# eBay/KPRN

Hardware: AMD Instinct MI355X
Metric: paths/sec (train+score) at path_len=6 d=64 (higher is better)
Workload: dtype f32

## Files before the change

### kprn_amd/csrc/batch_index.hip

```cpp
#include <string.h>
#include <rocprim/device/device_radix_sort.hpp>
#include <rocprim/device/device_run_length_encode.hpp>
#include <rocprim/device/device_select.hpp>
#include <rocprim/iterator/counting_iterator.hpp>

#include <algorithm>

#include "kprn_internal.h"

namespace bidx {

namespace {
__global__ void k_keys(const int32_t* __restrict__ idx, int64_t N, int T, int F, const int32_t* __restrict__ tile_k,
                       const int32_t* __restrict__ meta, int kcap, int sentinel, int32_t* __restrict__ keys, int32_t* __restrict__ vals) {
  const int64_t i = (int64_t)blockIdx.x * blockDim.x + threadIdx.x;
  const int64_t nsteps = N * T;
  if (i < nsteps) {
    const int64_t n = i / T;
    const int t = (int)(i - n * T);
    const bool skipped = tile_k && t < tile_k[n >> 6];
    keys[i] = skipped ? sentinel : idx[i * F + F - 2] - 1;
    vals[i] = (int32_t)i;
  } else if (i < nsteps + kcap) {
    const int t = (int)(i - nsteps);
    const int64_t npad = (N + 63) / 64 * 64;
    keys[i] = (t < meta[0]) ? meta[8 + F - 2] - 1 : sentinel;
    vals[i] = (int32_t)(npad * T + t);
  }
}
__global__ void k_drop_sentinel(const int32_t* __restrict__ uniq, const int32_t* __restrict__ runs, int sentinel, int32_t* __restrict__ count_out) {
  const int n = *runs;
  *count_out = (n > 0 && uniq[n - 1] == sentinel) ? n - 1 : n;
}
int bits_for(int64_t v) { int b = 1; while (((int64_t)1 << b) < v) ++b; return b; }

__global__ void k_find_ref(const int32_t* __restrict__ idx, int64_t N, int T, int F, int c0, int32_t* __restrict__ meta) {
  const int64_t n = (int64_t)blockIdx.x * blockDim.x + threadIdx.x;
  if (n >= N) return;
  const int32_t* r = idx + n * T * F;
  bool same = true;
  for (int c = c0; c < F; ++c) same &= (r[c] == r[F + c]);
  if (same) atomicMin(meta + 1, (int32_t)n);
}
__global__ void k_prefix_len(const int32_t* __restrict__ idx, int64_t N, int T, int F, int c0, int kcap, int32_t* __restrict__ meta,
                             int32_t* __restrict__ keys, int32_t* __restrict__ vals) {
  const int64_t n = (int64_t)blockIdx.x * blockDim.x + threadIdx.x;
  if (n >= N) return;
  const int ref = meta[1];
  int k = 0;
  if (ref != 0x7fffffff) {
    const int32_t* q = idx + (int64_t)ref * T * F;
    const int32_t* r = idx + n * T * F;
    const int kmax = (T - 2 < kcap) ? T - 2 : kcap;
    while (k < kmax) {
      bool same = true;
      for (int c = c0; c < F; ++c) same &= (r[k * F + c] == q[c]);
      if (!same) break;
      ++k;
    }
    if (n == 0) for (int c = 0; c < F; ++c) meta[8 + c] = q[c];
  }
  keys[n] = k;
  vals[n] = (int32_t)n;
}
__global__ void k_prefix_apply(const int32_t* __restrict__ idx, int64_t N, int T, int F, const int32_t* __restrict__ ksorted,
                               const int32_t* __restrict__ perm, int32_t* __restrict__ idx_s, int32_t* __restrict__ slot_of, int32_t* __restrict__ tile_k,
                               int32_t* __restrict__ meta) {
  const int64_t i = (int64_t)blockIdx.x * blockDim.x + threadIdx.x;
  const int64_t row = (int64_t)T * F;
  if (i < N * row) {
    const int64_t n = i / row;
    idx_s[i] = idx[(int64_t)perm[n] * row + (i - n * row)];
  }
  if (i < N) slot_of[perm[i]] = (int32_t)i;
  if (i < (N + 63) / 64) tile_k[i] = ksorted[i * 64];
  if (i == 0) meta[0] = ksorted[N - 1];
}
}

size_t prefix_scratch_bytes(int64_t N, int kcap) {
  size_t t1 = 0;
  int32_t* p = nullptr;
  (void)rocprim::radix_sort_pairs(nullptr, t1, p, p, p, p, (size_t)N, 0, bits_for(kcap + 1), (hipStream_t)0);
  return (size_t)N * 3 * sizeof(int32_t) + ((t1 + 255) & ~(size_t)255) + 1024;
}

void prefix_plan(hipStream_t s, const int32_t* idx, int64_t N, int T, int F, int nT, int kcap, int32_t* idx_s, int32_t* perm, int32_t* slot_of, int32_t* tile_k,
                 int32_t* meta, void* scratch, size_t scratch_sz) {
  int32_t* keys = (int32_t*)scratch;
  int32_t* vals = keys + N;
  int32_t* ksorted = vals + N;
  char* tmp = (char*)(ksorted + N);
  tmp = (char*)(((uintptr_t)tmp + 255) & ~(uintptr_t)255);
  const size_t tmp_bytes = scratch_sz - (size_t)(tmp - (char*)scratch);
  const int c0 = F - nT - 2;
  HIP_TRY(hipMemsetAsync(meta, 0, (size_t)(8 + F) * sizeof(int32_t), s));
  HIP_TRY(hipMemsetD32Async((hipDeviceptr_t)(meta + 1), 0x7fffffff, 1, s));
  const dim3 gn((unsigned)((N + 255) / 256));
  hipLaunchKernelGGL(k_find_ref, gn, dim3(256), 0, s, idx, N, T, F, c0, meta);
  hipLaunchKernelGGL(k_prefix_len, gn, dim3(256), 0, s, idx, N, T, F, c0, kcap, meta, keys, vals);
  HIP_TRY(hipGetLastError());
  size_t need = 0;
  HIP_TRY(rocprim::radix_sort_pairs(nullptr, need, keys, ksorted, vals, perm, (size_t)N, 0, bits_for(kcap + 1), s));
  KPRN_REQUIRE(need <= tmp_bytes, KPRN_E_DEVICE, "prefix plan scratch too small");
  HIP_TRY(rocprim::radix_sort_pairs(tmp, need, keys, ksorted, vals, perm, (size_t)N, 0, bits_for(kcap + 1), s));
  const int64_t work = N * T * F;
  hipLaunchKernelGGL(k_prefix_apply, dim3((unsigned)((work + 255) / 256)), dim3(256), 0, s, idx, N, T, F, ksorted, perm, idx_s, slot_of, tile_k, meta);
  HIP_TRY(hipGetLastError());
}

size_t scratch_bytes(int64_t n_index, int Ve) {
  size_t t1 = 0, t2 = 0;
  int32_t* p = nullptr;
  (void)rocprim::radix_sort_pairs(nullptr, t1, p, p, p, p, (size_t)n_index, 0, bits_for((int64_t)Ve + 1), (hipStream_t)0);
  (void)rocprim::run_length_encode(nullptr, t2, p, (size_t)n_index, p, p, p, (hipStream_t)0);
  const size_t tmp = (t1 > t2 ? t1 : t2);
  return (size_t)n_index * 3 * sizeof(int32_t) + ((tmp + 255) & ~(size_t)255) + 1024 + 256;
}

void build(hipStream_t s, const int32_t* idx, int64_t N, int T, int F, int Ve, const int32_t* tile_k, const int32_t* meta, int kcap,
           int32_t* key_sorted, int32_t* pos_sorted, int32_t* uniq, int32_t* n_uniq_dev, void* scratch, size_t scratch_sz) {
  const int64_t n_index = N * T + (tile_k ? kcap : 0);
  if (n_index <= 0) return;
  int32_t* keys = (int32_t*)scratch;
  int32_t* vals = keys + n_index;
  int32_t* counts = vals + n_index;
  char* tmp = (char*)(counts + n_index);
  tmp = (char*)(((uintptr_t)tmp + 255) & ~(uintptr_t)255);
  int32_t* runs = (int32_t*)tmp;
  tmp += 256;
  size_t tmp_bytes = scratch_sz - (size_t)(tmp - (char*)scratch);
  const int sentinel = Ve;
  const int bits = bits_for((int64_t)Ve + 1);
  hipLaunchKernelGGL(k_keys, dim3((unsigned)((n_index + 255) / 256)), dim3(256), 0, s, idx, N, T, F, tile_k, meta, tile_k ? kcap : 0, sentinel, keys, vals);
  HIP_TRY(hipGetLastError());
  size_t need = 0;
  HIP_TRY(rocprim::radix_sort_pairs(nullptr, need, keys, key_sorted, vals, pos_sorted, (size_t)n_index, 0, bits, s));
  KPRN_REQUIRE(need <= tmp_bytes, KPRN_E_DEVICE, "batch index scratch too small (sort)");
  HIP_TRY(rocprim::radix_sort_pairs(tmp, need, keys, key_sorted, vals, pos_sorted, (size_t)n_index, 0, bits, s));
  HIP_TRY(rocprim::run_length_encode(nullptr, need, key_sorted, (size_t)n_index, uniq, counts, runs, s));
  KPRN_REQUIRE(need <= tmp_bytes, KPRN_E_DEVICE, "batch index scratch too small (rle)");
  HIP_TRY(rocprim::run_length_encode(tmp, need, key_sorted, (size_t)n_index, uniq, counts, runs, s));
  hipLaunchKernelGGL(k_drop_sentinel, dim3(1), dim3(1), 0, s, uniq, runs, sentinel, n_uniq_dev);
  HIP_TRY(hipGetLastError());
}

}

namespace bidx {
namespace {
template <int FRAG, bool DET>
__device__ __forceinline__ void entity_grad_body(const float* __restrict__ DX, const int32_t* __restrict__ key_sorted,
                                                 const int32_t* __restrict__ pos_sorted, int64_t nsteps, int64_t N, int T, int D, int dt, int de,
                                                 int sentinel, float* __restrict__ gWe, int n_ent_blocks, int n_red_blocks, const SlabReduce red,
                                                 const SmallGrad sg, const int dbg, float* const det_seg, float* const det_sg) {
  const int order = (dbg >> 4) & 3;
  const int n_pass = gridDim.x - n_ent_blocks;
  int bid = blockIdx.x, rb = -1;
  if (order == 1) { if (bid < n_pass) { rb = bid; } else bid -= n_pass; }
  else if (order == 2) {
    const int both = 2 * (n_pass < n_ent_blocks ? n_pass : n_ent_blocks);
    if (bid < both) { if (bid & 1) rb = bid >> 1; else bid >>= 1; }
    else if (n_pass > n_ent_blocks) rb = bid - n_ent_blocks;
    else bid -= n_pass;
  } else if (bid >= n_ent_blocks) rb = bid - n_ent_blocks;
  if (rb >= 0) {
    if (dbg & 2) return;
    if (rb >= n_red_blocks) {
      if constexpr (DET) small_grad_block<true>(sg, rb - n_red_blocks, det_sg);
      else if (!(dbg & 8)) small_grad_block(sg, rb - n_red_blocks);
      return;
    }
    if (dbg & 4) return;
    const int nbx = (red.n_elem + 255) / 256;
    slab_reduce_block(red, rb % nbx, (rb / nbx) % red.ny, rb / (nbx * red.ny));
    return;
  }
  const int lane = threadIdx.x & 63;
  const int64_t seg = (int64_t)bid * 4 + (threadIdx.x >> 6);
  const int64_t base = seg * 64;
  if (base >= nsteps) return;
  const int cnt = (int)((nsteps - base < 64) ? (nsteps - base) : 64);
  const int64_t mine = base + (lane < cnt ? lane : cnt - 1);
  const int key_ld = key_sorted[mine], pos_ld = pos_sorted[mine];
  const int kb_ld = key_sorted[base > 0 ? base - 1 : 0], ka_ld = key_sorted[base + cnt < nsteps ? base + cnt : nsteps - 1];
  const int my_key = (lane < cnt) ? key_ld : -1;
  if (__builtin_amdgcn_readlane(my_key, 0) == sentinel) return;
  const int my_pos = (lane < cnt) ? pos_ld : 0;
  const int key_before = (base > 0) ? kb_ld : -1;
  const int key_after = (base + cnt < nsteps) ? ka_ld : -1;
  const int waves_per_group = D >> 4;
  const int key_next = __shfl_down(my_key, 1, 64);
  const bool is_end = (lane < cnt) && (lane == cnt - 1 || key_next != my_key);
  const unsigned long long endmask = __ballot(is_end);
  const bool continues = __builtin_amdgcn_readlane(my_key, (cnt - 1) & 63) == key_after;
  for (int c0 = 0; c0 < de; c0 += 64) {
    const bool act = c0 + lane < de;
    const int ecol = act ? c0 + lane : de - 1;
    const int col = dt + ecol;
    const int coff = (col >> 4) * 256 + (col & 15) * 4;
    float acc = 0.f;
    bool opened_here = __builtin_amdgcn_readlane(my_key, 0) != key_before;
#pragma unroll
    for (int hf = 0; hf < 2; ++hf) {
      if (hf * 32 >= cnt) break;
      float v[32];
#pragma unroll
      for (int i2 = 0; i2 < 32; ++i2) {
        const int i = 32 * hf + i2;
        const int p = __builtin_amdgcn_readlane(my_pos, i);
        const int n = p / T, t = p - n * T;
        int64_t off;
        if (FRAG == 1) {
          const int rr = n & 15;
          off = ((int64_t)(n >> 4) * T + t) * ((int64_t)waves_per_group * 256) + (rr >> 2) * 64 + (rr & 3) + coff;
        } else if (FRAG == 2) {
          off = (int64_t)p * de + ecol;
        } else {
          off = ((int64_t)t * N + n) * D + col;
        }
        v[i2] = DX[off];
      }
#pragma unroll
      for (int i2 = 0; i2 < 32; ++i2) {
        const int i = 32 * hf + i2;
        acc += v[i2];
        if (endmask & (1ull << i)) {
          const int k = __builtin_amdgcn_readlane(my_key, i);
          const bool whole = opened_here && !(i == cnt - 1 && continues);
          if (act && k != sentinel) {
            float* dst = gWe + (int64_t)k * de + ecol;
            if (whole) *dst = acc;
            else if constexpr (DET) det_seg[(seg * 2 + (opened_here ? 1 : 0)) * de + ecol] = acc;
            else if (!(dbg & 1)) unsafeAtomicAdd(dst, acc);
          }
          acc = 0.f;
          opened_here = true;
        }
      }
    }
  }
}
template <int FRAG>
__global__ __launch_bounds__(256) void k_entity_grad(const float* __restrict__ DX, const int32_t* __restrict__ key_sorted,
                                                     const int32_t* __restrict__ pos_sorted, int64_t nsteps, int64_t N, int T, int D, int dt, int de,
                                                     int sentinel, float* __restrict__ gWe, int n_ent_blocks, int n_red_blocks, SlabReduce red,
                                                     SmallGrad sg, int dbg) {
  entity_grad_body<FRAG, false>(DX, key_sorted, pos_sorted, nsteps, N, T, D, dt, de, sentinel, gWe, n_ent_blocks, n_red_blocks, red, sg, dbg, nullptr, nullptr);
}
__global__ __launch_bounds__(256) void k_egrad_det(const float* __restrict__ DX, const int32_t* __restrict__ key_sorted, const int32_t* __restrict__ pos_sorted,
                                                   int64_t nsteps, int64_t N, int T, int D, int dt, int de, int sentinel, float* __restrict__ gWe,
                                                   int n_ent_blocks, int n_red_blocks, SlabReduce red, SmallGrad sg, DetEntity det) {
  entity_grad_body<2, true>(DX, key_sorted, pos_sorted, nsteps, N, T, D, dt, de, sentinel, gWe, n_ent_blocks, n_red_blocks, red, sg, 0, det.seg_part, det.sg_part);
}
__global__ __launch_bounds__(256) void k_egrad_det_rowmajor(const float* __restrict__ DX, const int32_t* __restrict__ key_sorted, const int32_t* __restrict__ pos_sorted,
                                                            int64_t nsteps, int64_t N, int T, int D, int dt, int de, int sentinel, float* __restrict__ gWe,
                                                            int n_ent_blocks, int n_red_blocks, SlabReduce red, SmallGrad sg, DetEntity det) {
  entity_grad_body<0, true>(DX, key_sorted, pos_sorted, nsteps, N, T, D, dt, de, sentinel, gWe, n_ent_blocks, n_red_blocks, red, sg, 0, det.seg_part, det.sg_part);
}

__global__ __launch_bounds__(256) void k_det_tail(const int32_t* __restrict__ key_sorted, int64_t nsteps, int de, int sentinel, float* __restrict__ gWe,
                                                  int n_ent_blocks, DetEntity det, SmallGrad sg, int n_sg_groups) {
  constexpr int DEPTH = 16;
  if ((int)blockIdx.x >= n_ent_blocks) {
    const int ncb_t = sg.dt >> 4, ncb = ncb_t + (sg.dr >> 4);
    const int cb = (int)blockIdx.x - n_ent_blocks;
    const bool is_type = cb < ncb_t;
    const int v = threadIdx.x >> 4, c = threadIdx.x & 15;
    float acc = 0.f;
    for (int g0 = 0; g0 < n_sg_groups; g0 += DEPTH) {
      float x[DEPTH];
#pragma unroll
      for (int u = 0; u < DEPTH; ++u) {
        const int g = g0 + u < n_sg_groups ? g0 + u : n_sg_groups - 1;
        x[u] = det.sg_part[((int64_t)g * ncb + cb) * 256 + threadIdx.x];
      }
#pragma unroll
      for (int u = 0; u < DEPTH; ++u) if (g0 + u < n_sg_groups) acc += x[u];
    }
    if (v < (is_type ? sg.Vt : sg.Vr)) {
      if (is_type) sg.gWt[(int64_t)v * sg.dt + cb * 16 + c] += acc;
      else sg.gWr[(int64_t)v * sg.dr + (cb - ncb_t) * 16 + c] += acc;
    }
    return;
  }
  const int lane = threadIdx.x & 63;
  const int64_t seg = (int64_t)blockIdx.x * 4 + (threadIdx.x >> 6);
  const int64_t base = seg * 64;
  if (base + 64 >= nsteps) return;
  const int k = key_sorted[base + 63];
  if (k == sentinel || key_sorted[base + 64] != k) return;
  if (key_sorted[base] == k && base > 0 && key_sorted[base - 1] == k) return;
  const int64_t n_seg = (nsteps + 63) / 64;
  for (int c0 = 0; c0 < de; c0 += 64) {
    const int ecol = c0 + lane < de ? c0 + lane : de - 1;
    float acc = det.seg_part[(seg * 2 + 1) * de + ecol];
    bool more = true;
    for (int64_t s0 = seg + 1; more; s0 += DEPTH) {
      float x[DEPTH];
      int ks[DEPTH];
#pragma unroll
      for (int u = 0; u < DEPTH; ++u) {
        const int64_t sc = s0 + u < n_seg ? s0 + u : n_seg - 1;
        ks[u] = key_sorted[sc * 64];
        x[u] = det.seg_part[(sc * 2) * de + ecol];
      }
#pragma unroll
      for (int u = 0; u < DEPTH; ++u) {
        more = more && s0 + u < n_seg && ks[u] == k;
        if (more) acc += x[u];
      }
    }
    if (c0 + lane < de) gWe[(int64_t)k * de + ecol] += acc;
  }
}
}

void entity_grad_tail(hipStream_t s, const int32_t* key_sorted, int64_t n_index, int de, int Ve, float* gWe, const DetEntity& det, const SmallGrad* sg) {
  const int64_t segs = (n_index + 63) / 64;
  const int n_ent = (int)((segs + 3) / 4);
  SmallGrad g;
  memset(&g, 0, sizeof(g));
  int ncb = 0, groups = 0;
  if (sg) { g = *sg; ncb = (g.dt >> 4) + (g.dr >> 4); groups = g.nblocks / ncb; }
  if (n_ent + ncb <= 0) return;
  hipLaunchKernelGGL(k_det_tail, dim3((unsigned)(n_ent + ncb)), dim3(256), 0, s, key_sorted, n_index, de, Ve, gWe, n_ent, det, g, groups);
  HIP_TRY(hipGetLastError());
}

void entity_grad(hipStream_t s, const float* DX, int frag_order, const int32_t* key_sorted, const int32_t* pos_sorted, int64_t n_index, int64_t N,
                 int T, int D, int dt, int de, int Ve, float* gWe, const SlabReduce* red, const SmallGrad* sg, const DetEntity* det) {
  if (n_index <= 0 && !red && !sg) return;
  const int64_t segs = (n_index + 63) / 64;
  const int n_ent = (int)((segs + 3) / 4);
  SlabReduce r;
  memset(&r, 0, sizeof(r));
  SmallGrad g;
  memset(&g, 0, sizeof(g));
  int n_red = 0, n_sg = 0;
  if (red) { r = *red; n_red = ((r.n_elem + 255) / 256) * r.ny * r.L; }
  if (sg) { g = *sg; n_sg = g.nblocks; }
  static const int dbg = KPRN_DEV_ENV("KPRN_EGRAD_DBG") ? atoi(KPRN_DEV_ENV("KPRN_EGRAD_DBG")) : 0;
  const dim3 grid((unsigned)(n_ent + n_red + n_sg));
  if (det) {
    KPRN_REQUIRE(frag_order == 2 || (frag_order == 0 && !red && !sg), KPRN_E_UNSUPPORTED,
                 "deterministic entity gradient: the compact entity slice, or row-major dx without passenger jobs");
    if (frag_order == 0)
      hipLaunchKernelGGL(k_egrad_det_rowmajor, grid, dim3(256), 0, s, DX, key_sorted, pos_sorted, n_index, N, T, D, dt, de, Ve, gWe, n_ent, n_red, r, g, *det);
    else
    hipLaunchKernelGGL(k_egrad_det, grid, dim3(256), 0, s, DX, key_sorted, pos_sorted, n_index, N, T, D, dt, de, Ve, gWe, n_ent, n_red, r, g, *det);
  } else
  if (frag_order == 1) hipLaunchKernelGGL(k_entity_grad<1>, grid, dim3(256), 0, s, DX, key_sorted, pos_sorted, n_index, N, T, D, dt, de, Ve, gWe, n_ent, n_red, r, g, dbg);
  else if (frag_order == 2) hipLaunchKernelGGL(k_entity_grad<2>, grid, dim3(256), 0, s, DX, key_sorted, pos_sorted, n_index, N, T, D, dt, de, Ve, gWe, n_ent, n_red, r, g, dbg);
  else hipLaunchKernelGGL(k_entity_grad<0>, grid, dim3(256), 0, s, DX, key_sorted, pos_sorted, n_index, N, T, D, dt, de, Ve, gWe, n_ent, n_red, r, g, dbg);
  HIP_TRY(hipGetLastError());
}
}

namespace bidx {
namespace {
typedef float f32x4m __attribute__((ext_vector_type(4)));
__global__ void k_add_rank(const int32_t* __restrict__ buf, int cap, int de, float* __restrict__ G, int32_t* __restrict__ mark) {
  const int count = buf[0];
  const int per = de >> 2;
  const float* rows = (const float*)(buf + 4 + cap);
  for (int64_t i = (int64_t)blockIdx.x * blockDim.x + threadIdx.x; i < (int64_t)count * per; i += (int64_t)gridDim.x * blockDim.x) {
    const int k = (int)(i / per), c = (int)(i - (int64_t)k * per) * 4;
    const int row = buf[4 + k];
    f32x4m* dst = (f32x4m*)(G + (int64_t)row * de + c);
    *dst = *dst + *(const f32x4m*)(rows + (int64_t)k * de + c);
    if (c == 0) mark[row] = 1;
  }
}
__global__ void k_add_rank_scalar(const int32_t* __restrict__ buf, int cap, int de, float* __restrict__ G, int32_t* __restrict__ mark) {
  const int count = buf[0];
  const float* rows = (const float*)(buf + 4 + cap);
  for (int64_t i = (int64_t)blockIdx.x * blockDim.x + threadIdx.x; i < (int64_t)count * de; i += (int64_t)gridDim.x * blockDim.x) {
    const int k = (int)(i / de), c = (int)(i - (int64_t)k * de);
    const int row = buf[4 + k];
    G[(int64_t)row * de + c] += rows[(int64_t)k * de + c];
    if (c == 0) mark[row] = 1;
  }
}
__global__ void k_unmark(const int32_t* __restrict__ all, int world, int cap, int64_t stride, int32_t* __restrict__ mark) {
  const int64_t i = (int64_t)blockIdx.x * blockDim.x + threadIdx.x;
  if (i >= (int64_t)world * cap) return;
  const int r = (int)(i / cap), k = (int)(i - (int64_t)r * cap);
  const int32_t* buf = all + (int64_t)r * stride;
  if (k < buf[0]) mark[buf[4 + k]] = 0;
}
}

size_t merge_scratch_bytes(int64_t n, int Ve) {
  size_t t1 = 0;
  int32_t* p = nullptr;
  (void)rocprim::select(nullptr, t1, rocprim::counting_iterator<int32_t>(0), p, p, p, (size_t)Ve, (hipStream_t)0);
  return ((t1 + 255) & ~(size_t)255) + 1024;
}

void merge_rows(hipStream_t s, const void* all, int world, int cap, int de, int Ve, float* G, int32_t* union_rows, int32_t* union_count,
                int32_t* mark, void* scratch, size_t scratch_sz, int64_t tail_words) {
  const int64_t n = (int64_t)world * cap;
  if (n <= 0) return;
  const int64_t stride = 4 + (int64_t)cap * (1 + de) + tail_words;
  for (int r = 0; r < world; ++r) {
    const int32_t* buf = (const int32_t*)all + (int64_t)r * stride;
    if ((de & 3) == 0) {
      const int64_t work = (int64_t)cap * (de >> 2);
      hipLaunchKernelGGL(k_add_rank, dim3((unsigned)std::min<int64_t>((work + 255) / 256, 16384)), dim3(256), 0, s, buf, cap, de, G, mark);
    } else {
      const int64_t work = (int64_t)cap * de;
      hipLaunchKernelGGL(k_add_rank_scalar, dim3((unsigned)std::min<int64_t>((work + 255) / 256, 16384)), dim3(256), 0, s, buf, cap, de, G, mark);
    }
  }
  size_t need = 0;
  HIP_TRY(rocprim::select(nullptr, need, rocprim::counting_iterator<int32_t>(0), mark, union_rows, union_count, (size_t)Ve, s));
  KPRN_REQUIRE(need <= scratch_sz, KPRN_E_DEVICE, "merge scratch too small (select)");
  HIP_TRY(rocprim::select(scratch, need, rocprim::counting_iterator<int32_t>(0), mark, union_rows, union_count, (size_t)Ve, s));
  hipLaunchKernelGGL(k_unmark, dim3((unsigned)((n + 255) / 256)), dim3(256), 0, s, (const int32_t*)all, world, cap, stride, mark);
  HIP_TRY(hipGetLastError());
}

}
```

### kprn_amd/csrc/kernels_basic.hip

```cpp
#include <string.h>
#include "kprn_internal.h"
#include "adam_rows_dev.h"
#include "reduce_dev.h"

namespace {

constexpr int TPB = 256;
inline unsigned nblocks(int64_t n, int per = TPB) { return (unsigned)((n + per - 1) / per); }

__device__ __forceinline__ void lds_atomic_add(float* p, float v) {
  typedef __attribute__((address_space(3))) float lds_float;
  __hip_atomic_fetch_add((lds_float*)p, v, __ATOMIC_RELAXED, __HIP_MEMORY_SCOPE_WORKGROUP);
}

__device__ __forceinline__ float wave_sum(float v) {
#pragma unroll
  for (int o = 32; o > 0; o >>= 1) v += __shfl_down(v, o, 64);
  return v;
}

__global__ void k_validate(const int32_t* __restrict__ idx, int64_t nsteps, int F, int nT, int Vt, int Ve, int Vr, int32_t* flag) {
  int64_t i = (int64_t)blockIdx.x * blockDim.x + threadIdx.x;
  if (i >= nsteps) return;
  const int32_t* f = idx + i * F;
// ... 1319 lines not shown
      if (lane < dcols) lds_atomic_add(&acc[id[u] * dcols + lane], x[u][0]);
      if (lane + 64 < dcols) lds_atomic_add(&acc[id[u] * dcols + lane + 64], x[u][1]);
    }
  }
  __syncthreads();
  for (int i = threadIdx.x; i < V * dcols; i += 256) {
    const float v = acc[i];
    if (v != 0.f && !(dbg & 2)) unsafeAtomicAdd(gW + i, v);
  }
}

template <int RT, bool DET = false>
__global__ __launch_bounds__(256) void k_table_grad_mfma(const int32_t* __restrict__ idx, int64_t N, int T, int F, int idcol, int slots,
                                                          const float* __restrict__ dX, int D, int col0, int dcols, int V, float* __restrict__ gW,
                                                          int pos_per_block) {
  typedef float f4 __attribute__((ext_vector_type(4)));
  const int lane = threadIdx.x & 63, wv = threadIdx.x >> 6;
  const int kk = lane >> 4, n16 = lane & 15;
  const int ncb = (dcols + 15) >> 4;
  f4 acc[RT][2];
#pragma unroll
  for (int r = 0; r < RT; ++r) { acc[r][0] = f4{0.f, 0.f, 0.f, 0.f}; acc[r][1] = f4{0.f, 0.f, 0.f, 0.f}; }
  const int64_t total = N * T;
  const int64_t p0 = (int64_t)blockIdx.x * pos_per_block;
  const int np = (int)((p0 + pos_per_block < total ? p0 + pos_per_block : total) - p0);
  const int t0 = (int)(p0 / N);
  const int64_t n0 = p0 - (int64_t)t0 * N;
  if (wv >= ncb) return;
  const int c_a = 16 * wv + n16, c_b = 16 * (wv + 4) + n16;
  const bool has_a = wv < ncb && c_a < dcols, has_b = wv + 4 < ncb && c_b < dcols;
  constexpr int UN = 4;
  for (int q0 = 0; q0 < np; q0 += 4 * UN) {
    float xa[UN], xb[UN];
    int id[UN];
    int64_t ioff[UN];
#pragma unroll
    for (int u = 0; u < UN; ++u) {
      const int q = q0 + 4 * u + kk;
      const bool live = q < np;
      int t = t0;
      int64_t n = n0 + (live ? q : 0);
      while (n >= N) { n -= N; ++t; }
      const float* src = dX + (p0 + (live ? q : 0)) * D + col0;
      const float va = src[has_a ? c_a : 0], vb = src[has_b ? c_b : 0];
      ioff[u] = (n * T + t) * F + idcol;
      const int idr = idx[ioff[u]];
      xa[u] = (live && has_a) ? va : 0.f;
      xb[u] = (live && has_b) ? vb : 0.f;
      id[u] = live ? idr - 1 : -1;
    }
#pragma unroll
    for (int u = 0; u < UN; ++u) {
      for (int sl = 0; sl < slots; ++sl) {
        const int idv = (sl == 0) ? id[u] : ((id[u] >= 0) ? idx[ioff[u] + sl] - 1 : -1);
#pragma unroll
        for (int r = 0; r < RT; ++r) {
          if (RT > 1 && __ballot((idv >> 4) == r) == 0) continue;
          const float onehot = (idv == 16 * r + n16) ? 1.f : 0.f;
          acc[r][0] = __builtin_amdgcn_mfma_f32_16x16x4f32(onehot, xa[u], acc[r][0], 0, 0, 0);
          if (wv + 4 < ncb) acc[r][1] = __builtin_amdgcn_mfma_f32_16x16x4f32(onehot, xb[u], acc[r][1], 0, 0, 0);
        }
      }
    }
  }
#pragma unroll
  for (int r = 0; r < RT; ++r)
#pragma unroll
    for (int i = 0; i < 4; ++i) {
      const int v = 16 * r + 4 * kk + i;
      if (v < V) {
        if constexpr (DET) {
          float* const blk = gW + (int64_t)blockIdx.x * V * dcols;
          if (has_a) blk[(int64_t)v * dcols + c_a] = acc[r][0][i];
          if (has_b) blk[(int64_t)v * dcols + c_b] = acc[r][1][i];
        } else {
          if (has_a && acc[r][0][i] != 0.f) unsafeAtomicAdd(gW + (int64_t)v * dcols + c_a, acc[r][0][i]);
          if (has_b && acc[r][1][i] != 0.f) unsafeAtomicAdd(gW + (int64_t)v * dcols + c_b, acc[r][1][i]);
        }
      }
    }
}

static bool table_grad_mfma(hipStream_t s, const int32_t* idx, int64_t N, int T, int F, int idcol, int slots, const float* dX, int D, int col0, int dcols,
                            int V, float* gW, DetScratch* det = nullptr) {
  if (dcols <= 0 || dcols > 128 || V <= 0 || V > 128) return false;
  static const int ppb_env = KPRN_DEV_ENV("KPRN_TABLE_GRAD_PPB") ? atoi(KPRN_DEV_ENV("KPRN_TABLE_GRAD_PPB")) : 0;
  const int ppb = ppb_env > 0 ? ppb_env : 512;
  const int64_t total = N * T;
  const dim3 grid((unsigned)((total + ppb - 1) / ppb));
  if (det) {
    float* const slab = det_reserve(det, s, (int64_t)grid.x * V * dcols);
#define KPRN_TGD(RT_) hipLaunchKernelGGL((k_table_grad_mfma<RT_, true>), grid, dim3(256), 0, s, idx, N, T, F, idcol, slots, dX, D, col0, dcols, V, slab, ppb)
    if (V <= 16) KPRN_TGD(1);
    else if (V <= 32) KPRN_TGD(2);
    else if (V <= 64) KPRN_TGD(4);
    else KPRN_TGD(8);
#undef KPRN_TGD
    slab_join(s, slab, (int)grid.x, (int64_t)V * dcols, 1, V * dcols, gW, (int64_t)V * dcols);
    return true;
  }
#define KPRN_TG(RT_) hipLaunchKernelGGL(k_table_grad_mfma<RT_>, grid, dim3(256), 0, s, idx, N, T, F, idcol, slots, dX, D, col0, dcols, V, gW, ppb)
  if (V <= 16) KPRN_TG(1);
  else if (V <= 32) KPRN_TG(2);
  else if (V <= 64) KPRN_TG(4);
  else KPRN_TG(8);
#undef KPRN_TG
  return true;
}

static bool table_grad_lds(hipStream_t s, const int32_t* idx, int64_t N, int T, int F, int idcol, int slots, const float* dX, int D, int col0, int dcols,
                           int V, float* gW) {
  const size_t bytes = (size_t)V * dcols * sizeof(float);
  if (dcols <= 0 || dcols > 128 || bytes > 64 * 1024) return false;
  static PerDeviceOnce attr_set;
  if (bytes > 48 * 1024 && attr_set.need()) {
    HIP_TRY(hipFuncSetAttribute((const void*)k_table_grad_lds, hipFuncAttributeMaxDynamicSharedMemorySize, 64 * 1024));
  }
  const int64_t total = N * T;
  int ppb = 512;
  while (ppb < 8192 && (int64_t)V * dcols * 8 > (int64_t)ppb * dcols) ppb *= 2;
  static const int ppb_env = KPRN_DEV_ENV("KPRN_TABLE_GRAD_PPB") ? atoi(KPRN_DEV_ENV("KPRN_TABLE_GRAD_PPB")) : 0;
  if (ppb_env > 0) ppb = ppb_env;
  static const int dbg_env = KPRN_DEV_ENV("KPRN_TABLE_GRAD_DBG") ? atoi(KPRN_DEV_ENV("KPRN_TABLE_GRAD_DBG")) : 0;
  hipLaunchKernelGGL(k_table_grad_lds, dim3((unsigned)((total + ppb - 1) / ppb)), dim3(256), bytes, s, idx, N, T, F, idcol, slots, dX, D, col0, dcols, V, gW, ppb, dbg_env);
  return true;
}

__global__ __launch_bounds__(256) void k_onehot_cols(const int32_t* __restrict__ idx, int64_t NT, int64_t N, int T, int F, int Vr, int Vt, float* __restrict__ X, int64_t ldx,
                                                     int col0, int ns) {
  const int nq = ns >> 2;
  const int64_t g = (int64_t)blockIdx.x * 256 + threadIdx.x;
  if (g >= NT * nq) return;
  const int64_t pos = g / nq;
  const int q = (int)(g - pos * nq);
  const int64_t t = pos / N, n = pos - t * N;
  const int32_t* id = idx + (n * T + t) * F;
  const int r = id[F - 1] - 1, y = Vr + id[F - 3] - 1;
  float4 v;
  v.x = (4 * q == r || 4 * q == y) ? 1.f : 0.f;
  v.y = (4 * q + 1 == r || 4 * q + 1 == y) ? 1.f : 0.f;
  v.z = (4 * q + 2 == r || 4 * q + 2 == y) ? 1.f : 0.f;
  v.w = (4 * q + 3 == r || 4 * q + 3 == y) ? 1.f : 0.f;
  float* dst = X + pos * ldx + col0 + 4 * q;
  dst[0] = v.x; dst[1] = v.y; dst[2] = v.z; dst[3] = v.w;
}
void onehot_cols(hipStream_t s, const int32_t* idx, int64_t N, int T, int F, int Vr, int Vt, float* X, int64_t ldx, int col0, int ns) {
  const int64_t work = N * T * (ns >> 2);
  if (work <= 0) return;
  hipLaunchKernelGGL(k_onehot_cols, dim3((unsigned)((work + 255) / 256)), dim3(256), 0, s, idx, N * T, N, T, F, Vr, Vt, X, ldx, col0, ns);
  HIP_TRY(hipGetLastError());
}
__global__ __launch_bounds__(256) void k_small_tables_finish_f32(const float* __restrict__ Ct, int ns, int GH, int Din, int dt, int de, int dr, int Vt, int Vr,
                                                                 const float* __restrict__ Wt, const float* __restrict__ Wr, const float* __restrict__ Wi,
                                                                 float* __restrict__ gWi, float* __restrict__ gWt, float* __restrict__ gWr, int with_e) {
  __shared__ float g[128];
  const int tid = threadIdx.x, NZ = ns + (with_e ? de : 0);
  if ((int)blockIdx.x < GH) {
    const int k = blockIdx.x;
    const float* row = Ct + (int64_t)k * NZ;
    if (tid < ns) g[tid] = row[tid];
    __syncthreads();
    for (int j = tid; j < Din; j += 256) {
      float v = 0.f;
      if (j < dt) {
        for (int y = 0; y < Vt; ++y) v += g[Vr + y] * Wt[y * dt + j];
      } else if (j < dt + de) {
        if (!with_e) continue;
        v = row[ns + j - dt];
      } else {
        const int jj = j - dt - de;
        for (int r = 0; r < Vr; ++r) v += g[r] * Wr[r * dr + jj];
      }
      gWi[(int64_t)k * Din + j] += v;
    }
    return;
  }
  __shared__ float red[256];
  const int r = (int)blockIdx.x - GH;
  const bool rel = r < Vr;
  const int w = rel ? dr : dt, col0 = rel ? dt + de : 0;
  const int j = tid & 15, sb = tid >> 4;
  for (int j0 = 0; j0 < w; j0 += 16) {
    const int jj = j0 + j, jc = jj < w ? jj : w - 1;
    float acc = 0.f;
#pragma unroll 4
    for (int k = sb; k < GH; k += 16) acc += Ct[(int64_t)k * NZ + r] * Wi[(int64_t)k * Din + col0 + jc];
    red[tid] = acc;
    __syncthreads();
    if (sb == 0 && jj < w) {
      float v = 0.f;
#pragma unroll
      for (int q = 0; q < 16; ++q) v += red[q * 16 + j];
      (rel ? gWr + (int64_t)r * dr : gWt + (int64_t)(r - Vr) * dt)[jj] += v;
    }
    __syncthreads();
  }
}
void small_tables_finish(hipStream_t s, const float* Ct, int ns, int GH, int Din, int dt, int de, int dr, int Vt, int Vr, const float* Wt, const float* Wr,
                         const float* Wi, float* gWi, float* gWt, float* gWr, bool ct_has_entity) {
  hipLaunchKernelGGL(k_small_tables_finish_f32, dim3((unsigned)(GH + Vr + Vt)), dim3(256), 0, s, Ct, ns, GH, Din, dt, de, dr, Vt, Vr, Wt, Wr, Wi, gWi, gWt, gWr,
                     ct_has_entity ? 1 : 0);
  HIP_TRY(hipGetLastError());
}

bool embed_scatter_det_ok(int dt, int dr, int Vt, int Vr) { return (dt == 0 || (dt <= 128 && Vt >= 1 && Vt <= 128)) && (dr == 0 || (dr <= 128 && Vr >= 1 && Vr <= 128)); }

void embed_scatter(hipStream_t s, const int32_t* idx, int64_t N, int T, int F, int nT, const float* dX, int dt, int de, int dr, int Vt, int Vr,
                   float* gWt, float* gWe, float* gWr, bool skip_entity, DetScratch* det) {
  if (N <= 0) return;
  const int D_ = dt + de + dr;
  static const bool old_path = KPRN_DEV_ENV("KPRN_TABLE_GRAD") && strcmp(KPRN_DEV_ENV("KPRN_TABLE_GRAD"), "old") == 0;
  bool type_small = false, rel_small = false;
  static const bool lds_path = KPRN_DEV_ENV("KPRN_TABLE_GRAD") && strcmp(KPRN_DEV_ENV("KPRN_TABLE_GRAD"), "lds") == 0;
  if (det) {
    KPRN_REQUIRE(!old_path && !lds_path && skip_entity && embed_scatter_det_ok(dt, dr, Vt, Vr), KPRN_E_UNSUPPORTED,
                 "deterministic: the embedding scatter has a deterministic form for type / relation tables of at most 128 rows x 128 columns behind the occurrence index only");
    if (dt > 0) table_grad_mfma(s, idx, N, T, F, F - nT - 2, nT, dX, D_, 0, dt, Vt, gWt, det);
    if (dr > 0) table_grad_mfma(s, idx, N, T, F, F - 1, 1, dX, D_, dt + de, dr, Vr, gWr, det);
    CHECK_LAUNCH();
    return;
  }
  if (!old_path && !lds_path) {
    if (dt > 0) type_small = table_grad_mfma(s, idx, N, T, F, F - nT - 2, nT, dX, D_, 0, dt, Vt, gWt);
    if (dr > 0) rel_small = table_grad_mfma(s, idx, N, T, F, F - 1, 1, dX, D_, dt + de, dr, Vr, gWr);
  } else if (lds_path) {
    if (dt > 0 && Vt > 16) type_small = table_grad_lds(s, idx, N, T, F, F - nT - 2, nT, dX, D_, 0, dt, Vt, gWt);
    if (dr > 0 && Vr > 16) rel_small = table_grad_lds(s, idx, N, T, F, F - 1, 1, dX, D_, dt + de, dr, Vr, gWr);
  }
  const int ppb = 512;
  if (!type_small && dt > 0 && Vt <= 16) {
    hipLaunchKernelGGL(k_small_table_grad, dim3((unsigned)((N * T + ppb - 1) / ppb), (unsigned)((dt + 63) / 64)), dim3(256), 0, s, idx, N, T, F, F - nT - 2, nT,
                       dX, D_, 0, dt, Vt, gWt, ppb);
    type_small = true;
  }
  if (!rel_small && dr > 0 && Vr <= 16) {
    hipLaunchKernelGGL(k_small_table_grad, dim3((unsigned)((N * T + ppb - 1) / ppb), (unsigned)((dr + 63) / 64)), dim3(256), 0, s, idx, N, T, F, F - 1, 1, dX,
                       D_, dt + de, dr, Vr, gWr, ppb);
    rel_small = true;
  }
  if ((type_small || dt == 0) && (rel_small || dr == 0) && (skip_entity || de == 0)) { CHECK_LAUNCH(); return; }
  if (type_small) { Vt = 0; }
  size_t small = (size_t)((int64_t)(type_small ? 0 : Vt) * dt + (int64_t)(rel_small ? 0 : Vr) * dr) * sizeof(float);
  int use_lds = small <= 96 * 1024 ? 1 : 0;
  const int spb = 256;
  int64_t total = N * T;
  if (use_lds && small > 48 * 1024)
    HIP_TRY(hipFuncSetAttribute((const void*)k_embed_scatter, hipFuncAttributeMaxDynamicSharedMemorySize, (int)small));
  hipLaunchKernelGGL(k_embed_scatter, dim3((unsigned)((total + spb - 1) / spb)), dim3(TPB), use_lds ? small : 0, s, idx, N, T, F, nT, dX, dt, de,
                     dr, type_small ? 0 : Vt, rel_small ? 0 : Vr, gWt, gWe, gWr, use_lds, spb, skip_entity ? 1 : 0, type_small ? 1 : 0, rel_small ? 1 : 0);
  CHECK_LAUNCH();
}

void sumsq(hipStream_t s, const float* x, int64_t n, float* out) {
  if (n <= 0) return;
  unsigned g = nblocks(n);
  if (g > 2048) g = 2048;
  hipLaunchKernelGGL(k_sumsq, dim3(g), dim3(TPB), 0, s, x, n, out);
  CHECK_LAUNCH();
}

void sumsq_rows(hipStream_t s, const float* G, const int32_t* rows, const int32_t* count, int d, float* out) {
  hipLaunchKernelGGL(k_sumsq_rows, dim3(1024), dim3(TPB), 0, s, G, rows, count, d, out);
  CHECK_LAUNCH();
}

void sumsq_det(hipStream_t s, const float* x, int64_t n, const float* G, const int32_t* rows, const int32_t* count, int d, float* partial, float* out) {
  const int nb = SUMSQ_DET_BLOCKS / 2;
  hipLaunchKernelGGL(k_sumsq_det, dim3(2 * nb), dim3(256), 0, s, x, n, G, rows, count, d, nb, partial);
  hipLaunchKernelGGL(k_sum_partials, dim3(1), dim3(256), 0, s, partial, 2 * nb, out, 0);
  CHECK_LAUNCH();
}

static AdamDenseJob dense_job(float* x, float* g, float* m, float* v, int64_t n, float step, float b1, float b2, float eps,
                              const float* norm2, float clip, float l2, int consume, int64_t z0, int zn0, int64_t z1, int zn1, float* tab_slot) {
  AdamDenseJob a;
  a.x = x; a.g = g; a.m = m; a.v = v; a.n = n; a.step = step; a.b1 = b1; a.b2 = b2; a.eps = eps; a.norm2 = norm2; a.clip = clip; a.l2 = l2;
  a.reg = (norm2 != nullptr || l2 != 0.f) ? 1 : 0; a.consume = consume; a.z0 = z0; a.zn0 = zn0; a.z1 = z1; a.zn1 = zn1; a.tab_slot = tab_slot;
  return a;
}
void adam_dense(hipStream_t s, float* x, float* g, float* m, float* v, int64_t n, float step, float b1, float b2, float eps,
                const float* norm2, float clip, float l2, int consume, int64_t z0, int zn0, int64_t z1, int zn1, float* tab_slot) {
  if (n <= 0) return;
  hipLaunchKernelGGL(k_adam_dense, dim3(nblocks(n)), dim3(TPB), 0, s, dense_job(x, g, m, v, n, step, b1, b2, eps, norm2, clip, l2, consume, z0, zn0, z1, zn1, tab_slot));
  CHECK_LAUNCH();
}

void adagrad_dense(hipStream_t s, float* x, float* g, float* G, int64_t n, float clr, const float* norm2, float clip, float l2, int consume,
                   int64_t z0, int zn0, int64_t z1, int zn1) {
  if (n <= 0) return;
  int reg = (norm2 != nullptr || l2 != 0.f) ? 1 : 0;
  hipLaunchKernelGGL(k_adagrad_dense, dim3(nblocks(n)), dim3(TPB), 0, s, x, g, G, n, clr, norm2, clip, l2, reg, consume, z0, zn0, z1, zn1);
  CHECK_LAUNCH();
}

void adam_rows(hipStream_t s, float* W, float* g, float* m, float* v, int32_t* last, const int32_t* rows, const int32_t* count, int64_t max_rows,
               int d, int32_t t_now, int apply_step, const float* step_tab, float b1, float b2, float eps, int64_t pad_row) {
  if (max_rows <= 0) return;
  const bool al = !(((uintptr_t)W | (uintptr_t)g | (uintptr_t)m | (uintptr_t)v) & 15);
  AdamDenseJob none;
  memset(&none, 0, sizeof(none));
  if (al && d == 32) { const int nb = (int)nblocks(max_rows * 8); hipLaunchKernelGGL(k_adam_rows_v<8>, dim3(nb), dim3(TPB), 0, s, W, g, m, v, last, rows, count, t_now, apply_step, step_tab, b1, b2, eps, pad_row, nb, -1.f, none); }
  else if (al && d == 64) { const int nb = (int)nblocks(max_rows * 16); hipLaunchKernelGGL(k_adam_rows_v<16>, dim3(nb), dim3(TPB), 0, s, W, g, m, v, last, rows, count, t_now, apply_step, step_tab, b1, b2, eps, pad_row, nb, -1.f, none); }
  else if (al && d == 128) { const int nb = (int)nblocks(max_rows * 32); hipLaunchKernelGGL(k_adam_rows_v<32>, dim3(nb), dim3(TPB), 0, s, W, g, m, v, last, rows, count, t_now, apply_step, step_tab, b1, b2, eps, pad_row, nb, -1.f, none); }
  else hipLaunchKernelGGL(k_adam_rows, dim3(nblocks(max_rows * 64)), dim3(TPB), 0, s, W, g, m, v, last, rows, count, d, t_now, apply_step, step_tab, b1,
                          b2, eps, pad_row);
  CHECK_LAUNCH();
}

bool adam_step_merged(hipStream_t s, float* W, float* g, float* m, float* v, int32_t* last, const int32_t* rows, const int32_t* count, int64_t max_rows, int d,
                      int32_t t_now, const float* step_tab, int64_t pad_row, float* dx, float* dg, float* dm, float* dv, int64_t dn, float step, float b1,
                      float b2, float eps, const float* norm2, float clip, float l2, int64_t z0, int zn0, int64_t z1, int zn1, float* tab_slot) {
  const bool al = !(((uintptr_t)W | (uintptr_t)g | (uintptr_t)m | (uintptr_t)v) & 15);
  if (max_rows <= 0 || dn <= 0 || !al || !(d == 32 || d == 64 || d == 128)) return false;
  const AdamDenseJob dj = dense_job(dx, dg, dm, dv, dn, step, b1, b2, eps, norm2, clip, l2, 1, z0, zn0, z1, zn1, tab_slot);
  const int nd = (int)nblocks(dn);
  if (d == 32) { const int nb = (int)nblocks(max_rows * 8); hipLaunchKernelGGL(k_adam_rows_v<8>, dim3(nb + nd), dim3(TPB), 0, s, W, g, m, v, last, rows, count, t_now, 1, step_tab, b1, b2, eps, pad_row, nb, step, dj); }
  else if (d == 64) { const int nb = (int)nblocks(max_rows * 16); hipLaunchKernelGGL(k_adam_rows_v<16>, dim3(nb + nd), dim3(TPB), 0, s, W, g, m, v, last, rows, count, t_now, 1, step_tab, b1, b2, eps, pad_row, nb, step, dj); }
  else { const int nb = (int)nblocks(max_rows * 32); hipLaunchKernelGGL(k_adam_rows_v<32>, dim3(nb + nd), dim3(TPB), 0, s, W, g, m, v, last, rows, count, t_now, 1, step_tab, b1, b2, eps, pad_row, nb, step, dj); }
  CHECK_LAUNCH();
  return true;
}

void adam_flush_all(hipStream_t s, float* W, float* m, float* v, int32_t* last, int64_t V, int d, int32_t t_now, const float* step_tab, float b1,
                    float b2, float eps, int64_t pad_row) {
  hipLaunchKernelGGL(k_adam_flush_all, dim3(nblocks(V * 64)), dim3(TPB), 0, s, W, m, v, last, V, d, t_now, step_tab, b1, b2, eps, pad_row);
  CHECK_LAUNCH();
}

void adagrad_rows(hipStream_t s, float* W, float* g, float* G, const int32_t* rows, const int32_t* count, int64_t max_rows, int d, float clr,
                  int64_t pad_row) {
  if (max_rows <= 0) return;
  hipLaunchKernelGGL(k_adagrad_rows, dim3(nblocks(max_rows * 64)), dim3(TPB), 0, s, W, g, G, rows, count, d, clr, pad_row);
  CHECK_LAUNCH();
}

void zero_pad3(hipStream_t s, float* a, int na, float* b, int nb, float* c, int nc) {
  const int n = na > nb ? (na > nc ? na : nc) : (nb > nc ? nb : nc);
  hipLaunchKernelGGL(k_zero_pad3, dim3(nblocks(n)), dim3(TPB), 0, s, a, na, b, nb, c, nc);
  CHECK_LAUNCH();
}

void zero_rows(hipStream_t s, float* W, int64_t row, int d) {
  hipLaunchKernelGGL(k_zero_row, dim3(nblocks(d)), dim3(TPB), 0, s, W, row, d);
  CHECK_LAUNCH();
}

void pack_rows(hipStream_t s, float* G, const int32_t* rows, const int32_t* count, int64_t max_rows, int d, int32_t* ids_out, float* rows_out,
               int32_t* count_out, const float* tail_src, int64_t n_tail, float* tail_dst) {
  int64_t waves = max_rows > 0 ? max_rows : 1;
  const bool al = !(((uintptr_t)G | (uintptr_t)rows_out | (uintptr_t)tail_dst) & 15);
  const int tail_blocks = n_tail > 0 ? (int)std::min<int64_t>((n_tail + 255) / 256, 256) : 0;
#define KPRN_PACK_V(LG)                                                                                                                      \
  {                                                                                                                                          \
    const int rb = (int)nblocks(waves * LG);                                                                                                 \
// ... 49 lines not shown
```

### kprn_amd/csrc/kprn_api.hip

```cpp
#include <ctype.h>
#include <dlfcn.h>
#include <errno.h>
#include <math.h>
#include <stdio.h>
#include <string.h>

#include <algorithm>
#include <thread>

#include "kprn_internal.h"

static thread_local std::string g_create_error;

ProfScope::ProfScope(kprn_handle* h_, const char* n, hipStream_t on) : h(h_), name(n), strm(on ? on : h_->stream) {
  if (!h->prof_on) return;
  if (!h->prof_filter.empty() && strncmp(n, h->prof_filter.c_str(), h->prof_filter.size()) != 0) return;
  auto get = [&]() {
    hipEvent_t e;
    if (!h->event_pool.empty()) { e = h->event_pool.back(); h->event_pool.pop_back(); }
    else if (hipEventCreate(&e) != hipSuccess) e = nullptr;
    return e;
  };
  a = get(); b = get();
  if (a) hipEventRecord(a, strm);
// ... 1646 lines not shown
  API_END(h)
}

int kprn_stream(kprn_handle* h, void** stream) {
  API_BEGIN(h)
  KPRN_REQUIRE(stream, KPRN_E_ARG, "NULL argument");
  *stream = (void*)h->stream;
  h->stream_known = true;
  API_END(h)
}

static const char kMagic[8] = {'K', 'P', 'R', 'N', 'A', 'M', 'D', '1'};

int kprn_save(kprn_handle* h, const char* path) {
  API_BEGIN(h)
  KPRN_REQUIRE(path, KPRN_E_ARG, "path is NULL");
  std::vector<float> flat((size_t)h->n_params);
  {
    int rc = kprn_get_flat_params(h, flat.data(), h->n_params);
    if (rc != KPRN_OK) return rc;
  }
  FILE* f = fopen(path, "wb");
  KPRN_REQUIRE(f, KPRN_E_IO, std::string("cannot open for writing: ") + path);
  const kprn_config& c = h->cfg;
  int32_t hdr[16] = {c.Vt, c.Ve, c.Vr, c.dt, c.de, c.dr, c.F, c.num_types, c.H, c.L, c.C, c.rnn_type, c.reducer, c.K, 0, 0};
  bool ok = fwrite(kMagic, 1, 8, f) == 8 && fwrite(hdr, sizeof(int32_t), 16, f) == 16 && fwrite(&h->n_params, sizeof(int64_t), 1, f) == 1 &&
            fwrite(flat.data(), sizeof(float), flat.size(), f) == flat.size();
  ok = (fclose(f) == 0) && ok;
  KPRN_REQUIRE(ok, KPRN_E_IO, "short write");
  API_END(h)
}

int kprn_load(kprn_handle* h, const char* path) {
  API_BEGIN(h)
  KPRN_REQUIRE(path, KPRN_E_ARG, "path is NULL");
  FILE* f = fopen(path, "rb");
  KPRN_REQUIRE(f, KPRN_E_IO, std::string("cannot open: ") + path);
  char magic[8];
  int32_t hdr[16];
  int64_t n = 0;
  bool ok = fread(magic, 1, 8, f) == 8 && memcmp(magic, kMagic, 8) == 0 && fread(hdr, sizeof(int32_t), 16, f) == 16 &&
            fread(&n, sizeof(int64_t), 1, f) == 1;
  const kprn_config& c = h->cfg;
  const int32_t want[12] = {c.Vt, c.Ve, c.Vr, c.dt, c.de, c.dr, c.F, c.num_types, c.H, c.L, c.C, c.rnn_type};
  if (ok) ok = memcmp(hdr, want, sizeof(want)) == 0 && n == h->n_params;
  std::vector<float> flat;
  if (ok) { flat.resize((size_t)n); ok = fread(flat.data(), sizeof(float), flat.size(), f) == flat.size(); }
  fclose(f);
  KPRN_REQUIRE(ok, KPRN_E_IO, "not a kprn checkpoint for this configuration");
  return kprn_set_flat_params(h, flat.data(), n);
  API_END(h)
}

int kprn_profile_enable(kprn_handle* h, int32_t on) {
  API_BEGIN(h)
  prof_drain(h);
  h->prof_on = on != 0;
  API_END(h)
}
int kprn_profile_reset(kprn_handle* h) {
  API_BEGIN(h)
  prof_drain(h);
  h->prof.clear();
  API_END(h)
}
int kprn_profile_get(kprn_handle* h, kprn_prof_entry* out, int32_t cap, int32_t* n) {
  API_BEGIN(h)
  KPRN_REQUIRE(n, KPRN_E_ARG, "n is NULL");
  prof_drain(h);
  int k = 0;
  for (auto& kv : h->prof) {
    if (out && k < cap) {
      memset(&out[k], 0, sizeof(kprn_prof_entry));
      strncpy(out[k].name, kv.first.c_str(), sizeof(out[k].name) - 1);
      out[k].total_ms = kv.second.total_ms;
      out[k].launches = kv.second.launches;
    }
    ++k;
  }
  *n = k;
  API_END(h)
}

int kprn_debug_gemm(kprn_handle* h, int32_t what, int64_t M, int32_t N, int64_t K, int32_t iters, float* ms) {
  API_BEGIN(h)
  KPRN_REQUIRE(ms && M > 0 && N > 0 && K > 0 && iters > 0, KPRN_E_ARG, "bad argument");
  hipStream_t s = h->stream;
  if (what == 5 || what == 6) {
    *ms = bf16p::debug_gemm16(s, M, N, K, what == 6 ? 1024 : 1, iters);
    return KPRN_OK;
  }
  float *A = nullptr, *B = nullptr, *C = nullptr, *X = nullptr, *Z = nullptr;
  hipEvent_t e0, e1;
  HIP_TRY(hipEventCreate(&e0)); HIP_TRY(hipEventCreate(&e1));
  try {
    const int64_t H = N, Din = K;
    if (what <= 2) {
      const int64_t na = M * K, nb = (int64_t)N * K, nc = (what == 2) ? (int64_t)N * K : M * (int64_t)N;
      A = dalloc<float>(what == 2 ? M * (int64_t)N : na); B = dalloc<float>(what == 2 ? M * K : nb); C = dalloc<float>(nc);
      kk::fill_uniform(s, A, what == 2 ? M * (int64_t)N : na, 0.1f, 1, 0); kk::fill_uniform(s, B, what == 2 ? M * K : nb, 0.1f, 2, 0);
      HIP_TRY(hipMemsetAsync(C, 0, (size_t)nc * sizeof(float), s));
    } else {
      X = dalloc<float>(M * Din); A = dalloc<float>(2 * M * H); B = dalloc<float>(4 * H * (Din + H) + 8 * H); C = dalloc<float>(2 * M * H); Z = dalloc<float>(M * 4 * H);
      kk::fill_uniform(s, X, M * Din, 0.1f, 1, 0); kk::fill_uniform(s, A, 2 * M * H, 0.1f, 2, 0); kk::fill_uniform(s, B, 4 * H * (Din + H) + 8 * H, 0.1f, 3, 0);
    }
    for (int it = -2; it < iters; ++it) {
      if (it == 0) HIP_TRY(hipEventRecord(e0, s));
      if (what == 0) gemm::run(s, A, K, 1, B, 1, K, C, N, M, N, K, false, nullptr, 1);
      else if (what == 1) gemm::run(s, A, K, 1, B, N, 1, C, N, M, N, K, false, nullptr, 1);
      else if (what == 2) gemm::run(s, A, 1, N, B, K, 1, C, K, N, (int)K, M, true, nullptr, 1024);
      else if (what == 3) gemm::lstm_step(s, X, Din, (int)Din, B, B + 4 * H * (Din + H), A, B + 4 * H * Din, A + M * H, C, C + M * H, H, Z, M, (int)H);
      else gemm::rnn_step(s, X, Din, (int)Din, B, B + 4 * H * (Din + H), A, B + H * Din, B + 4 * H * (Din + H) + H, A + M * H, Z, C, H, M, (int)H, 1);
    }
    HIP_TRY(hipEventRecord(e1, s));
    HIP_TRY(hipEventSynchronize(e1));
    float t = 0.f;
    HIP_TRY(hipEventElapsedTime(&t, e0, e1));
    *ms = t / (float)iters;
  } catch (...) { dfree(A); dfree(B); dfree(C); dfree(X); dfree(Z); hipEventDestroy(e0); hipEventDestroy(e1); throw; }
  dfree(A); dfree(B); dfree(C); dfree(X); dfree(Z); hipEventDestroy(e0); hipEventDestroy(e1);
  API_END(h)
}

int kprn_set_option(kprn_handle* h, const char* key, const char* value) {
  API_BEGIN(h)
  KPRN_REQUIRE(key && value, KPRN_E_ARG, "NULL argument");
  if (strcmp(key, "impl") == 0) {
    if (strcmp(value, "auto") == 0) h->impl = 0;
    else if (strcmp(value, "generic") == 0) h->impl = 1;
    else throw KprnError{KPRN_E_ARG, "impl must be auto or generic"};
  } else if (strcmp(key, "prefix_plan") == 0) {
    h->prefix_plan = atoi(value) ? 1 : 0;
  } else if (strcmp(key, "small_tiles") == 0) {
    join_score(h);
    h->small_tiles_on = atoi(value) != 0;
  } else if (strcmp(key, "tile_handover") == 0) {
    const int v = atoi(value);
    KPRN_REQUIRE(v >= 0 && v <= 2, KPRN_E_ARG, "tile_handover must be 0, 1 or 2");
    h->tile_handover = v;
  } else if (strcmp(key, "rank_sort_min") == 0) {
    const int v = atoi(value);
    KPRN_REQUIRE(v >= 257 && v <= 4097, KPRN_E_ARG, "rank_sort_min must be in 257..4097");
    h->rank_sort_min = v;
  } else if (strcmp(key, "adam_merged") == 0) {
    h->adam_merged = atoi(value) != 0;
  } else if (strcmp(key, "bwd_pipe") == 0) {
    h->bwd_pipe = atoi(value) != 0;
  } else if (strcmp(key, "score_dual") == 0) {
    const int v = atoi(value);
    KPRN_REQUIRE(v >= 0 && v <= 2, KPRN_E_ARG, "score_dual must be 0, 1 or 2");
    h->score_dual = v;
  } else if (strcmp(key, "catchup_prefix") == 0) {
    h->catchup_prefix = atoi(value) != 0;
  } else if (strcmp(key, "fused_small_tables") == 0) {
    h->fused_small_tables = atoi(value) != 0;
  } else if (strcmp(key, "persist_layers") == 0) {
    const int v = atoi(value);
    KPRN_REQUIRE(v >= 0 && v <= 2, KPRN_E_ARG, "persist_layers must be 0, 1 or 2");
    h->persist_layers = v;
  } else if (strcmp(key, "small_tables") == 0) {
    h->small_tables = atoi(value) != 0;
  } else if (strcmp(key, "small_tables_fwd") == 0) {
    join_score(h);
    h->small_tables_fwd = atoi(value) != 0;
  } else if (strcmp(key, "head_select") == 0) {
    join_score(h);
    h->head_select = atoi(value) != 0;
  } else if (strcmp(key, "bf16_t_pad") == 0) {
    bf16p::set_t_pad(atoi(value));
  } else if (strcmp(key, "bf16_gemm_regstage") == 0) {
    bf16p::set_gemm_regstage(atoi(value) != 0);
  } else if (strcmp(key, "bf16_gemm_touch") == 0) {
    bf16p::set_gemm_touch(atoi(value));
  } else if (strcmp(key, "bf16_gemm_pingpong") == 0) {
    bf16p::set_gemm_pingpong(atoi(value) != 0);
  } else if (strcmp(key, "bf16_bptt_dxe") == 0) {
    const int v = atoi(value);
    KPRN_REQUIRE(v == 0 || v == 8 || v == 16, KPRN_E_ARG, "bf16_bptt_dxe must be 0, 8 or 16");
    h->bf16_bptt_dxe = v;
  } else if (strcmp(key, "bf16_small_tables") == 0) {
    h->bf16_small_tables = atoi(value) != 0;
  } else if (strcmp(key, "score_rest_before_bptt") == 0) {
    join_score(h);
    h->score_rest_before_bptt = atoi(value) ? 1 : 0;
  } else if (strcmp(key, "score_rest_in_backward") == 0) {
    join_score(h);
    h->score_rest_in_backward = atoi(value) ? 1 : 0;
    h->after_bptt_hook = h->score_rest_in_backward ? score_rest_hook : nullptr;
  } else if (strcmp(key, "score_split") == 0) {
    join_score(h);
    const double f = atof(value);
    KPRN_REQUIRE(f >= 0.0 && f < 1.0, KPRN_E_ARG, "score_split: a fraction in [0, 1)");
    h->score_split = (float)f;
  } else if (strcmp(key, "score_overlap") == 0) {
    join_score(h);
    h->score_overlap = atoi(value) ? 1 : 0;
  } else if (strcmp(key, "loss_accumulate") == 0) {
    h->loss_accumulate = atoi(value) ? 1 : 0;
  } else if (strcmp(key, "inline_upload") == 0) {
    if (strcmp(value, "side") == 0) h->inline_upload_side = 1;
    else if (strcmp(value, "main") == 0) h->inline_upload_side = 0;
    else throw KprnError{KPRN_E_ARG, "inline_upload must be side or main"};
  } else if (strcmp(key, "train_step_return") == 0) {
    if (strcmp(value, "loss") == 0) h->train_step_drain = 0;
    else if (strcmp(value, "drain") == 0) h->train_step_drain = 1;
    else throw KprnError{KPRN_E_ARG, "train_step_return must be loss or drain"};
  } else if (strcmp(key, "feed_build") == 0) {
    if (strcmp(value, "host") == 0) h->feed_build_host = 1;
    else if (strcmp(value, "device") == 0) h->feed_build_host = 0;
    else throw KprnError{KPRN_E_ARG, "feed_build must be host or device"};
  } else if (strcmp(key, "feed_threads") == 0) {
    const int v = atoi(value);
    KPRN_REQUIRE(v >= 1 && v <= 64, KPRN_E_ARG, "feed_threads must be in 1..64");
    h->feed_threads = v;
  } else if (strcmp(key, "feed_workers") == 0) {
    const int v = atoi(value);
    KPRN_REQUIRE(v >= 1 && v <= 64 && !h->feed_pool, KPRN_E_ARG, "feed_workers must be in 1..64 and set before the first feed");
    h->feed_workers = v;
  } else if (strcmp(key, "profile_filter") == 0) {
    h->prof_filter = value;
  } else if (strcmp(key, "dp_comm_stream") == 0) {
    h->dp_comm_stream_on = atoi(value) != 0;
  } else if (strcmp(key, "dp_fused_update") == 0) {
    h->dp_fused_update = atoi(value) != 0;
  } else if (strcmp(key, "dp_dense_in_pack") == 0) {
    h->dp_dense_in_pack = atoi(value) != 0;
  } else if (strcmp(key, "deterministic") == 0) {
    KPRN_REQUIRE(strcmp(value, "0") == 0 || strcmp(value, "1") == 0 || strcmp(value, "2") == 0, KPRN_E_ARG, "deterministic must be 0, 1 or 2");
    h->deterministic = value[0] - '0';
  } else if (strcmp(key, "dropout") == 0) {
    char* end = nullptr;
    const bool decimal = (isdigit((unsigned char)value[0]) || value[0] == '.') && value[strspn(value, "0123456789.eE+-")] == 0;
    const double p = decimal ? strtod(value, &end) : 0.0;
    KPRN_REQUIRE(decimal && end != value && *end == 0 && p >= 0.0 && p < 1.0 && (double)(float)p < 1.0, KPRN_E_ARG, "dropout must be a decimal rate in [0, 1)");
    if (p > 0.0) {
      KPRN_REQUIRE(h->cfg.rnn_type == 1, KPRN_E_UNSUPPORTED,
                   "dropout > 0: built for rnn_type 1 (rnn) only -- the reference's lstm / gru modules ignore -useDropout (OneModel.lua:237-239), so there is nothing to reproduce");
      KPRN_REQUIRE(h->cfg.compute_dtype == 0, KPRN_E_UNSUPPORTED, "dropout > 0: built for compute_dtype 0 (fp32) only; the bf16-product pipeline has no dropped form");
    }
    h->dropout_p = (float)p;
  } else if (strcmp(key, "dropout_seed") == 0) {
    char* end = nullptr;
    errno = 0;
    const bool hex = value[0] == '0' && (value[1] == 'x' || value[1] == 'X');
    const unsigned long long v = isdigit((unsigned char)value[0]) ? strtoull(value, &end, hex ? 16 : 10) : 0;
    KPRN_REQUIRE(end != nullptr && end != value && !(hex && end == value + 2) && *end == 0 && errno == 0, KPRN_E_ARG, "dropout_seed must be a decimal or 0x hex unsigned 64-bit number");
    h->dropout_seed = (uint64_t)v;
    h->drop_draw = 0;
  } else if (strcmp(key, "reserve_cus") == 0) {
    const int v = atoi(value);
    KPRN_REQUIRE(v >= 0 && v <= 1024, KPRN_E_ARG, "reserve_cus must be in 0..1024");
    h->reserve_cus = v;
  } else {
    throw KprnError{KPRN_E_ARG, std::string("unknown option: ") + key};
  }
  API_END(h)
}

}
```

### kprn_amd/csrc/kprn_internal.h

```cpp
#pragma once
#include <stdlib.h>
#include <hip/hip_runtime.h>
#include <stdint.h>
#include <exception>
#include <functional>
#include <future>
#include <string>
#include <vector>
#include <map>

#include "../../include/kprn.h"
#include "philox_dev.h"

#define KPRN_MAX_LAYERS 8

struct KprnError { int code; std::string msg; };
#define HIP_TRY(expr)                                                                     \
  do {                                                                                    \
    hipError_t e__ = (expr);                                                              \
    if (e__ != hipSuccess)                                                                \
      throw KprnError{KPRN_E_DEVICE, std::string(#expr) + ": " + hipGetErrorString(e__)}; \
  } while (0)
#define KPRN_REQUIRE(cond, code, text) \
  do { if (!(cond)) throw KprnError{(code), std::string(text)}; } while (0)

struct ParamInfo {
  std::string name;
  int64_t flat_off;
  int64_t rows, cols;
  int where;
  int64_t dev_off;
};

struct LayerOff {
  int64_t Wi, bi, Wo, bo;
  int64_t Wc, bc, Uc;
  int Din;
};

struct Workspace {
  int64_t cap_N = 0;
  int cap_T = 0;
  int64_t cap_Nc = 0;
  float* X = nullptr;
  float* Hs = nullptr;
  float* Cs = nullptr;
  float* ACT = nullptr;
  float* dA = nullptr;
  float* dIn = nullptr;
  float* dH = nullptr;
  float* dC = nullptr;
  float* S = nullptr;
  float* dS = nullptr;
  int64_t cap_B = 0;
  float* pooled = nullptr;
  float* probs = nullptr;
  float* sel = nullptr;
  float* dy = nullptr;
  float* mask = nullptr;
  float* HsD = nullptr;
  int64_t cap_HsD = 0;
};

struct ProfEntry { double total_ms = 0; int64_t launches = 0; };

struct DetScratch { float* p = nullptr; int64_t cap = 0; };

namespace fused { constexpr int KCAP = 8; }

struct kprn_graph;
struct kprn_sampler;

struct kprn_batch {
  int32_t B, P, T, F;
  int64_t N = 0;
  int32_t* off = nullptr;
  int32_t* wg = nullptr;
  int32_t n_wg = 0;
  int32_t max_cnt = 0;
  int32_t seg_wave = 0;
  std::vector<int32_t> hrag;
  int32_t* idx = nullptr;
  float* labels = nullptr;
  int32_t* uniq = nullptr;
  int64_t uniq_cap = 0;
  int32_t n_uniq = 0;
  int64_t serial = 0;
  int32_t* key_sorted = nullptr;
  int32_t* pos_sorted = nullptr;
  int64_t n_index = 0;
  int32_t* idx_s = nullptr;
  int32_t* perm = nullptr;
  int32_t* slot_of = nullptr;
  int32_t* tile_k = nullptr;
  int32_t* pmeta = nullptr;
  int kcap = 0;
  int h_kmax = 0;
  int32_t h_ref[16] = {0};
  int64_t exec_steps = 0;
  int32_t* block = nullptr; int64_t block_cap = 0;
  int32_t* d_flag = nullptr;
  int32_t* h_meta = nullptr;
  int64_t h_meta_cap = 0;
  hipEvent_t ev_ready = nullptr;
  bool pending = false;
  bool bad = false;
  bool has_index = true;
  bool idx_valid = true;
  bool host_built = false;
  std::future<void> job;
  int32_t* hs = nullptr; int64_t hs_cap = 0;
  std::vector<int32_t> hw;
  hipEvent_t ev_fork = nullptr, ev_fork2 = nullptr;
  struct HostResult { bool bad = false; int kmax = 0; int32_t ref[16] = {0}; int32_t n_uniq = 0; int64_t exec_steps = 0; } hres;
};

struct kprn_handle {
  kprn_config cfg;
  int D = 0;
  int G = 4;
  hipStream_t stream = nullptr;
  bool own_stream = false;
  bool stream_known = false;
  std::string err;

  std::vector<ParamInfo> params;
  int64_t n_params = 0, n_dense = 0, n_ent = 0;
  int64_t off_Wt = 0, off_Wr = 0, off_outW = 0, off_outb = 0;
  LayerOff layer[KPRN_MAX_LAYERS];
  float *dense = nullptr, *g_dense = nullptr, *s1_dense = nullptr, *s2_dense = nullptr;
  float *We = nullptr, *g_We = nullptr, *s1_We = nullptr, *s2_We = nullptr;

  int32_t* We_last = nullptr;
  int64_t opt_step = 0;
  int opt_method = -1;
  float* step_tab = nullptr;
  float* step_tab_host = nullptr;
  int64_t step_tab_cap = 0;
  bool lazy_pending = false;
  bool ent_dense_mode = false;
  bool ent_grads_dirty = false;
  float last_b1 = 0.9f, last_b2 = 0.999f, last_eps = 1e-8f;

  int32_t* step_rows = nullptr;
  int32_t* step_count = nullptr;
  int64_t step_rows_cap = 0;
  int64_t step_rows_ub = 0;
  const int32_t* rows_view = nullptr; const int32_t* count_view = nullptr; const kprn_batch* view_batch = nullptr;
  bool pad_clean = false;
  bool dense_grads_clean = false;
  int64_t caught_serial = -1, caught_step = -1;
  int64_t grads_serial = -1;
  int64_t next_serial = 1;
  int loss_accumulate = 0;
  float* loss_partial = nullptr; int64_t loss_partial_cap = 0; int loss_pending = 0;
  float* loss_mirror = nullptr; int64_t loss_mirror_cap = 0; hipEvent_t ev_loss = nullptr;
  bool loss_early_armed = false; int loss_early_n = 0; int train_step_drain = 0;
  float* probs_mirror = nullptr; int64_t probs_mirror_cap = 0; float* sel_host_armed = nullptr;
  int32_t* dp_mark = nullptr;
  bool dp_fused_update = false, dp_union_pending = false;
  const void* dp_all = nullptr; int dp_world = 0, dp_cap = 0;
  void* dp_comm = nullptr; int dp_rank = 0, dp_nranks = 0;
  int32_t* dp_gather = nullptr; int64_t dp_gather_words = 0;
  bool dp_comm_stream_on = false, dp_begun = false;
  hipStream_t dp_comm_stream = nullptr; hipEvent_t ev_dp_packed = nullptr, ev_dp_gathered = nullptr;
  bool dp_dense_in_pack = false;
  bool dp_saved_dense_in_pack = false, dp_saved_fused_update = false;
  int32_t* pack_buf = nullptr; int64_t pack_cap = 0, pack_words = 0;

  float* d_loss = nullptr;
  float* d_norm2 = nullptr;
  int32_t* d_flag = nullptr;
  float* h_pinned = nullptr;

  Workspace ws;
  float* score_buf = nullptr;
  void* fused_state = nullptr;
  void* bf16_state = nullptr;
  void* bidx_scratch = nullptr; size_t bidx_scratch_bytes = 0;
  hipStream_t feed_stream = nullptr; hipEvent_t ev_feed_fork = nullptr;
  void* feed_scratch = nullptr; size_t feed_scratch_bytes = 0;
  int feed_build_host = 1;
  int feed_workers = 0, feed_threads = 0;
  void* feed_pool = nullptr;
  void* upload_pool = nullptr;
  hipStream_t upload_stream = nullptr;
  int impl = 0;
  int prefix_plan = 1;
  int score_overlap = 0;
  hipStream_t score_stream = nullptr;
  int side_stream_probes = 0;
  hipEvent_t ev_fork = nullptr, ev_score_done = nullptr;
  kprn_batch* dropin_slot[4] = {nullptr, nullptr, nullptr, nullptr};
  int dropin_next_train = 0, dropin_next_score = 0, dropin_last = 0;
  bool dropin_prev_waited = false, dropin_prev_waited_now = false; int inline_upload_side = 1;
  bool inline_side_ok = true;
  bool score_pending = false;
  int bf16_bptt_dxe = 8;
  int persist_layers = 1;
  bool small_tables_fwd = true;
  bool head_select = true;
  bool small_tables = true;
  float* lp_wot = nullptr; int64_t lp_wot_cap = 0;
  float* st_ctmp = nullptr; int64_t st_ctmp_cap = 0;
  bool bf16_small_tables = true;
  bool small_tiles_on = true;
  int tile_handover = 2; int* ho_fault = nullptr;
  bool adam_merged = true;
  bool bwd_pipe = true;
  int score_dual = 2;
  bool catchup_prefix = true;
  bool fused_small_tables = true;
  float score_split = 0.f;
  int score_rest_in_backward = 0;
  int score_rest_before_bptt = 0;
  hipStream_t rest_stream = nullptr; hipEvent_t ev_part1 = nullptr;
  void (*after_bptt_hook)(kprn_handle*) = nullptr;
  const kprn_batch* score_rest_batch = nullptr; int score_rest_cid = 1; int64_t score_rest_tile0 = 0;
  bool last_forward_side = false;
  bool score_on_main = false;
  const kprn_batch* pool_defer_batch = nullptr; int pool_defer_cid = 0;
  float* S2 = nullptr; float* sel2 = nullptr; int64_t cap_N2 = 0, cap_B2 = 0;
  int reserve_cus = 0;
  int32_t last_B = 0;
  float* board = nullptr; int64_t board_n = 0;
  hipEvent_t ev_put = nullptr; bool put_side = false;
  void* rank_buf = nullptr; size_t rank_buf_bytes = 0;
  int rank_sort_min = 512;
  void* rank_pin = nullptr; size_t rank_pin_bytes = 0, rank_pin_off[2] = {0, 0};
  void* explain_buf = nullptr; size_t explain_buf_bytes = 0;
  void* explain_pin = nullptr; size_t explain_pin_bytes = 0;
  std::vector<kprn_graph*> graphs;
  void* pf_buf = nullptr; size_t pf_buf_bytes = 0;
  std::vector<kprn_sampler*> samplers;
  void* ns_buf = nullptr; size_t ns_buf_bytes = 0;

  int deterministic = 0;
  DetScratch det_slab;
  float* det_seg = nullptr; int64_t det_seg_cap = 0;
  float dropout_p = 0.f;
  uint64_t dropout_seed = 0;
  uint32_t drop_draw = 0, drop_draw_cur = 0;
  bool drop_live = false;
  float* det_norm_part = nullptr;

  bool prof_on = false;

  std::string prof_filter;
  std::map<std::string, ProfEntry> prof;
  struct Pending { std::string name; hipEvent_t a, b;  int launches = 1; };
  std::vector<Pending> prof_pending;
  std::vector<hipEvent_t> event_pool;
};

struct ProfScope {
  kprn_handle* h; const char* name; hipEvent_t a = nullptr, b = nullptr;
  int launches = 1;
  hipStream_t strm;
  ProfScope(kprn_handle* h_, const char* n, hipStream_t on = nullptr);
  ~ProfScope();
};
hipStream_t make_concurrent_stream(kprn_handle* h, int* probes = nullptr);
void prof_drain(kprn_handle* h);
void join_score(kprn_handle* h);

#define API_BEGIN(h)                                   \
  if (!(h)) return KPRN_E_ARG;                         \
  try {                                                \
    HIP_TRY(hipSetDevice((h)->cfg.device_id));         \
    if ((h)->ho_fault && *(volatile int*)(h)->ho_fault) throw KprnError{KPRN_E_DEVICE, "a fused kernel's tile hand-over wait timed out: results since then are invalid"};
#define API_END(h)                                                                        \
  }                                                                                       \
  catch (const KprnError& e) { (h)->err = e.msg; return e.code; }                         \
  catch (const std::exception& e) { (h)->err = e.what(); return KPRN_E_DEVICE; }          \
  catch (...) { (h)->err = "unknown error"; return KPRN_E_DEVICE; }                       \
  return KPRN_OK;

inline void sync_stream(hipStream_t s, bool nothrow) { const hipError_t e = hipStreamSynchronize(s); if (!nothrow) HIP_TRY(e); }
inline void sync_side_streams(kprn_handle* h, bool nothrow = false) {
  for (hipStream_t s : {h->score_stream, h->rest_stream}) if (s) sync_stream(s, nothrow);
}
inline void sync_compute_streams(kprn_handle* h, bool nothrow = false) { sync_side_streams(h, nothrow); sync_stream(h->stream, nothrow); }
inline void sync_all_streams(kprn_handle* h, bool nothrow = false) {
  sync_compute_streams(h, nothrow);
  for (hipStream_t s : {h->feed_stream, h->upload_stream}) if (s) sync_stream(s, nothrow);
}
inline hipStream_t make_priority_stream(bool high) {
  int lo = 0, hi = 0;
  hipStream_t s = nullptr;
  HIP_TRY(hipDeviceGetStreamPriorityRange(&lo, &hi));
  HIP_TRY(hipStreamCreateWithPriority(&s, hipStreamNonBlocking, high ? hi : lo));
  return s;
}

bool use_fused(kprn_handle* h, const kprn_batch* b, bool save_for_backward);
void launch_score_rest(kprn_handle* h);
void materialize_step_rows(kprn_handle* h);
namespace slots {
typedef std::function<void(int32_t* idx_dev, hipStream_t s)> DeviceFill;
void create(kprn_handle* h, const int32_t* idx, const int32_t* counts, const float* labels, int32_t B, int32_t P, int64_t N, int32_t T, int32_t F, kprn_batch** out,
            const DeviceFill* fill = nullptr);
void feed(kprn_handle* h, kprn_batch** slot, const int32_t* idx, const float* labels, const int64_t* rows, int32_t B, int32_t P, int32_t T, int32_t F,
          bool inline_now = false, const int32_t* counts = nullptr, int64_t n_ragged = 0);
void ready(kprn_handle* h, const kprn_batch* b);
void release(kprn_batch* b);
void scratch_reserve(void** scratch, size_t* bytes, size_t need);
}

namespace kk {
void validate_indices(hipStream_t s, const int32_t* idx, int64_t nsteps, int F, int nT, int Vt, int Ve, int Vr, int32_t* flag);
void embed_gather(hipStream_t s, const int32_t* idx, int64_t N, int T, int F, int nT, const float* Wt, const float* We,
                  const float* Wr, int dt, int de, int dr, float* X, bool time_major, float* mask = nullptr );
void lstm_gates_fwd(hipStream_t s, float* act , const float* c_prev, float* c, float* h, int64_t N, int H);
void lstm_gates_bwd(hipStream_t s, const float* act, const float* c, const float* c_prev, const float* dH_up ,
                    float* dH, float* dC, float* dA, int64_t N, int H);
void row_nonzero(hipStream_t s, const float* in, int64_t N, int D, float* mask);
void embed_gather_drop(hipStream_t s, const int32_t* idx, int64_t N, int T, int F, int nT, const float* Wt, const float* We, const float* Wr, int dt, int de,
                       int dr, float* X, float* mask, const philox::DropArgs& a);
void drop_rows(hipStream_t s, const float* in, float* out, int64_t N, int T, int W, const philox::DropArgs& a);
void rnn_cell_fwd(hipStream_t s, float* pre, const float* bh, const float* mask, float* h, int64_t N, int H, int relu);
void rnn_cell_bwd(hipStream_t s, const float* pre, const float* hcur, const float* mask, const float* dH_up, const float* dH, float* dA, int64_t N,
                  int H, int relu);
void add_bias_rows(hipStream_t s, float* Y, const float* b, int64_t rows, int cols);
void add_into(hipStream_t s, float* dst, const float* src, int64_t n);
void col_sum_add(hipStream_t s, const float* A, int64_t rows, int cols, float* out, int64_t ld = 0, float* out2 = nullptr,
                 DetScratch* det = nullptr);
float* det_reserve(DetScratch* det, hipStream_t s, int64_t n);
void slab_join(hipStream_t s, const float* slabs, int nslab, int64_t stride, int64_t rows, int cols, float* dst, int64_t ldc, float* dst2 = nullptr);
void gru_gates_fwd(hipStream_t s, float* a, const float* hp, int64_t N, int H);
void gru_out_fwd(hipStream_t s, float* a, const float* hp, float* h, int64_t N, int H);
void gru_bwd1(hipStream_t s, const float* a, const float* hp, const float* dH, const float* dH_up, float* dA, float* dHdir, int64_t N, int H);
void gru_bwd2(hipStream_t s, const float* a, const float* hp, float* dA, const float* dHdir, float* dH, int64_t N, int H);
void pool_sigmoid(hipStream_t s, const float* S, int B, int P, int C, int reducer, int K, float* pooled, float* probs, int cid, float* sel, float* sel_host = nullptr);
struct TransposeJob { const float* W[4]; float* WT[4]; int n; };
struct PoolJob { const float* S; int B, P, cid; float* sel; float* sel_host; const int32_t* off = nullptr; int wave = 0; };
struct Segs { int B, P; const int32_t* off; const int32_t* wg; int n_wg; int wave; };
void pool_sigmoid_ragged(hipStream_t s, const float* S, const Segs& g, int C, int reducer, int K, float* pooled, float* probs, int cid, float* sel,
                         float* sel_host = nullptr);
int loss_stage_ragged(hipStream_t s, const float* S, const float* labels, const float* hT, const Segs& g, int C, int H, int cid, int reducer, int K,
                      int literal, float invB, float* pooled, float* probs, float* sel, float* dS, const int32_t* slot_of, float* gW_row, float* gb_c,
                      float* partial, const TransposeJob* tj = nullptr, float* partial_host = nullptr, const PoolJob* pj = nullptr);
constexpr int RAGGED_MAX_SEG = 4096;
constexpr int RAGGED_THREAD_MAX = 28;
constexpr int RAGGED_WG_PAIRS = 16;
constexpr int RAGGED_WG_PATHS = 448;
bool ragged_plan(const int32_t* counts, int32_t B, int64_t N, int32_t* off, int32_t* wg, int32_t* summary);
void loss_stage(hipStream_t s, const float* S, const float* labels, const float* hT, int B, int P, int C, int H, int cid, int reducer, int K,
                int literal, float invB, float* pooled, float* probs, float* sel, float* dS, const int32_t* slot_of ,
                float* gW_row, float* gb_c, float* partial, const TransposeJob* tj = nullptr, float* partial_host = nullptr, const PoolJob* pj = nullptr);
void sum_partials(hipStream_t s, const float* partial, int n, float* out, int accumulate);
int loss_partials(int B);
void zero_pad3(hipStream_t s, float* a, int na, float* b, int nb, float* c, int nc);
void head_bwd(hipStream_t s, const float* dS, const float* hT, const float* Wout, int64_t N, int H, int cid, float* dH, float* gWout, float* gbout,
              DetScratch* det = nullptr);
void embed_scatter(hipStream_t s, const int32_t* idx, int64_t N, int T, int F, int nT, const float* dX , int dt, int de, int dr,
                   int Vt, int Vr, float* gWt, float* gWe, float* gWr, bool skip_entity = false, DetScratch* det = nullptr);
bool embed_scatter_det_ok(int dt, int dr, int Vt, int Vr);
void onehot_cols(hipStream_t s, const int32_t* idx, int64_t N, int T, int F, int Vr, int Vt, float* X, int64_t ldx, int col0, int ns);
void small_tables_finish(hipStream_t s, const float* Ct, int ns, int GH, int Din, int dt, int de, int dr, int Vt, int Vr, const float* Wt, const float* Wr,
                         const float* Wi, float* gWi, float* gWt, float* gWr, bool ct_has_entity = true);
void sumsq(hipStream_t s, const float* x, int64_t n, float* out);
void sumsq_rows(hipStream_t s, const float* G, const int32_t* rows, const int32_t* count, int d, float* out);
constexpr int SUMSQ_DET_BLOCKS = 512;
void sumsq_det(hipStream_t s, const float* x, int64_t n, const float* G, const int32_t* rows, const int32_t* count, int d, float* partial, float* out);
void adam_dense(hipStream_t s, float* x, float* g, float* m, float* v, int64_t n, float step, float b1, float b2, float eps,
                const float* norm2, float clip, float l2, int consume, int64_t z0, int zn0, int64_t z1, int zn1, float* tab_slot);
void adagrad_dense(hipStream_t s, float* x, float* g, float* G, int64_t n, float clr, const float* norm2, float clip, float l2, int consume,
                   int64_t z0, int zn0, int64_t z1, int zn1);
void adam_rows(hipStream_t s, float* W, float* g, float* m, float* v, int32_t* last, const int32_t* rows, const int32_t* count, int64_t max_rows,
               int d, int32_t t_now, int apply_step, const float* step_tab, float b1, float b2, float eps, int64_t pad_row);
bool adam_step_merged(hipStream_t s, float* W, float* g, float* m, float* v, int32_t* last, const int32_t* rows, const int32_t* count, int64_t max_rows, int d,
                      int32_t t_now, const float* step_tab, int64_t pad_row, float* dx, float* dg, float* dm, float* dv, int64_t dn, float step, float b1,
                      float b2, float eps, const float* norm2, float clip, float l2, int64_t z0, int zn0, int64_t z1, int zn1, float* tab_slot);
void adam_flush_all(hipStream_t s, float* W, float* m, float* v, int32_t* last, int64_t V, int d, int32_t t_now, const float* step_tab, float b1, float b2, float eps, int64_t pad_row);
void adagrad_rows(hipStream_t s, float* W, float* g, float* G, const int32_t* rows, const int32_t* count, int64_t max_rows, int d, float clr, int64_t pad_row);
void zero_rows(hipStream_t s, float* W, int64_t row, int d);
void pack_rows(hipStream_t s, float* G, const int32_t* rows, const int32_t* count, int64_t max_rows, int d, int32_t* ids_out, float* rows_out, int32_t* count_out,
               const float* tail_src = nullptr, int64_t n_tail = 0, float* tail_dst = nullptr);
bool union_adam(hipStream_t s, const void* all, int world, int cap, int64_t stride, int d, float* W, float* m, float* v, int32_t* last, int32_t t_now,
                const float* step_tab, float b1, float b2, float eps, int64_t pad_row);
void fill_uniform(hipStream_t s, float* x, int64_t n, float a, uint64_t seed, uint64_t offset);
void fill_i32(hipStream_t s, int32_t* x, int64_t n, int32_t v);
void clear_rows(hipStream_t s, float* G, const int32_t* rows, const int32_t* count, int64_t max_rows, int d);
}

namespace rk {
struct Args {
  const float* scores; const int64_t* members; const int64_t* goff; const int32_t* pos;
  int G, mode, K, hist_len;
  int32_t* ranks; int32_t* tk_idx; float* tk_score; unsigned long long* hist;
  int sort_min;
};
int validate(int64_t n_scores, const int64_t* members, const int64_t* goff, const int32_t* pos, int32_t G, int32_t mode, int32_t K, int32_t hist_len,
             int* max_n, std::string* why);
void launch(hipStream_t s, const Args& a, int max_n);
}

namespace pf {
void release_all(kprn_handle* h);
}
namespace ns {
void release_all(kprn_handle* h);
}

namespace ex {
struct Args {
  const float* S;
  const int32_t* off; int B, P;
  int seg_wave;
  int C, cid, reducer, K, M;
  const int32_t* pairs;
  const int64_t* goff; int per_group;
  int64_t n;
  int32_t* idx; float* score; float* weight;
  float* pooled; float* prob;
};
int validate(int32_t B, const int32_t* pairs, int64_t n, int32_t M, std::string* why);
void launch(hipStream_t s, const Args& a, int max_cnt);
}

namespace bidx {
size_t scratch_bytes(int64_t n_index, int Ve);
void build(hipStream_t s, const int32_t* idx, int64_t N, int T, int F, int Ve, const int32_t* tile_k, const int32_t* meta, int kcap,
           int32_t* key_sorted, int32_t* pos_sorted, int32_t* uniq, int32_t* n_uniq_dev, void* scratch, size_t scratch_sz);
size_t prefix_scratch_bytes(int64_t N, int kcap);
void prefix_plan(hipStream_t s, const int32_t* idx, int64_t N, int T, int F, int nT, int kcap, int32_t* idx_s, int32_t* perm, int32_t* slot_of, int32_t* tile_k,
                 int32_t* meta, void* scratch, size_t scratch_sz);
struct SlabReduce {
  const float* part[2]; float* gWi[2]; float* gWo[2]; float* gbi[2];
  int nslab, n_elem;
  int slab;
  float* gG[2];
  int L, ny;
  const float* r1; int kmax, kcap, r1_stride, G, H;
};
__device__ __forceinline__ void slab_reduce_block(const SlabReduce& a, int bx, int by, int l) {
  const int i = bx * 256 + threadIdx.x;
  if (i >= a.n_elem) return;
  const int GH = a.G * a.H, nW = GH * a.H, nB = 2 * nW + GH;
  if (i >= nB && !a.gG[l]) return;
  const float* __restrict__ part = a.part[l];
  float acc[4] = {0.f, 0.f, 0.f, 0.f};
  for (int s = by * 4; s < a.nslab; s += a.ny * 16) {
    float x[16];
#pragma unroll
    for (int u = 0; u < 16; ++u) {
      const int sl = s + (u >> 2) * a.ny * 4 + (u & 3);
      const float v = part[(int64_t)(sl < a.nslab ? sl : a.nslab - 1) * a.slab + i];
      x[u] = (sl < a.nslab) ? v : 0.f;
    }
#pragma unroll
    for (int u = 0; u < 16; ++u) acc[u & 3] += x[u];
  }
  float v = (acc[0] + acc[1]) + (acc[2] + acc[3]);
  if (by == 0 && i < nB) {
    for (int t = 0; t < a.kmax; ++t) {
      const float* r1 = a.r1 + ((int64_t)l * a.kcap + t) * a.r1_stride;
      if (i < nW) v += r1[GH + i / a.H] * r1[2 * GH + a.H + i % a.H];
      else if (i < 2 * nW) v += r1[(i - nW) / a.H] * r1[2 * GH + (i - nW) % a.H];
      else v += r1[GH + (i - 2 * nW)];
    }
  }
  if (i < nW) unsafeAtomicAdd(a.gWi[l] + i, v);
  else if (i < 2 * nW) unsafeAtomicAdd(a.gWo[l] + (i - nW), v);
  else if (i < nB) unsafeAtomicAdd(a.gbi[l] + (i - 2 * nW), v);
  else unsafeAtomicAdd(a.gG[l] + (i - nB), v);
}
struct SmallGrad {
  const float* DX; const int32_t* idx; const int32_t* tile_k;
  int64_t N, n_mtiles; int T, F, nT, dt, de, dr, Vt, Vr;
  float* gWt; float* gWr; int nblocks;
};
template <bool DET = false>
__device__ __forceinline__ void small_grad_block(const SmallGrad& a, int bx, float* det_part = nullptr) {
  typedef float f32x4_ __attribute__((ext_vector_type(4)));
  const int lane = threadIdx.x & 63, wv = threadIdx.x >> 6;
  const int arow = lane & 15, ag = lane >> 4;
  const int ncb_t = a.dt >> 4, ncb = ncb_t + (a.dr >> 4);
  const int cb = bx % ncb, part = (bx / ncb) * 4 + wv, nparts = ((a.nblocks + ncb - 1) / ncb) * 4;
  const bool is_type = cb < ncb_t;
  const int wave_of_block = is_type ? cb : ((a.dt + a.de) >> 4) + (cb - ncb_t);
  const int idcol = is_type ? (a.F - a.nT - 2) : (a.F - 1);
  const int V = is_type ? a.Vt : a.Vr;
  f32x4_ acc = f32x4_{0.f, 0.f, 0.f, 0.f};
  const int64_t items = a.n_mtiles * a.T;
  auto fetch = [&](int64_t it, f32x4_& x, int (&id)[4]) -> bool {
    const int64_t mtile = it / a.T;
    const int t = (int)(it - mtile * a.T);
    const int tk = a.tile_k ? a.tile_k[mtile >> 2] : 0;
    x = *(const f32x4_*)(a.DX + ((mtile * a.T + t) * 4 + wave_of_block) * 256 + lane * 4);
    int raw[4];
#pragma unroll
    for (int r = 0; r < 4; ++r) {
      const int64_t n = mtile * 16 + ag * 4 + r;
      const int rv = a.idx[((n < a.N ? n : a.N - 1) * a.T + t) * a.F + idcol];
      raw[r] = (n < a.N) ? rv : 0;
    }
    const bool live = !(t < tk);
#pragma unroll
    for (int r = 0; r < 4; ++r) id[r] = live ? raw[r] - 1 : -1;
    return live;
  };
  constexpr int DEPTH = 4;
  for (int64_t it0 = part; it0 < items; it0 += (int64_t)nparts * DEPTH) {
    f32x4_ x[DEPTH];
    int id[DEPTH][4];
#pragma unroll
    for (int d = 0; d < DEPTH; ++d) {
      const int64_t it = it0 + (int64_t)d * nparts;
      fetch(it < items ? it : items - 1, x[d], id[d]);
      if (!(it < items)) { id[d][0] = id[d][1] = id[d][2] = id[d][3] = -1; }
    }
#pragma unroll
    for (int d = 0; d < DEPTH; ++d)
#pragma unroll
      for (int r = 0; r < 4; ++r) {
        const float onehot = (id[d][r] == arow) ? 1.f : 0.f;
        const float xv = (id[d][r] >= 0) ? x[d][r] : 0.f;
        acc = __builtin_amdgcn_mfma_f32_16x16x4f32(onehot, xv, acc, 0, 0, 0);
      }
  }
  __shared__ float sg_red[4][16][16];
#pragma unroll
  for (int i = 0; i < 4; ++i) sg_red[wv][4 * ag + i][arow] = acc[i];
  __syncthreads();
  {
    const int v = threadIdx.x >> 4, c = threadIdx.x & 15;
    const float s = (sg_red[0][v][c] + sg_red[1][v][c]) + (sg_red[2][v][c] + sg_red[3][v][c]);
    if constexpr (DET) { det_part[(int64_t)bx * 256 + threadIdx.x] = s; return; }
    if (v < V && s != 0.f) {
      if (is_type) unsafeAtomicAdd(a.gWt + (int64_t)v * a.dt + cb * 16 + c, s);
      else unsafeAtomicAdd(a.gWr + (int64_t)v * a.dr + (cb - ncb_t) * 16 + c, s);
    }
  }
}
struct DetEntity {
  float* seg_part;
  float* sg_part;
};
void entity_grad(hipStream_t s, const float* DX, int frag_order, const int32_t* key_sorted, const int32_t* pos_sorted, int64_t n_index, int64_t N,
                 int T, int D, int dt, int de, int Ve, float* gWe, const SlabReduce* red = nullptr, const SmallGrad* sg = nullptr, const DetEntity* det = nullptr);
void entity_grad_tail(hipStream_t s, const int32_t* key_sorted, int64_t n_index, int de, int Ve, float* gWe, const DetEntity& det, const SmallGrad* sg);
size_t merge_scratch_bytes(int64_t n, int Ve);
void merge_rows(hipStream_t s, const void* all, int world, int cap, int de, int Ve, float* G, int32_t* union_rows, int32_t* union_count,
                int32_t* mark , void* scratch, size_t scratch_sz, int64_t tail_words = 0);
}

namespace bf16p {
bool supported(const kprn_handle* h, const kprn_batch* b);
void forward(kprn_handle* h, const kprn_batch* b, bool save);
void backward(kprn_handle* h, const kprn_batch* b, int cid);
void params_changed(kprn_handle* h, bool entity_rows_only);
void rows_updated(kprn_handle* h, const int32_t* rows, const int32_t* count, int64_t max_rows);
void release(kprn_handle* h);
float debug_gemm16(hipStream_t s, int64_t M, int N, int64_t K, int split_k, int iters);
void set_gemm_touch(int chunks);
void set_gemm_regstage(bool on);
void set_t_pad(int elements);
void set_gemm_pingpong(bool on);
}

namespace fused {
bool fwd_supported(const kprn_handle* h, int T);
void forward(kprn_handle* h, const kprn_batch* b, bool save, int64_t tile_begin = 0, int64_t tile_end = -1, bool ignore_reserve = false, int sel = -1);
bool small_tiles(const kprn_handle* h, int64_t N, bool has_plan);
bool bwd_supported(const kprn_handle* h, int T);
void backward(kprn_handle* h, const kprn_batch* b, int cid);
void params_changed(kprn_handle* h);
bool transpose_job(kprn_handle* h, kk::TransposeJob* tj);
void prefix_forward(kprn_handle* h, const kprn_batch* b);
bool forward_dual(kprn_handle* h, const kprn_batch* bt, const kprn_batch* bs, float* S_score, int sel_train, int sel_score);
bool catch_up_with_prefix(kprn_handle* h, const kprn_batch* b, float* W, float* g, float* m, float* v, int32_t* last, int32_t t_now, const float* step_tab,
                          float b1, float b2, float eps);
void mc_prepare(kprn_handle* h);
void forward_mc(kprn_handle* h, const kprn_batch* b, bool save);
bool prefix_backward(kprn_handle* h, const kprn_batch* b, int64_t n_tiles);
void release(kprn_handle* h);
void handover_stats(kprn_handle* h, const kprn_batch* b, int64_t* out );
}

namespace generic {
void forward(kprn_handle* h, const kprn_batch* b, bool save);
void backward(kprn_handle* h, const kprn_batch* b, int cid);
int small_tables_route(const kprn_handle* h, int F, bool dropped, bool have_index);
void drop_check(const kprn_handle* h, const kprn_batch* b);
}
void ensure_ws_generic(kprn_handle* h, int64_t N, int T);

struct PerDeviceOnce {
  unsigned long long mask = 0;
  bool need() {
    int d = 0;
    if (hipGetDevice(&d) != hipSuccess) return true;
    const unsigned long long bit = 1ull << (d & 63);
    const unsigned long long old = __atomic_fetch_or(&mask, bit, __ATOMIC_RELAXED);
    return !(old & bit);
  }
};

#ifdef KPRN_PERSIST_VARIANTS
#define KPRN_DEV_ENV(name) getenv(name)
#else
#define KPRN_DEV_ENV(name) ((const char*)nullptr)
#endif
inline int kprn_dbg_mask() {
  static const int m = [] { const char* e = getenv("KPRN_DBG"); return e ? atoi(e) : 0; }();
  return m;
}

inline hipError_t kprn_dev_malloc(void** p, size_t bytes) {
  hipError_t e = hipMalloc(p, bytes);
  if (e == hipSuccess) {
    static const bool poison = getenv("KPRN_POISON_ALLOC") != nullptr;
    if (poison) { e = hipMemset(*p, 0xFF, bytes); if (e == hipSuccess) e = hipDeviceSynchronize(); }
  }
  return e;
}

template <typename T>
inline T* dalloc(int64_t n) {
  void* p = nullptr;
  if (n <= 0) n = 1;
  hipError_t e = kprn_dev_malloc(&p, (size_t)n * sizeof(T) + 64);
  if (e != hipSuccess) throw KprnError{KPRN_E_NOMEM, std::string("hipMalloc failed: ") + hipGetErrorString(e)};
  return (T*)p;
}
template <typename T>
inline void dfree(T*& p) { if (p) { hipFree(p); p = nullptr; } }
template <typename T>
inline T* dev_grow(hipStream_t s, T*& p, int64_t& cap, int64_t need, int factor = 1) {
  if (need > cap) {
    HIP_TRY(hipStreamSynchronize(s));
    dfree(p);
    p = dalloc<T>(need * factor);
    cap = need * factor;
  }
  return p;
}
template <typename T>
inline T* dev_grow2(hipStream_t s, T*& p, int64_t& cap, int64_t need) { return dev_grow(s, p, cap, need, 2); }

namespace hostfeed {
struct Shape { int B, P, T, F, nT, Vt, Ve, Vr; };
typedef kprn_batch::HostResult Result;
class Pool;
Pool* make_pool(int workers);
void free_pool(Pool* p);
std::future<void> submit(Pool* p, std::function<void()> fn);
int64_t format_scores(int64_t counter0, const float* probs, const float* labels, int64_t n, char* out, int64_t cap, int nth);
void gather_rows(int32_t* dst, const int32_t* src, int64_t row_words, const int64_t* rows, int64_t n, int nth);
void build(const Shape& g, const int32_t* idx, int kcap, int nth, bool want_index, Result* r, int32_t* idx_s, int32_t* perm, int32_t* slot_of, int32_t* tile_k,
           int32_t* pmeta, int32_t* key_sorted, int32_t* pos_sorted, int32_t* uniq, int32_t* w0, int32_t* w1, int32_t* w2, int32_t* w3);
}

namespace lp32 {
bool supported(int cell , int64_t N, int Din, int H, bool force );
void forward_layer(hipStream_t s, int cell, const float* in, int64_t N, int T, int Din, int H, const float* Wi, const float* Wo, const float* bi, const float* bo,
                   float* hs, float* cs, float* act, const float* mask, int relu, bool save, bool write_all_h, const float* Wc = nullptr ,
                   const float* Uc = nullptr , const float* bc = nullptr );
bool bptt_supported(int cell, int64_t N, int H, bool force);
size_t bptt_scratch_floats(int H, int GH);
void bptt_layer(hipStream_t s, int cell, const float* act, const float* cs, const float* hs, const float* mask, const float* dHup, bool up, const float* Wo,
                float* wot, float* dA, int64_t N, int T, int H, int relu, const float* Uc = nullptr ,
                float* dbias = nullptr, float* dbias2 = nullptr );
bool bptt_sums_bias(int cell, int H);
}

namespace gemm {
void run(hipStream_t s, const float* A, int64_t sAm, int64_t sAk, const float* B, int64_t sBk, int64_t sBn, float* C, int64_t ldc,
         int64_t M, int N, int64_t K, bool accumulate, const float* bias, int split_k, bool bf16 = false, bool untiled = false, DetScratch* det = nullptr);
constexpr int64_t DET_SLAB_FLOATS = (int64_t)1 << 24;
void run_untiled_slab(hipStream_t s, const float* A, int64_t sAm, int64_t sAk, const float* B, int64_t sBk, int64_t sBn, float* C, int64_t ldc, int64_t M, int N,
                      int64_t K, int64_t kchunk, int split_k, DetScratch* det);
bool run_tiled(hipStream_t s, const float* A, int64_t sAm, int64_t sAk, const float* B, int64_t sBk, int64_t sBn, float* C, int64_t ldc, int64_t M, int N,
               int64_t K, bool accumulate, const float* bias, int split_k, DetScratch* det = nullptr);
bool step_supported(const float* X, int64_t ldx, int Din, const float* Hprev, int64_t ldh, int H, const float* Wi, const float* Wo, int64_t N);
void lstm_step(hipStream_t s, const float* X, int64_t ldx, int Din, const float* Wi, const float* bi, const float* Hprev, const float* Wo,
               const float* Cprev, float* Cout, float* Hout, int64_t ldh, float* act, int64_t N, int H);
void rnn_step(hipStream_t s, const float* X, int64_t ldx, int Din, const float* Wi, const float* bi, const float* Hprev, const float* Wh,
              const float* bh, const float* mask, float* pre, float* Hout, int64_t ldh, int64_t N, int H, int relu);
}
```

### kprn_amd/csrc/lstm_fused_bwd.hip

```cpp
#include <string.h>

#include <memory>

#include "lstm_fused_common.h"

namespace fused {

struct BwdArgs {
  const int32_t* idx; int64_t N; int T, F, nT;
  const float *Wt, *We, *Wr; int dt, de, dr; int Vt, Vr;
  int L, layer;
  const float* WiT;
  const float* WoT;
  const float* save_frag;
  const float* dS;
  const float* wout_row;
  float* gWout_row; float* gbout_c;
  float* DX;
  float* DXe;
  int64_t Npad;
  float* gWi; float* gbi; float* gWo;
  float* gWt; float* gWe; float* gWr;
  float* part;
  unsigned long long* timing;
  int dbg;
  int64_t n_tiles;
  const int32_t* tile_k;
  float* PG;
  HoArgs ho;
  int small_lds;
  float* gG;
  unsigned* pipe_flag;
  int pipe;
};


constexpr int PART = 2 * 256 * 64 + 256;
constexpr int NS_ID = 16;
constexpr int PART_G = PART + 256 * NS_ID;
constexpr int LDD = 4 * DH + 4;
constexpr int DET_PG = 80, DET_SMALL = DET_PG + (KCAP + 1) * PFB, DET_STRIDE = DET_SMALL + 1024;

#ifdef KPRN_TIMING_PROBES
#define KPRN_PROBES_ON 1
#else
#define KPRN_PROBES_ON 0
#endif
#define TPROBE(slot)                                                                 \
  if (KPRN_PROBES_ON && a.timing) {                                                   \
    const unsigned long long now__ = __builtin_amdgcn_s_memtime();                    \
    tacc[slot] += now__ - tlast;                                                      \
    tlast = now__;                                                                    \
  }

struct Pre {
  f32x4 P[6];
  f32x4 up;
  f32x4 bin[4];
  f32x4 bhp[4];
};

__device__ __forceinline__ void gather_load_ident(const BwdArgs& a, const int t, const int32_t* ids, f32x4 (&v)[4]) {
  const int ch = threadIdx.x & 15, c0 = 4 * ch;
  const int32_t* p = ids + t * MT + (threadIdx.x >> 4);
  const float* eb = a.We - a.de + ((ch + 4) & 7) * 4;
#pragma unroll
  for (int k = 0; k < 4; ++k) {
    const f32x4 e = *(const f32x4*)(eb + (int64_t)p[IDS_PLANE<MT> + k * 16] * a.de);
    const int rel = p[2 * IDS_PLANE<MT> + k * 16] - 1, typ = a.Vr + p[k * 16] - 1;
    f32x4 oh;
#pragma unroll
    for (int i = 0; i < 4; ++i) oh[i] = (c0 + i == rel || c0 + i == typ) ? 1.f : 0.f;
    v[k] = (ch < 4) ? oh : ((ch < 12) ? e : f32x4{0.f, 0.f, 0.f, 0.f});
  }
}

template <bool BOTTOM, bool TOP, int NMT, bool IDENT = false, bool DET = false>
__device__ __forceinline__ void bwd_body(const BwdArgs& a, const int bx, const int G_, float* const det_part = nullptr) {
  static_assert(!IDENT || (BOTTOM && !TOP && NMT == 4), "the identity route: bottom layer of two, 64-path tiles");
  constexpr int MTR = 16 * NMT;
  constexpr int NXT = IDENT ? 3 : 4;
  extern __shared__ __attribute__((aligned(16))) float lds[];
  unsigned long long tacc[8] = {0, 0, 0, 0, 0, 0, 0, 0};
  unsigned long long tlast = (KPRN_PROBES_ON && a.timing) ? __builtin_amdgcn_s_memtime() : 0ull;
  float* dA_t = lds;
  float* in_t = dA_t + MT * LDD;
  int32_t* ids = (int32_t*)(in_t + (BOTTOM ? MT * LDA : 0));
  constexpr int IDS_BUF = MT * MAXT_LDS * 4;
  float* pg = (float*)(ids + (BOTTOM ? 2 * IDS_BUF : 0));

  const int tid = threadIdx.x;
  const int lane = tid & 63;
  const int j = __builtin_amdgcn_readfirstlane(tid >> 6);
  const int arow = lane & 15, ag = lane >> 4;
  const int T = a.T, L = a.L, ly = a.layer;
  const HoPlan ho = ho_plan(a.ho, a.tile_k, a.n_tiles, T, 1, bx, G_);
  auto mof = [&](const int i) -> int { return IDENT ? ((i + 2 * (j >> 1)) & 3) : i; };
  if (IDENT && bx == 0) for (int c = tid; c < 256 * NS_ID; c += 256) a.gG[c] = 0.f;

  f32x4 wiT[16], woT[16];
  {
    const float* wi_row = a.WiT + (int64_t)((IDENT ? a.dt + 16 * (j & 1) : j * 16) + arow) * (4 * DH) + ag * 4;
    const float* wo_row = a.WoT + (int64_t)(j * 16 + arow) * (4 * DH) + ag * 4;
#pragma unroll
    for (int S = 0; S < 16; ++S) { wiT[S] = *(const f32x4*)(wi_row + S * 16); woT[S] = *(const f32x4*)(wo_row + S * 16); }
#pragma unroll
    for (int S = 0; S < 16; ++S) { asm volatile("" : "+a"(wiT[S])); asm volatile("" : "+a"(woT[S])); }
  }
  f32x4 dwi[4][4], dwo[4][4];
  float dbias[4];
#pragma unroll
  for (int q = 0; q < 4; ++q) {
    dbias[q] = 0.f;
#pragma unroll
    for (int nt = 0; nt < 4; ++nt) {
      dwi[q][nt] = f32x4{0.f, 0.f, 0.f, 0.f}; dwo[q][nt] = f32x4{0.f, 0.f, 0.f, 0.f};
      if (nt < NXT) asm volatile("" : "+a"(dwi[q][nt]));
      asm volatile("" : "+a"(dwo[q][nt]));
    }
  }

  const int64_t frag_unit = (int64_t)NPL * 256;
  const int64_t frag_mt_stride = (int64_t)T * L * 4 * frag_unit;
  const int wcls = (j * 16 < a.dt) ? 0 : ((j * 16 < a.dt + a.de) ? 1 : 2);
  GatherSrc gsrc;
  if (BOTTOM) gsrc = gather_src(a);
  const float wout_c = TOP ? a.wout_row[j * 16 + arow] : 0.f;
  float gwo = 0.f, gbo = 0.f;
  for (int c = tid; c < (KCAP + 1) * PFB; c += 256) pg[c] = 0.f;
  f32x4 sacc[2] = {f32x4{0.f, 0.f, 0.f, 0.f}, f32x4{0.f, 0.f, 0.f, 0.f}};
  TPROBE(0)

  const int64_t n_mine = (a.n_tiles > (int64_t)bx) ? (a.n_tiles - 1 - bx) / G_ + 1 : 0;
  float* const ho_slot = a.ho.state + (int64_t)ho.slot * HO_STATE + threadIdx.x * 4;
  auto own_of = [&](const int64_t it) -> int64_t {
    const int64_t ti = TOP ? n_mine - 1 - it : ((ho.role == 1) ? (it + 1 < n_mine ? it + 1 : 0) : it);
    return (int64_t)bx + ti * G_;
  };
  int ipar = 1;
  int k0_req = 0;
  auto request_tile = [&](const int64_t tl, const int buf) {
    if (a.tile_k) k0_req = a.tile_k[tl];
    if (BOTTOM) ids_stage_dma<256, MTR>(a.idx, a.N, T, a.F, a.nT, tl, ids + buf * IDS_BUF);
  };
  if (n_mine > 0) request_tile(ho.role == 2 ? ho.tile : own_of(0), 0);
  for (int64_t it = 0; it < n_mine; ++it) {
    const int64_t own_tile = own_of(it);
    const bool late = ho.role == 1 && own_tile == (int64_t)bx;
    const bool early = ho.role == 2 && it == 0;
    int64_t tile, n0;
    int k0, Te;
    const float* frag_tile;
    float* dx_tile;
    auto retarget = [&](const int64_t tl) {
      tile = tl;
      n0 = tl * MTR;
      k0 = a.tile_k ? __builtin_amdgcn_readfirstlane(k0_req) : 0;
// ... 463 lines not shown
    f32x4 v[4];
#pragma unroll
    for (int k = 0; k < 4; ++k) v[k] = *(const f32x4*)(a.DX + (((tile * 4 + k) * T + t) * 4 + w0) * 256 + lane * 4);
    int my_ids[4] = {0, 0, 0, -1};
    if (tid < MT) {
      int64_t n = n0 + tid;
      const bool valid = n < a.N;
      if (!valid) n = a.N - 1;
      const int32_t* f = a.idx + (n * T + t) * a.F;
      my_ids[0] = f[a.F - a.nT - 2] - 1;
      my_ids[1] = f[a.F - 2] - 1;
      my_ids[2] = f[a.F - 1] - 1;
      my_ids[3] = valid ? tid : -1;
    }
    __syncthreads();
    if (tid < MT) {
#pragma unroll
      for (int k = 0; k < 4; ++k) ids[tid * 4 + k] = my_ids[k];
    }
#pragma unroll
    for (int k = 0; k < 4; ++k)
#pragma unroll
      for (int r = 0; r < 4; ++r) dxt[(k * 16 + ag * 4 + r) * LDA + w0 * 16 + arow] = v[k][r];
    __syncthreads();
    {
      int ld = -1;
      if (tid < MT && ids[tid * 4 + 3] >= 0) {
        const int e = ids[tid * 4 + 1];
        ld = tid;
        for (int r2 = tid - 1; r2 >= 0; --r2) if (ids[r2 * 4 + 1] == e) ld = r2;
      }
      __syncthreads();
      if (tid < MT) ids[tid * 4 + 3] = ld;
      __syncthreads();
    }
    if (col < D) {
      for (int k = 0; k < 16; ++k) {
        const int row = rg + 4 * k;
        const int ld = ids[row * 4 + 3];
        if (ld < 0) continue;
        const float val = dxt[row * LDA + col];
        if (col < e0) {
          if (!a.do_small) continue;
          const int32_t* f = a.idx + ((n0 + row) * T + t) * a.F;
          for (int kk = 0; kk < a.nT; ++kk) {
            const int rr = (kk == 0) ? ids[row * 4 + 0] : f[a.F - a.nT - 2 + kk] - 1;
            if (small_in_lds) lds_atomic_add(&small_g[rr * a.dt + col], val);
            else unsafeAtomicAdd(a.gWt + (int64_t)rr * a.dt + col, val);
          }
        } else if (col < e1) {
          if (a.do_entity && ld != row) lds_atomic_add(&dxt[ld * LDA + col], val);
        } else {
          if (!a.do_small) continue;
          const int rr = ids[row * 4 + 2];
          if (small_in_lds) lds_atomic_add(&small_g[a.Vt * a.dt + rr * a.dr + (col - e1)], val);
          else unsafeAtomicAdd(a.gWr + (int64_t)rr * a.dr + (col - e1), val);
        }
      }
    }
    __syncthreads();
    if (col >= e0 && col < e1 && a.do_entity) {
      for (int k = 0; k < 16; ++k) {
        const int row = rg + 4 * k;
        if (ids[row * 4 + 3] == row) unsafeAtomicAdd(a.gWe + (int64_t)ids[row * 4 + 1] * a.de + (col - e0), dxt[row * LDA + col]);
      }
    }
  }
  if (small_in_lds) {
    __syncthreads();
    for (int i = tid; i < n_small; i += 256) a.part_small[(int64_t)blockIdx.x * n_small + i] = small_g[i];
  }
}

__global__ __launch_bounds__(256) void k_reduce_small(const float* __restrict__ part, int nslab, int n_small, int nt_small, float* __restrict__ gWt, float* __restrict__ gWr) {
  __shared__ float red[16][17];
  const int e = threadIdx.x & 15, sl = threadIdx.x >> 4;
  const int i = blockIdx.x * 16 + e;
  float acc = 0.f;
  if (i < n_small) for (int s = sl; s < nslab; s += 16) acc += part[(int64_t)s * n_small + i];
  red[sl][e] = acc;
  __syncthreads();
  if (sl == 0 && i < n_small) {
    float v = 0.f;
#pragma unroll
    for (int k = 0; k < 16; ++k) v += red[k][e];
    if (i < nt_small) unsafeAtomicAdd(gWt + i, v); else unsafeAtomicAdd(gWr + (i - nt_small), v);
  }
}

__global__ void k_reduce_partials(bidx::SlabReduce a) { bidx::slab_reduce_block(a, blockIdx.x, blockIdx.y, blockIdx.z); }

struct TransArgs { const float* W[4]; float* WT[4]; };
__global__ void k_transpose_256x64(TransArgs a) {
  const int i = blockIdx.x * blockDim.x + threadIdx.x;
  if (i >= 64 * 256) return;
  const int n = i >> 8, k = i & 255;
  a.WT[blockIdx.y][i] = a.W[blockIdx.y][k * 64 + n];
}

bool transpose_job(kprn_handle* h, kk::TransposeJob* tj) {
  State* s = st(h);
  if (!s->wt_dirty) return false;
  const int L = h->cfg.L;
  if (!s->WT) HIP_TRY(kprn_dev_malloc((void**)&s->WT, (size_t)2 * 2 * 64 * 256 * sizeof(float)));
  tj->n = 2 * L;
  for (int m = 0; m < 4; ++m) {
    const int l = (m >> 1) < L ? (m >> 1) : 0;
    tj->W[m] = h->dense + ((m & 1) ? h->layer[l].Wo : h->layer[l].Wi);
    tj->WT[m] = s->WT + (size_t)(l * 2 + (m & 1)) * 64 * 256;
  }
  s->wt_dirty = false;
  return true;
}

bool bwd_supported(const kprn_handle* h, int T) { return fwd_supported(h, T); }

template <bool BOTTOM, bool TOP, int NMT = 4, bool IDENT = false>
static void launch_bwd(kprn_handle* h, const BwdArgs& a, int grid, float* det_part = nullptr) {
  size_t lds_bytes = (size_t)MT * LDD * sizeof(float);
  if (BOTTOM) lds_bytes += (size_t)MT * LDA * sizeof(float) + 2 * (MT * MAXT_LDS * 4) * sizeof(int32_t);
  lds_bytes += (size_t)(KCAP + 1) * PFB * sizeof(float);
  if (det_part) {
    if constexpr (BOTTOM || TOP) {
      static PerDeviceOnce det_attr_done;
      if (det_attr_done.need())
        HIP_TRY(hipFuncSetAttribute((const void*)k_lstm_bwd_det<BOTTOM, TOP, NMT, IDENT>, hipFuncAttributeMaxDynamicSharedMemorySize, (int)lds_bytes));
      hipLaunchKernelGGL((k_lstm_bwd_det<BOTTOM, TOP, NMT, IDENT>), dim3(grid), dim3(256), lds_bytes, h->stream, a, det_part);
      HIP_TRY(hipGetLastError());
      return;
    }
    throw KprnError{KPRN_E_UNSUPPORTED, "deterministic: the fused path has no middle layer"};
  }
  static PerDeviceOnce attr_done;
  const void* fn = IDENT ? (const void*)k_lstm_bwd_ident : (const void*)k_lstm_bwd<BOTTOM, TOP, NMT>;
  if (attr_done.need()) HIP_TRY(hipFuncSetAttribute(fn, hipFuncAttributeMaxDynamicSharedMemorySize, (int)lds_bytes));
  if constexpr (IDENT) hipLaunchKernelGGL(k_lstm_bwd_ident, dim3(grid), dim3(256), lds_bytes, h->stream, a);
  else hipLaunchKernelGGL((k_lstm_bwd<BOTTOM, TOP, NMT>), dim3(grid), dim3(256), lds_bytes, h->stream, a);
  HIP_TRY(hipGetLastError());
}

void backward(kprn_handle* h, const kprn_batch* b, int cid) {
  const kprn_config& c = h->cfg;
  State* s = st(h);
  const int64_t N = b->N;
  const int T = b->T, L = c.L;
  hipStream_t strm = h->stream;
  if (N > s->cap_Nb || T > s->cap_Tb) {
    HIP_TRY(hipStreamSynchronize(strm));
    if (s->DX) hipFree(s->DX);
    const int64_t cn = std::max<int64_t>(N, s->cap_Nb);
    const int ct = std::max(T, s->cap_Tb);
    HIP_TRY(kprn_dev_malloc((void**)&s->DX, (size_t)ct * (cn + 2 * MT) * DH * sizeof(float)));
    if (s->DXe) hipFree(s->DXe);
    HIP_TRY(kprn_dev_malloc((void**)&s->DXe, (size_t)(ct * (cn + 2 * MT) + KCAP) * c.de * sizeof(float)));
    s->cap_Nb = cn; s->cap_Tb = ct;
  }
  if (!s->part) HIP_TRY(kprn_dev_malloc((void**)&s->part, (size_t)2 * s->num_cu * PART_G * sizeof(float)));
  const bool det = h->deterministic;
  if (det && !s->det_part) HIP_TRY(kprn_dev_malloc((void**)&s->det_part, (size_t)2 * s->num_cu * DET_STRIDE * sizeof(float)));
  static const bool want_timing = KPRN_DEV_ENV("KPRN_TIMING") != nullptr;
  if (want_timing && !s->timing) HIP_TRY(kprn_dev_malloc((void**)&s->timing, (size_t)s->num_cu * 12 * sizeof(unsigned long long)));
  if (s->wt_dirty) {
    ProfScope ps(h, "weight_transpose");
    kk::TransposeJob tj;
    transpose_job(h, &tj);
    TransArgs ta;
    for (int m = 0; m < 4; ++m) { ta.W[m] = tj.W[m < tj.n ? m : 0]; ta.WT[m] = tj.WT[m < tj.n ? m : 0]; }
    hipLaunchKernelGGL(k_transpose_256x64, dim3(64, tj.n), dim3(256), 0, strm, ta);
    HIP_TRY(hipGetLastError());
  }
  float* gd = h->g_dense;
  const bool small = small_tiles(h, N, b->tile_k != nullptr);
  const int64_t n_tiles64 = (N + MT - 1) / MT;
  const int64_t n_tiles = small ? (N + 15) / 16 : n_tiles64;
  const int nmt = small ? 1 : 4;
  const int grid = (int)std::min<int64_t>(n_tiles, (int64_t)s->num_cu);
  bool have_r1 = false, reduced = false, ident = false;
  std::unique_ptr<ProfScope> bwd_scope;
  bidx::SlabReduce ra;
  BwdArgs pipe_top;
  for (int l = L - 1; l >= 0; --l) {
    BwdArgs a;
    a.pipe = 0; a.pipe_flag = nullptr;
    a.idx = b->idx_s ? b->idx_s : b->idx; a.N = N; a.T = T; a.F = b->F; a.nT = c.num_types;
    a.tile_k = b->tile_k; a.PG = s->PG + (size_t)l * (KCAP + 1) * PFB;
    a.Wt = h->dense + h->off_Wt; a.We = h->We; a.Wr = h->dense + h->off_Wr;
    a.dt = c.dt; a.de = c.de; a.dr = c.dr; a.Vt = c.Vt; a.Vr = c.Vr;
    a.L = L; a.layer = l;
    a.WiT = s->WT + (size_t)(l * 2 + 0) * 64 * 256; a.WoT = s->WT + (size_t)(l * 2 + 1) * 64 * 256;
    a.save_frag = s->save_frag; a.dS = h->ws.dS; a.wout_row = h->dense + h->off_outW + (int64_t)cid * DH; a.DX = s->DX;
    a.gWout_row = gd + h->off_outW + (int64_t)cid * DH; a.gbout_c = gd + h->off_outb + cid; a.Npad = n_tiles64 * MT;
    a.gWi = gd + h->layer[l].Wi; a.gbi = gd + h->layer[l].bi; a.gWo = gd + h->layer[l].Wo;
    a.gWt = gd + h->off_Wt; a.gWe = h->g_We; a.gWr = gd + h->off_Wr;
    a.n_tiles = n_tiles;
    a.part = s->part + (size_t)l * s->num_cu * PART_G; a.timing = s->timing;
    a.dbg = kprn_dbg_mask();
    float* const det_l = det ? s->det_part + (size_t)l * s->num_cu * DET_STRIDE : nullptr;
    a.ho = handover_args(h, grid);
    const bool bottom = (l == 0), top = (l == L - 1);
    const bool small_job = c.num_types == 1 && (c.dt % 16) == 0 && (c.de % 16) == 0 && (c.dr % 16) == 0 && c.Vt <= 16 && c.Vr <= 16 && !(a.dbg & 8);
    const bool have_index = b->key_sorted != nullptr && !(a.dbg & 16);
    s->DXe_on = have_index && !(a.dbg & 1);
    a.DXe = (bottom && s->DXe_on) ? s->DXe : nullptr;
    ident = bottom && !top && !small && small_job && have_index && !(a.dbg & 1) && h->small_tables && c.de == 32 && c.Vt + c.Vr <= NS_ID;
    if (ident && !s->gG) HIP_TRY(kprn_dev_malloc((void**)&s->gG, (size_t)256 * NS_ID * sizeof(float)));
    a.gG = ident ? s->gG : nullptr;
    const bool small_lds = bottom && small_job && have_index && !(a.dbg & 1) && h->fused_small_tables && !small && !ident;
    a.small_lds = small_lds ? 1 : 0;
    {
      if (top) { bwd_scope.reset(new ProfScope(h, "lstm_fused_bwd")); bwd_scope->launches = L; }
      const bool pipe = small && L == 2 && 2 * grid <= s->num_cu && h->bwd_pipe && !s->timing && a.ho.fault != nullptr;
      if (pipe && top) {
        if (!s->pipe_flag) {
          HIP_TRY(kprn_dev_malloc((void**)&s->pipe_flag, (size_t)s->num_cu * MAXT_LDS * sizeof(unsigned)));
          HIP_TRY(hipMemsetAsync(s->pipe_flag, 0, (size_t)s->num_cu * MAXT_LDS * sizeof(unsigned), strm));
        }
        a.pipe = 1; a.pipe_flag = s->pipe_flag;
        pipe_top = a;
        bwd_scope->launches = 1;
      } else if (pipe && bottom) {
        a.pipe = 2; a.pipe_flag = s->pipe_flag; a.ho = pipe_top.ho;
        size_t lds_bytes = (size_t)MT * LDD * sizeof(float) + (size_t)MT * LDA * sizeof(float) + 2 * (MT * MAXT_LDS * 4) * sizeof(int32_t) + (size_t)(KCAP + 1) * PFB * sizeof(float);
        if (det) {
          static PerDeviceOnce det_once;
          if (det_once.need()) HIP_TRY(hipFuncSetAttribute((const void*)k_lstm_bwd_dual_det<1>, hipFuncAttributeMaxDynamicSharedMemorySize, (int)lds_bytes));
          hipLaunchKernelGGL((k_lstm_bwd_dual_det<1>), dim3(2 * grid), dim3(256), lds_bytes, h->stream, pipe_top, a, grid,
                             s->det_part + (size_t)(L - 1) * s->num_cu * DET_STRIDE, det_l);
        } else {
          static PerDeviceOnce once;
          if (once.need()) HIP_TRY(hipFuncSetAttribute((const void*)k_lstm_bwd_dual<1>, hipFuncAttributeMaxDynamicSharedMemorySize, (int)lds_bytes));
          hipLaunchKernelGGL((k_lstm_bwd_dual<1>), dim3(2 * grid), dim3(256), lds_bytes, h->stream, pipe_top, a, grid);
        }
        HIP_TRY(hipGetLastError());
      } else
      if (small) { if (bottom) launch_bwd<true, false, 1>(h, a, grid, det_l); else launch_bwd<false, true, 1>(h, a, grid, det_l); }
      else if (bottom && top) launch_bwd<true, true>(h, a, grid, det_l);
      else if (bottom && ident) launch_bwd<true, false, 4, true>(h, a, grid, det_l);
      else if (bottom) launch_bwd<true, false>(h, a, grid, det_l);
      else if (top) launch_bwd<false, true>(h, a, grid, det_l);
      else launch_bwd<false, false>(h, a, grid, det_l);
      if (bottom || s->timing) bwd_scope.reset();
      if (bottom && det) {
        ProfScope ps(h, "det_join");
        DetJoin dj;
        memset(&dj, 0, sizeof(dj));
        dj.nslab = grid;
        int nb = 0;
        auto span = [&](float* dst, const float* src, int n) {
          if (n <= 0) return;
          dj.dst[dj.nseg] = dst; dj.src[dj.nseg] = src; dj.n[dj.nseg] = n; dj.blk0[dj.nseg] = nb;
          nb += (n + 255) / 256; ++dj.nseg; dj.blk0[dj.nseg] = nb;
        };
        const float* dtop = s->det_part + (size_t)(L - 1) * s->num_cu * DET_STRIDE;
        span(a.gWout_row, dtop, DH);
        span(a.gbout_c, dtop + DH, 1);
        if (b->tile_k) for (int ll = 0; ll < L; ++ll)
          span(s->PG + (size_t)ll * (KCAP + 1) * PFB + PFB, s->det_part + (size_t)ll * s->num_cu * DET_STRIDE + DET_PG + PFB, KCAP * PFB);
        if (a.small_lds) { span(a.gWt, det_l + DET_SMALL, c.Vt * c.dt); span(a.gWr, det_l + DET_SMALL + c.Vt * c.dt, c.Vr * c.dr); }
        hipLaunchKernelGGL(k_det_join, dim3(nb), dim3(256), 0, strm, dj);
        HIP_TRY(hipGetLastError());
      }
      if (bottom && h->after_bptt_hook) h->after_bptt_hook(h);
    }
    if (bottom) have_r1 = prefix_backward(h, b, n_tiles64);
    if (bottom) {
      for (int q = 0; q < 2; ++q) {
        const int ll = q < L ? q : 0;
        ra.part[q] = s->part + (size_t)ll * s->num_cu * PART_G;
        ra.gWi[q] = gd + h->layer[ll].Wi; ra.gWo[q] = gd + h->layer[ll].Wo; ra.gbi[q] = gd + h->layer[ll].bi;
      }
      ra.nslab = grid; ra.n_elem = ident ? PART_G : PART; ra.slab = PART_G; ra.L = L; ra.ny = det ? 1 : 16;
      ra.gG[0] = ident ? s->gG : nullptr; ra.gG[1] = nullptr;
      ra.r1 = s->r1; ra.kmax = have_r1 ? b->h_kmax : 0; ra.kcap = KCAP; ra.r1_stride = R1; ra.G = 4; ra.H = DH;
    }
    if (bottom && have_index && !(a.dbg & 1)) {
      ProfScope ps(h, "entity_grad+dw_reduce");
      bidx::SmallGrad sg;
      sg.DX = s->DX; sg.idx = b->idx_s ? b->idx_s : b->idx; sg.tile_k = b->tile_k; sg.N = N; sg.n_mtiles = n_tiles * nmt; sg.T = T; sg.F = b->F;
      sg.nT = c.num_types; sg.dt = c.dt; sg.de = c.de; sg.dr = c.dr; sg.Vt = c.Vt; sg.Vr = c.Vr; sg.gWt = a.gWt; sg.gWr = a.gWr; sg.nblocks = 4 * s->num_cu;
      { static const int sgb = KPRN_DEV_ENV("KPRN_SG_BLOCKS") ? atoi(KPRN_DEV_ENV("KPRN_SG_BLOCKS")) : 0; if (sgb > 0) sg.nblocks = sgb; }
      const bool sg_on = small_job && !a.small_lds && !ident;
      if (det) {
        const int ncb = (c.dt + c.dr) >> 4;
        sg.nblocks = ncb * (int)std::min<int64_t>(64, std::max<int64_t>(1, (sg.n_mtiles * T + 15) / 16));
        const int64_t need_seg = (b->n_index + 63) / 64 * 2 * c.de, need_sg = (int64_t)sg.nblocks * 256;
        if (need_seg > s->det_seg_cap || need_sg > s->det_sg_cap) {
          HIP_TRY(hipStreamSynchronize(strm));
          if (need_seg > s->det_seg_cap) { if (s->det_seg) hipFree(s->det_seg); HIP_TRY(kprn_dev_malloc((void**)&s->det_seg, (size_t)need_seg * sizeof(float))); s->det_seg_cap = need_seg; }
          if (need_sg > s->det_sg_cap) { if (s->det_sg) hipFree(s->det_sg); HIP_TRY(kprn_dev_malloc((void**)&s->det_sg, (size_t)need_sg * sizeof(float))); s->det_sg_cap = need_sg; }
        }
      }
      const bidx::DetEntity de_{s->det_seg, s->det_sg};
      bidx::entity_grad(strm, s->DXe, 2, b->key_sorted, b->pos_sorted, b->n_index, N, T, DH, c.dt, c.de, c.Ve, a.gWe, &ra,
                        sg_on ? &sg : nullptr, det ? &de_ : nullptr);
      if (det) bidx::entity_grad_tail(strm, b->key_sorted, b->n_index, c.de, c.Ve, a.gWe, de_, sg_on ? &sg : nullptr);
      reduced = true;
    }
    const bool small_in_kernel = small_job && have_index;
    if (bottom && !(a.dbg & 1) && (!small_in_kernel || !have_index)) {
      ProfScope ps(h, "embed_scatter");
      ScatArgs sa;
      sa.idx = b->idx_s ? b->idx_s : b->idx; sa.tile_k = b->tile_k; sa.N = N; sa.T = T; sa.F = b->F; sa.nT = c.num_types;
      sa.dt = c.dt; sa.de = c.de; sa.dr = c.dr; sa.Vt = c.Vt; sa.Vr = c.Vr;
      sa.DX = s->DX; sa.gWt = a.gWt; sa.gWe = a.gWe; sa.gWr = a.gWr; sa.n_tiles = n_tiles64;
      sa.do_small = small_in_kernel ? 0 : 1; sa.do_entity = have_index ? 0 : 1;
      const int n_small = c.Vt * c.dt + c.Vr * c.dr;
      const bool small_fits = n_small <= 4096;
      const size_t lds_b = (size_t)MT * LDA * sizeof(float) + MT * 4 * sizeof(int32_t) + (size_t)(small_fits ? n_small : 0) * sizeof(float);
      const int sgrid = (int)std::min<int64_t>(n_tiles64 * T, (int64_t)s->num_cu * 8);
      const bool slabs = small_fits && sa.do_small;
      if (slabs && (!s->part_small || s->part_small_n < n_small)) {
        HIP_TRY(hipStreamSynchronize(strm));
        if (s->part_small) hipFree(s->part_small);
        HIP_TRY(kprn_dev_malloc((void**)&s->part_small, (size_t)s->num_cu * 8 * n_small * sizeof(float)));
        s->part_small_n = n_small;
      }
      sa.part_small = small_fits ? s->part_small : nullptr;
      hipLaunchKernelGGL(k_embed_scatter_frag, dim3(sgrid), dim3(256), lds_b, strm, sa);
      if (slabs) hipLaunchKernelGGL(k_reduce_small, dim3((n_small + 15) / 16), dim3(256), 0, strm, s->part_small, sgrid, n_small, c.Vt * c.dt, sa.gWt, sa.gWr);
      HIP_TRY(hipGetLastError());
    }
    if (s->timing) {
      HIP_TRY(hipStreamSynchronize(strm));
      std::vector<unsigned long long> tb((size_t)grid * 8);
      HIP_TRY(hipMemcpy(tb.data(), s->timing, tb.size() * sizeof(unsigned long long), hipMemcpyDeviceToHost));
      double sum[8] = {0};
      for (int g = 0; g < grid; ++g) for (int k = 0; k < 8; ++k) sum[k] += (double)tb[(size_t)g * 8 + k];
      {
        double tmax = 0, th = 0, tl = 0; int nh = 0, nl = 0, imax = 0;
        for (int g = 0; g < grid; ++g) {
          double tot = 0; for (int k = 0; k < 8; ++k) tot += (double)tb[(size_t)g * 8 + k];
          if (tot > tmax) { tmax = tot; imax = g; }
          if (g < 21) { th += tot; ++nh; } else { tl += tot; ++nl; }
        }
        if (getenv("KPRN_TIMING_DUMP")) {
          fprintf(stderr, "[kprn timing dump] bwd layer %d:", l);
          for (int g = 0; g < grid; ++g) { double tot = 0; for (int k = 0; k < 8; ++k) tot += (double)tb[(size_t)g * 8 + k]; fprintf(stderr, " %.0f", tot / 1000.0); }
          fprintf(stderr, "\n");
        }
        fprintf(stderr, "[kprn timing] bwd layer %d per-WG total: max %.0f (WG %d) mean of WG 0..20 %.0f, of the others %.0f; tile-prologue of WG 0: %.0f, WG 100: %.0f\n", l, tmax, imax,
                th / (nh ? nh : 1), tl / (nl ? nl : 1), (double)tb[1], grid > 100 ? (double)tb[100 * 8 + 1] : 0.0);
      }
      fprintf(stderr, "[kprn timing] bwd layer %d N=%lld grid=%d avg cycles/WG: prologue %.0f tile-prologue %.0f stageC-valu %.0f stageC-mfma %.0f midbar %.0f stageE %.0f endbar %.0f flush %.0f\n",
              l, (long long)N, grid, sum[0] / grid, sum[1] / grid, sum[7] / grid, sum[2] / grid, sum[3] / grid, sum[4] / grid, sum[5] / grid, sum[6] / grid);
    }
  }
  if (!reduced) {
    ProfScope ps(h, "dw_reduce");
    hipLaunchKernelGGL(k_reduce_partials, dim3((ra.n_elem + 255) / 256, ra.ny, L), dim3(256), 0, strm, ra);
    HIP_TRY(hipGetLastError());
  }
  if (ident) {
    ProfScope ps(h, "small_tables_finish");
    kk::small_tables_finish(strm, s->gG, NS_ID, 4 * DH, DH, c.dt, c.de, c.dr, c.Vt, c.Vr, h->dense + h->off_Wt, h->dense + h->off_Wr, h->dense + h->layer[0].Wi,
                            gd + h->layer[0].Wi, gd + h->off_Wt, gd + h->off_Wr, false);
  }
}

void params_changed(kprn_handle* h) {
  if (!h->fused_state) return;
  State* s = (State*)h->fused_state;
  s->wt_dirty = true;
  s->pf_batch = -1;
  s->mc_dirty = true;
}

void release(kprn_handle* h) {
  State* s = (State*)h->fused_state;
  if (!s) return;
  for (float* p : {s->det_part, s->det_seg, s->det_sg}) if (p) hipFree(p);
  for (float* p : {s->save_frag, s->WT, s->DX, s->DXe, s->part, s->gG, s->part_small, s->pfb, s->pfs, s->pfx, s->PG, s->r1, s->mc_bias, s->mc_hseq[0], s->mc_hseq[1],
                   s->ho_state[0], s->ho_state[1]}) if (p) hipFree(p);
  for (unsigned* p : {s->ho_flag[0], s->ho_flag[1], s->pipe_flag}) if (p) hipFree(p);
  if (s->mc_wsp) hipFree(s->mc_wsp);
  if (s->timing) hipFree(s->timing);
  delete s;
  h->fused_state = nullptr;
}

}
```

### kprn_amd/csrc/lstm_fused_common.h

```cpp
#pragma once
#include <stdio.h>
#include <stdlib.h>

#include <algorithm>
#include <type_traits>

#include "kprn_internal.h"

namespace fused {

typedef float f32x4 __attribute__((ext_vector_type(4)));

constexpr int DH = 64;
constexpr int MT = 64;
constexpr int LDA = DH + 4;

struct HoArgs {
  float* state = nullptr;
  unsigned* flag = nullptr;
  unsigned epoch = 0;
  int mode = 1;
  int* fault = nullptr;
};

// ... 151 lines not shown
}

constexpr int IDENT_DE = 32, IDENT_NS = 16;
template <int MTR> struct IdentGather { f32x4 e[MTR == 64 ? 2 : 1]; int rel, typ; };
template <int NTHREADS, int MTR, class Args>
__device__ __forceinline__ void gather_load_ident_fwd(const Args& a, int t, const int32_t* ids, IdentGather<MTR>& g) {
  static_assert(NTHREADS == 256 && (MTR == 64 || MTR == 16), "3 pieces per thread of a 64-row tile, at most one of a 16-row tile");
  const int tid = threadIdx.x;
  const float* eb = a.We - IDENT_DE + (tid & 7) * 4;
  const int32_t* p = ids + t * MTR;
  if constexpr (MTR == 64) {
#pragma unroll
    for (int k = 0; k < 2; ++k) g.e[k] = *(const f32x4*)(eb + (int64_t)p[IDS_PLANE<MTR> + (tid >> 3) + 32 * k] * IDENT_DE);
    g.rel = p[2 * IDS_PLANE<MTR> + (tid >> 2)] - 1;
    g.typ = a.Vr + p[tid >> 2] - 1;
  } else {
    g.e[0] = *(const f32x4*)(eb + (int64_t)p[IDS_PLANE<MTR> + ((tid >> 3) & 15)] * IDENT_DE);
    g.rel = p[2 * IDS_PLANE<MTR> + ((tid >> 2) & 15)] - 1;
    g.typ = a.Vr + p[(tid >> 2) & 15] - 1;
  }
}
template <int NTHREADS, int MTR>
__device__ __forceinline__ void gather_store_ident_fwd(float* xbuf, const IdentGather<MTR>& g) {
  const int tid = threadIdx.x, c0 = 4 * (tid & 3);
  f32x4 oh;
#pragma unroll
  for (int i = 0; i < 4; ++i) oh[i] = (c0 + i == g.rel || c0 + i == g.typ) ? 1.f : 0.f;
  if constexpr (MTR == 64) {
    *(f32x4*)(xbuf + (tid >> 2) * LDA + c0) = oh;
#pragma unroll
    for (int k = 0; k < 2; ++k) *(f32x4*)(xbuf + ((tid >> 3) + 32 * k) * LDA + IDENT_NS + (tid & 7) * 4) = g.e[k];
  } else {
    const bool ent = tid < 128;
    const int off = ent ? (tid >> 3) * LDA + IDENT_NS + (tid & 7) * 4 : ((tid >> 2) - 32) * LDA + c0;
    *(f32x4*)(xbuf + off) = ent ? g.e[0] : oh;
  }
}

constexpr int NPL = 7;
typedef __attribute__((address_space(1))) char gchar;
typedef __attribute__((address_space(1))) f32x4 gf32x4;
__device__ __forceinline__ gchar* uniform_global(const void* p) {
  const uint64_t v = (uint64_t)(size_t)p;
  const uint32_t lo = (uint32_t)__builtin_amdgcn_readfirstlane((int)(uint32_t)v), hi = (uint32_t)__builtin_amdgcn_readfirstlane((int)(uint32_t)(v >> 32));
  return (gchar*)(((uint64_t)hi << 32) | lo);
}

#define KPRN_MFMA(ACC, A_, B_) asm volatile("v_mfma_f32_16x16x4_f32 %0, %1, %2, %0" : "+v"(ACC) : "v"(A_), "a"(B_))
#define KPRN_MFMA_C(ACC, A_, B_, C_) asm volatile("v_mfma_f32_16x16x4_f32 %0, %1, %2, %3" : "=&v"(ACC) : "v"(A_), "a"(B_), "v"(C_))
#define KPRN_MFMA_Z(ACC, A_, B_) asm volatile("v_mfma_f32_16x16x4_f32 %0, %1, %2, 0" : "=&v"(ACC) : "v"(A_), "a"(B_))
#define KPRN_MFMA_ACC_A(ACC, A_, B_) asm volatile("v_mfma_f32_16x16x4_f32 %0, %1, %2, %0" : "+a"(ACC) : "v"(A_), "v"(B_))
#define KPRN_MFMA_VV(ACC, A_, B_) asm volatile("s_nop 1\n\tv_mfma_f32_16x16x4_f32 %0, %1, %2, %0" : "+v"(ACC) : "v"(A_), "v"(B_))
#define KPRN_MFMA_VVZ(ACC, A_, B_) asm volatile("s_nop 1\n\tv_mfma_f32_16x16x4_f32 %0, %1, %2, 0" : "=&v"(ACC) : "v"(A_), "v"(B_))
#define KPRN_MFMA_VA_Z(ACC, A_, B_) asm volatile("s_nop 1\n\tv_mfma_f32_16x16x4_f32 %0, %1, %2, 0" : "=&v"(ACC) : "v"(A_), "a"(B_))
#define KPRN_MFMA_VA(ACC, A_, B_) asm volatile("s_nop 1\n\tv_mfma_f32_16x16x4_f32 %0, %1, %2, %0" : "+v"(ACC) : "v"(A_), "a"(B_))
#define KPRN_MFMA_DRAIN() asm volatile("s_nop 15\n\ts_nop 15" ::: "memory")
#define KPRN_PIN_V4(A) asm volatile("" : "+v"((A)[0]), "+v"((A)[1]), "+v"((A)[2]), "+v"((A)[3]))
#define KPRN_PIN_V2(X, Y) asm volatile("" : "+v"(X), "+v"(Y))
#define KPRN_PIN_A8(A, B) \
  asm volatile("" : "+a"((A)[0]), "+a"((A)[1]), "+a"((A)[2]), "+a"((A)[3]), "+a"((B)[0]), "+a"((B)[1]), "+a"((B)[2]), "+a"((B)[3]))

constexpr int HO_STATE = 4 * MT * DH;
struct HoPlan { int role; int d; int64_t tile; int slot; };
constexpr long long HO_TIMEOUT_TICKS = 200000000ll;

__host__ __device__ __forceinline__ int ho_partner(int mode, int G, int bx) {
  const int half = G >> 1;
  return (mode == 2) ? (bx < half ? bx + half : (bx - half < half ? bx - half : bx)) : G - 1 - bx;
}
__host__ __device__ __forceinline__ HoPlan ho_decide(int bx, int px, int mine, int theirs, int steps, int keep, int64_t heavy_tiles) {
  HoPlan p{0, 0, -1, 0};
  const int diff = mine > theirs ? mine - theirs : theirs - mine;
  if (px == bx || diff < 4 || heavy_tiles < 2) return p;
  p.role = mine > theirs ? 1 : 2;
  p.tile = mine > theirs ? bx : px;
  p.slot = (int)p.tile;
  int d = diff >> 2;
  if (2 * (d + 1) - diff < -2 * d) ++d;
  p.d = d < steps - keep ? d : steps - keep;
  if (p.d < 1) p.role = 0;
  return p;
}
template <class K0>
inline HoPlan ho_plan_host(bool on, int mode, int G, int bx, int64_t n_tiles, int T, K0 tile_k0, int* load, int keep = 1) {
  const int px = ho_partner(mode, G, bx);
  int mine = 0, theirs = 0;
  for (int64_t t = bx; t < n_tiles; t += G) mine += 2 * (T - tile_k0(t)) - 1;
  for (int64_t t = px; t < n_tiles; t += G) theirs += 2 * (T - tile_k0(t)) - 1;
  if (load) *load = mine;
  if (!on || (n_tiles + G - 1) / G > 32) return HoPlan{0, 0, -1, 0};
  const int64_t heavy = mine > theirs ? bx : px;
  return ho_decide(bx, px, mine, theirs, T - tile_k0(heavy), keep, (n_tiles - 1 - heavy) / G + 1);
}
__device__ __forceinline__ HoPlan ho_plan(const HoArgs& ho, const int32_t* tile_k, int64_t n_tiles, int T, int keep, const int bx, const int G) {
  const int px = ho_partner(ho.mode, G, bx);
  if (!ho.epoch || px == bx || (n_tiles + G - 1) / G > 32) return HoPlan{0, 0, -1, 0};
  const int lane = threadIdx.x & 63, i = lane & 31;
  const int64_t t = (int64_t)(lane < 32 ? bx : px) + (int64_t)i * G;
  const int k = (tile_k && t < n_tiles) ? tile_k[t] : 0;
  int cost = t < n_tiles ? 2 * (T - k) - 1 : 0;
#pragma unroll
  for (int sh = 1; sh < 32; sh <<= 1) cost += __shfl_xor(cost, sh, 64);
  const int mine = __builtin_amdgcn_readlane(cost, 0), theirs = __builtin_amdgcn_readlane(cost, 32);
  const int k_mine = __builtin_amdgcn_readlane(k, 0), k_theirs = __builtin_amdgcn_readlane(k, 32);
  return ho_decide(bx, px, mine, theirs, T - (mine > theirs ? k_mine : k_theirs), keep, (n_tiles - 1 - (mine > theirs ? bx : px)) / G + 1);
}

__device__ __forceinline__ void ho_store4(float* p, const f32x4& v) {
  union { f32x4 f; unsigned long long u[2]; } c;
  c.f = v;
  __hip_atomic_store((unsigned long long*)p, c.u[0], __ATOMIC_RELAXED, __HIP_MEMORY_SCOPE_AGENT);
  __hip_atomic_store((unsigned long long*)p + 1, c.u[1], __ATOMIC_RELAXED, __HIP_MEMORY_SCOPE_AGENT);
}
__device__ __forceinline__ f32x4 ho_load4(const float* p) {
  union { f32x4 f; unsigned long long u[2]; } c;
  c.u[0] = __hip_atomic_load((const unsigned long long*)p, __ATOMIC_RELAXED, __HIP_MEMORY_SCOPE_AGENT);
  c.u[1] = __hip_atomic_load((const unsigned long long*)p + 1, __ATOMIC_RELAXED, __HIP_MEMORY_SCOPE_AGENT);
  return c.f;
}
__device__ __forceinline__ void ho_store1(float* p, float v) { __hip_atomic_store(p, v, __ATOMIC_RELAXED, __HIP_MEMORY_SCOPE_AGENT); }
__device__ __forceinline__ float ho_load1(const float* p) { return __hip_atomic_load(p, __ATOMIC_RELAXED, __HIP_MEMORY_SCOPE_AGENT); }
__device__ __forceinline__ void ho_publish(const HoArgs& ho, int slot) {
  asm volatile("s_waitcnt vmcnt(0)" ::: "memory");
  __syncthreads();
  if (threadIdx.x == 0) __hip_atomic_store(ho.flag + slot, ho.epoch, __ATOMIC_RELAXED, __HIP_MEMORY_SCOPE_AGENT);
}
__device__ __forceinline__ void ho_wait(const HoArgs& ho, int slot) {
  const long long t0 = wall_clock64();
  while (__hip_atomic_load(ho.flag + slot, __ATOMIC_RELAXED, __HIP_MEMORY_SCOPE_AGENT) != ho.epoch) {
    __builtin_amdgcn_s_sleep(16);
    if (wall_clock64() - t0 > HO_TIMEOUT_TICKS) {
      if (threadIdx.x == 0) __hip_atomic_store(ho.fault, 1, __ATOMIC_RELAXED, __HIP_MEMORY_SCOPE_SYSTEM);
      break;
    }
  }
  asm volatile("" ::: "memory");
}

struct State {
  float* save_frag = nullptr;
  unsigned* pipe_flag = nullptr;
  int64_t cap_N = 0;
  int cap_T = 0;
  int num_cu = 0;
  float* WT = nullptr;
  bool wt_dirty = true;
  float* DX = nullptr;
  float* DXe = nullptr;
  bool DXe_on = false;
  float* pfb = nullptr;
  float* pfs = nullptr;
  float* pfx = nullptr;
  float* PG = nullptr;
  float* r1 = nullptr;
  void* mc_wsp = nullptr; float* mc_bias = nullptr; bool mc_dirty = true; int mc_ns = 0;
  float* mc_hseq[2] = {nullptr, nullptr}; int64_t mc_capN[2] = {0, 0}; int mc_capT[2] = {0, 0};
  int64_t pf_batch = -1;

  float* part = nullptr;
  float* gG = nullptr;
  float* ho_state[2] = {nullptr, nullptr}; unsigned* ho_flag[2] = {nullptr, nullptr};
  unsigned ho_epoch = 0;
  float* part_small = nullptr;
  int part_small_n = 0;
  unsigned long long* timing = nullptr;
  int64_t cap_Nb = 0; int cap_Tb = 0;
  float* det_part = nullptr;
  float* det_seg = nullptr; int64_t det_seg_cap = 0;
  float* det_sg = nullptr; int64_t det_sg_cap = 0;
};

static inline State* st(kprn_handle* h) {
  if (!h->fused_state) {
    State* s = new State();
    hipDeviceProp_t p;
    if (hipGetDeviceProperties(&p, h->cfg.device_id) == hipSuccess) s->num_cu = p.multiProcessorCount;
    if (s->num_cu <= 0) s->num_cu = 256;
    h->fused_state = s;
  }
  return (State*)h->fused_state;
}

constexpr int64_t SMALL_TILES_MAX_PATHS = 8192;
HoArgs handover_args(kprn_handle* h, int grid);

}
```

### kprn_amd/csrc/lstm_fused_prefix.hip

```cpp
#include "lstm_fused_common.h"
#include "adam_rows_dev.h"

namespace fused {

struct PrefFwdArgs {
  int kmax;
  int32_t ref[16];
  int F, nT;
  const float *Wt, *We, *Wr;
  int dt, de, dr;
  const float* Wi[2];
  const float* bi[2];
  const float* Wo[2];
  float* pfb;
  float* pfs;
  float* pfx;
};

constexpr int LDW = DH + 4;
__device__ __forceinline__ float row_dot(const f32x4 (&w)[16], const float* v) {
  float acc0 = 0.f, acc1 = 0.f;
#pragma unroll
  for (int i = 0; i < 16; ++i) {
    acc0 += w[i][0] * v[4 * i] + w[i][2] * v[4 * i + 2];
    acc1 += w[i][1] * v[4 * i + 1] + w[i][3] * v[4 * i + 3];
  }
  return acc0 + acc1;
}
__device__ __forceinline__ void rows_request(const float* __restrict__ W, f32x4 (&st)[16]) {
#pragma unroll
  for (int i = 0; i < 16; ++i) st[i] = *(const f32x4*)(W + (int64_t)(i * 256 + threadIdx.x) * 4);
}
__device__ __forceinline__ void rows_land(const f32x4 (&st)[16], float* tile, f32x4 (&row)[16]) {
#pragma unroll
  for (int half = 0; half < 2; ++half) {
    __syncthreads();
#pragma unroll
    for (int i = 0; i < 8; ++i) {
      const int e = (i * 256 + threadIdx.x) * 4;
      *(f32x4*)(tile + (e >> 6) * LDW + (e & 63)) = st[half * 8 + i];
    }
    __syncthreads();
    if ((int)(threadIdx.x >> 7) == half) {
#pragma unroll
      for (int i = 0; i < 16; ++i) row[i] = *(const f32x4*)(tile + (threadIdx.x & 127) * LDW + 4 * i);
    }
  }
}

template <int L>
__device__ __forceinline__ void prefix_fwd_block(const PrefFwdArgs& a) {
  __shared__ float x[DH], hcur[DH], cst[DH], gates[4 * DH], hhist[KCAP][DH];
  __shared__ __attribute__((aligned(16))) float wtile[128 * LDW];
  const int r = threadIdx.x;
  const int kmax = a.kmax;
  if (r < DH) {
    const int32_t* ids = a.ref;
    float v = 0.f;
    if (r < a.dt) {
      for (int q = 0; q < a.nT; ++q) v += a.Wt[(int64_t)(ids[a.F - a.nT - 2 + q] - 1) * a.dt + r];
    } else if (r < a.dt + a.de) {
      v = a.We[(int64_t)(ids[a.F - 2] - 1) * a.de + (r - a.dt)];
    } else {
      v = a.Wr[(int64_t)(ids[a.F - 1] - 1) * a.dr + (r - a.dt - a.de)];
    }
    x[r] = v;
    a.pfx[r] = v;
  }
#pragma unroll
  for (int l = 0; l < L; ++l) {
    f32x4 wi[16], wo[16];
    const float bias = a.bi[l][r];
    {
      f32x4 sa[16], sb[16];
      rows_request(a.Wi[l], sa);
      rows_request(a.Wo[l], sb);
      rows_land(sa, wtile, wi);
      rows_land(sb, wtile, wo);
    }
    if (r < DH) { hcur[r] = 0.f; cst[r] = 0.f; }
    __syncthreads();
    float rec = 0.f;
    for (int t = 0; t < kmax; ++t) {
      const float* in = (l == 0) ? x : hhist[t];
      gates[r] = (bias + rec) + row_dot(wi, in);
      __syncthreads();
      if (r < DH) {
        const float gi = fast_sigmoid(gates[r]), gg = fast_tanh(gates[DH + r]), gf = fast_sigmoid(gates[2 * DH + r]), go = fast_sigmoid(gates[3 * DH + r]);
        const float cp = cst[r];
        const float cn = gf * cp + gi * gg;
        const float tc = fast_tanh(cn);
        const float hh = go * tc;
        float* sv = a.pfs + (int64_t)(t * L + l) * NPL * DH + r;
        sv[0 * DH] = gi * gg * (1.0f - gi);
        sv[1 * DH] = gi * (1.0f - gg * gg);
        sv[2 * DH] = cp * gf * (1.0f - gf);
        sv[3 * DH] = hh * (1.0f - go);
        sv[4 * DH] = go * (1.0f - tc * tc);
        sv[5 * DH] = gf;
        sv[6 * DH] = hh;
        cst[r] = cn;
        hcur[r] = hh;
      }
      __syncthreads();
      const float rr = row_dot(wo, hcur);
      rec = rr;
      a.pfb[((t + 1) * L + l) * PFB + r] = rr;
      if (r < DH) { a.pfb[((t + 1) * L + l) * PFB + 4 * DH + r] = cst[r]; if (l + 1 < L) hhist[t][r] = hcur[r]; }
      __syncthreads();
    }
  }
}

template <int L>
__global__ __launch_bounds__(256) void k_prefix_fwd(PrefFwdArgs a) { prefix_fwd_block<L>(a); }

template <int G, int L>
__global__ __launch_bounds__(256, 2) void k_catchup_prefix(kk_dev::AdamRowsArgs ra, PrefFwdArgs pa) {
  if (blockIdx.x == 0) { prefix_fwd_block<L>(pa); return; }
  kk_dev::adam_rows_lane_block<G>(ra, (int64_t)blockIdx.x - 1);
}

struct PrefBwdArgs {
  int kmax;
  int32_t ref[16];
  int F, nT, L, T;
  int dt, de, dr;
  const float* Wi[2];
  const float* Wo[2];
  const float* pfs;
  const float* pfx;
  float* PG;
  float* r1;
  float *gWt, *gWe, *gWr;
  float* DXv;
  float* DXe_v;
  int entity_direct;
};

__device__ __forceinline__ float col_dot(const float (&w)[64], const float* v256, float (*red)[DH]) {
  const int c = threadIdx.x & 63, part = threadIdx.x >> 6;
  float acc0 = 0.f, acc1 = 0.f;
#pragma unroll
  for (int i = 0; i < 64; i += 2) { acc0 += w[i] * v256[part * 64 + i]; acc1 += w[i + 1] * v256[part * 64 + i + 1]; }
  red[part][c] = acc0 + acc1;
  __syncthreads();
  return (red[0][c] + red[1][c]) + (red[2][c] + red[3][c]);
}

__global__ __launch_bounds__(256) void k_prefix_bwd(PrefBwdArgs a) {
  __shared__ float dAn[4 * DH], dAg[4 * DH], up[KCAP][DH], red[4][DH], red2[4][DH];
  const int r = threadIdx.x;
  const int c = r & 63, part = r >> 6;
  const int L = a.L;
  const int kmax = a.kmax;
  const int32_t* ids = a.ref;
  for (int l = L - 1; l >= 0; --l) {
    float wi[64], wo[64];
#pragma unroll
    for (int i = 0; i < 64; ++i) {
      wi[i] = a.Wi[l][(int64_t)(part * 64 + i) * DH + c];
      wo[i] = a.Wo[l][(int64_t)(part * 64 + i) * DH + c];
    }
    float dA_next = 0.f;
    float dc_next = 0.f;
    for (int t = kmax - 1; t >= 0; --t) {
      float* pg = a.PG + ((int64_t)l * (KCAP + 1) + (t + 1)) * PFB;
      float* r1 = a.r1 + ((int64_t)l * KCAP + t) * R1;
      const float v = dA_next + pg[r];
      pg[r] = 0.f;
      dAn[r] = v;
      r1[r] = v;
      float pgc = 0.f;
      if (r < DH) {
        r1[2 * 4 * DH + r] = a.pfs[((int64_t)(t * L + l) * NPL + 6) * DH + r];
        r1[2 * 4 * DH + DH + r] = (l == 0) ? a.pfx[r] : a.pfs[((int64_t)(t * L + l - 1) * NPL + 6) * DH + r];
        pgc = pg[4 * DH + r];
        pg[4 * DH + r] = 0.f;
      }
      __syncthreads();
      const float dh = col_dot(wo, dAn, red);
      if (r < DH) {
        const float dc = dc_next + pgc;
        const float dhv = dh + ((l < L - 1) ? up[t][r] : 0.f);
        const float* P = a.pfs + (int64_t)(t * L + l) * NPL * DH + r;
        const float dC = dc + dhv * P[4 * DH];
        dAg[r] = dC * P[0 * DH];
        dAg[DH + r] = dC * P[1 * DH];
        dAg[2 * DH + r] = dC * P[2 * DH];
        dAg[3 * DH + r] = dhv * P[3 * DH];
        dc_next = dC * P[5 * DH];
      }
      __syncthreads();
      dA_next = dAg[r];
      r1[4 * DH + r] = dA_next;
      const float dx = col_dot(wi, dAg, red2);
      if (r < DH) {
        if (l > 0) {
          up[t][r] = dx;
        } else {
          a.DXv[((int64_t)t * 4 + (r >> 4)) * 256 + (r & 15) * 4] = dx;
          if (a.DXe_v && r >= a.dt && r < a.dt + a.de) a.DXe_v[(int64_t)t * a.de + (r - a.dt)] = dx;
          if (r < a.dt) {
            for (int q = 0; q < a.nT; ++q) unsafeAtomicAdd(a.gWt + (int64_t)(ids[a.F - a.nT - 2 + q] - 1) * a.dt + r, dx);
          } else if (r < a.dt + a.de) {
            if (a.entity_direct) unsafeAtomicAdd(a.gWe + (int64_t)(ids[a.F - 2] - 1) * a.de + (r - a.dt), dx);
          } else {
            unsafeAtomicAdd(a.gWr + (int64_t)(ids[a.F - 1] - 1) * a.dr + (r - a.dt - a.de), dx);
          }
        }
      }
      __syncthreads();
    }
  }
}

static void ensure_prefix_buffers(State* s, hipStream_t stream) {
  if (s->pfb) return;
  HIP_TRY(kprn_dev_malloc((void**)&s->pfb, (size_t)(KCAP + 1) * 2 * PFB * sizeof(float)));
  HIP_TRY(kprn_dev_malloc((void**)&s->pfs, (size_t)KCAP * 2 * NPL * DH * sizeof(float)));
  HIP_TRY(kprn_dev_malloc((void**)&s->pfx, (size_t)DH * sizeof(float)));
  HIP_TRY(kprn_dev_malloc((void**)&s->PG, (size_t)2 * (KCAP + 1) * PFB * sizeof(float)));
  HIP_TRY(kprn_dev_malloc((void**)&s->r1, (size_t)2 * KCAP * R1 * sizeof(float)));
  HIP_TRY(hipMemsetAsync(s->PG, 0, (size_t)2 * (KCAP + 1) * PFB * sizeof(float), stream));
  HIP_TRY(hipMemsetAsync(s->pfb, 0, (size_t)(KCAP + 1) * 2 * PFB * sizeof(float), stream));
}

static void prefix_fwd_args(kprn_handle* h, const kprn_batch* b, State* s, PrefFwdArgs& a) {
  const kprn_config& c = h->cfg;
  a.kmax = b->h_kmax;
  for (int q = 0; q < 16; ++q) a.ref[q] = b->h_ref[q];
  a.F = b->F; a.nT = c.num_types;
  a.Wt = h->dense + h->off_Wt; a.We = h->We; a.Wr = h->dense + h->off_Wr;
  a.dt = c.dt; a.de = c.de; a.dr = c.dr;
  for (int l = 0; l < 2; ++l) {
    const int ll = l < c.L ? l : 0;
    a.Wi[l] = h->dense + h->layer[ll].Wi; a.bi[l] = h->dense + h->layer[ll].bi; a.Wo[l] = h->dense + h->layer[ll].Wo;
  }
  a.pfb = s->pfb; a.pfs = s->pfs; a.pfx = s->pfx;
}

bool catch_up_with_prefix(kprn_handle* h, const kprn_batch* b, float* W, float* g, float* m, float* v, int32_t* last, int32_t t_now, const float* step_tab,
                          float b1, float b2, float eps) {
  State* s = st(h);
  const kprn_config& c = h->cfg;
  if (!h->catchup_prefix || !b->tile_k || b->h_kmax == 0 || b->n_uniq <= 0) return false;
  if (!(c.de == 32 || c.de == 64 || c.de == 128) || (((uintptr_t)W | (uintptr_t)m | (uintptr_t)v) & 15)) return false;
  if (b->h_ref[b->F - 2] != c.Ve) return false;
  ensure_prefix_buffers(s, h->stream);
  if (s->pf_batch == b->serial) return false;
  PrefFwdArgs pa;
  prefix_fwd_args(h, b, s, pa);
  kk_dev::AdamRowsArgs ra{W, g, m, v, last, b->uniq, b->uniq + b->uniq_cap, t_now, 0, step_tab, b1, b2, eps, (int64_t)c.Ve - 1, -1.f};
  const int G = c.de / 4;
  const unsigned nb = (unsigned)(((int64_t)b->n_uniq * G + 255) / 256) + 1;
#define KPRN_CP(G_) \
  { if (c.L == 1) hipLaunchKernelGGL((k_catchup_prefix<G_, 1>), dim3(nb), dim3(256), 0, h->stream, ra, pa); \
    else hipLaunchKernelGGL((k_catchup_prefix<G_, 2>), dim3(nb), dim3(256), 0, h->stream, ra, pa); }
  if (G == 8) KPRN_CP(8) else if (G == 16) KPRN_CP(16) else KPRN_CP(32)
#undef KPRN_CP
  HIP_TRY(hipGetLastError());
  s->pf_batch = b->serial;
  return true;
}

void prefix_forward(kprn_handle* h, const kprn_batch* b) {
  State* s = st(h);
  ensure_prefix_buffers(s, h->stream);
  if (s->pf_batch == b->serial) return;
  const kprn_config& c = h->cfg;
  PrefFwdArgs a;
  if (!b->tile_k || b->h_kmax == 0) { s->pf_batch = b->serial; return; }
  join_score(h);
  prefix_fwd_args(h, b, s, a);
  ProfScope ps(h, "prefix_fwd");
  if (c.L == 1) hipLaunchKernelGGL(k_prefix_fwd<1>, dim3(1), dim3(256), 0, h->stream, a);
  else hipLaunchKernelGGL(k_prefix_fwd<2>, dim3(1), dim3(256), 0, h->stream, a);
  HIP_TRY(hipGetLastError());
  s->pf_batch = b->serial;
}

bool prefix_backward(kprn_handle* h, const kprn_batch* b, int64_t n_tiles) {
  State* s = st(h);
  const kprn_config& c = h->cfg;
  if (!b->tile_k || b->h_kmax == 0) return false;
  PrefBwdArgs a;
  a.kmax = b->h_kmax;
  for (int q = 0; q < 16; ++q) a.ref[q] = b->h_ref[q];
  a.F = b->F; a.nT = c.num_types; a.L = c.L; a.T = b->T;
  a.dt = c.dt; a.de = c.de; a.dr = c.dr;
  float* gd = h->g_dense;
  for (int l = 0; l < 2; ++l) {
    const int ll = l < c.L ? l : 0;
    a.Wi[l] = h->dense + h->layer[ll].Wi; a.Wo[l] = h->dense + h->layer[ll].Wo;
  }
  a.pfs = s->pfs; a.pfx = s->pfx; a.PG = s->PG; a.r1 = s->r1;
  a.gWt = gd + h->off_Wt; a.gWe = h->g_We; a.gWr = gd + h->off_Wr;
  a.DXv = s->DX + (size_t)n_tiles * 4 * b->T * 4 * 256;
  a.DXe_v = s->DXe_on ? s->DXe + (size_t)n_tiles * MT * b->T * c.de : nullptr;
  a.entity_direct = (kprn_dbg_mask() & 16) ? 1 : 0;
  ProfScope ps(h, "prefix_bwd");
  hipLaunchKernelGGL(k_prefix_bwd, dim3(1), dim3(256), 0, h->stream, a);
  HIP_TRY(hipGetLastError());
  return true;
}

}
```

Baseline: 50.95 million.

## Run prefix backward walk beside entity-grad and fold its terms into finish

```diff
diff --git a/kprn_amd/csrc/batch_index.hip b/kprn_amd/csrc/batch_index.hip
--- a/kprn_amd/csrc/batch_index.hip
+++ b/kprn_amd/csrc/batch_index.hip
@@ -7,6 +7,7 @@
 #include <algorithm>
 
 #include "kprn_internal.h"
+#include "prefix_bwd_dev.h"
 
 namespace bidx {
 
@@ -153,10 +154,17 @@
 __device__ __forceinline__ void entity_grad_body(const float* __restrict__ DX, const int32_t* __restrict__ key_sorted,
                                                  const int32_t* __restrict__ pos_sorted, int64_t nsteps, int64_t N, int T, int D, int dt, int de,
                                                  int sentinel, float* __restrict__ gWe, int n_ent_blocks, int n_red_blocks, const SlabReduce red,
-                                                 const SmallGrad sg, const int dbg, float* const det_seg, float* const det_sg) {
+                                                 const SmallGrad sg, const int dbg, float* const det_seg, float* const det_sg, const fused::PrefBwdArgs& pb) {
+  __shared__ float pass_lds[4 * 16 * 16];
+  const int first = pb.kmax > 0 ? 1 : 0;
+  if (first && blockIdx.x == 0) {
+    fused::prefix_bwd_walk<true>(pb, pass_lds, pass_lds + 4 * fused::DH, (float (*)[fused::DH])pb.up, (float (*)[fused::DH])(pass_lds + 8 * fused::DH),
+                                 (float (*)[fused::DH])(pass_lds + 8 * fused::DH));
+    return;
+  }
   const int order = (dbg >> 4) & 3;
-  const int n_pass = gridDim.x - n_ent_blocks;
-  int bid = blockIdx.x, rb = -1;
+  const int n_pass = (int)gridDim.x - first - n_ent_blocks;
+  int bid = (int)blockIdx.x - first, rb = -1;
   if (order == 1) { if (bid < n_pass) { rb = bid; } else bid -= n_pass; }
   else if (order == 2) {
     const int both = 2 * (n_pass < n_ent_blocks ? n_pass : n_ent_blocks);
@@ -167,8 +175,8 @@
   if (rb >= 0) {
     if (dbg & 2) return;
     if (rb >= n_red_blocks) {
-      if constexpr (DET) small_grad_block<true>(sg, rb - n_red_blocks, det_sg);
-      else if (!(dbg & 8)) small_grad_block(sg, rb - n_red_blocks);
+      if constexpr (DET) small_grad_block<true>(sg, rb - n_red_blocks, (float (*)[16][16])pass_lds, det_sg);
+      else if (!(dbg & 8)) small_grad_block(sg, rb - n_red_blocks, (float (*)[16][16])pass_lds);
       return;
     }
     if (dbg & 4) return;
@@ -186,7 +194,8 @@
   const int kb_ld = key_sorted[base > 0 ? base - 1 : 0], ka_ld = key_sorted[base + cnt < nsteps ? base + cnt : nsteps - 1];
   const int my_key = (lane < cnt) ? key_ld : -1;
   if (__builtin_amdgcn_readlane(my_key, 0) == sentinel) return;
-  const int my_pos = (lane < cnt) ? pos_ld : 0;
+  const int pos_real = pos_ld >= pb.virt0 ? pb.zero_pos : pos_ld;
+  const int my_pos = (lane < cnt) ? pos_real : 0;
   const int key_before = (base > 0) ? kb_ld : -1;
   const int key_after = (base + cnt < nsteps) ? ka_ld : -1;
   const int waves_per_group = D >> 4;
@@ -245,18 +254,18 @@
 __global__ __launch_bounds__(256) void k_entity_grad(const float* __restrict__ DX, const int32_t* __restrict__ key_sorted,
                                                      const int32_t* __restrict__ pos_sorted, int64_t nsteps, int64_t N, int T, int D, int dt, int de,
                                                      int sentinel, float* __restrict__ gWe, int n_ent_blocks, int n_red_blocks, SlabReduce red,
-                                                     SmallGrad sg, int dbg) {
-  entity_grad_body<FRAG, false>(DX, key_sorted, pos_sorted, nsteps, N, T, D, dt, de, sentinel, gWe, n_ent_blocks, n_red_blocks, red, sg, dbg, nullptr, nullptr);
+                                                     SmallGrad sg, int dbg, fused::PrefBwdArgs pb) {
+  entity_grad_body<FRAG, false>(DX, key_sorted, pos_sorted, nsteps, N, T, D, dt, de, sentinel, gWe, n_ent_blocks, n_red_blocks, red, sg, dbg, nullptr, nullptr, pb);
 }
 __global__ __launch_bounds__(256) void k_egrad_det(const float* __restrict__ DX, const int32_t* __restrict__ key_sorted, const int32_t* __restrict__ pos_sorted,
                                                    int64_t nsteps, int64_t N, int T, int D, int dt, int de, int sentinel, float* __restrict__ gWe,
-                                                   int n_ent_blocks, int n_red_blocks, SlabReduce red, SmallGrad sg, DetEntity det) {
-  entity_grad_body<2, true>(DX, key_sorted, pos_sorted, nsteps, N, T, D, dt, de, sentinel, gWe, n_ent_blocks, n_red_blocks, red, sg, 0, det.seg_part, det.sg_part);
+                                                   int n_ent_blocks, int n_red_blocks, SlabReduce red, SmallGrad sg, DetEntity det, fused::PrefBwdArgs pb) {
+  entity_grad_body<2, true>(DX, key_sorted, pos_sorted, nsteps, N, T, D, dt, de, sentinel, gWe, n_ent_blocks, n_red_blocks, red, sg, 0, det.seg_part, det.sg_part, pb);
 }
 __global__ __launch_bounds__(256) void k_egrad_det_rowmajor(const float* __restrict__ DX, const int32_t* __restrict__ key_sorted, const int32_t* __restrict__ pos_sorted,
                                                             int64_t nsteps, int64_t N, int T, int D, int dt, int de, int sentinel, float* __restrict__ gWe,
-                                                            int n_ent_blocks, int n_red_blocks, SlabReduce red, SmallGrad sg, DetEntity det) {
-  entity_grad_body<0, true>(DX, key_sorted, pos_sorted, nsteps, N, T, D, dt, de, sentinel, gWe, n_ent_blocks, n_red_blocks, red, sg, 0, det.seg_part, det.sg_part);
+                                                            int n_ent_blocks, int n_red_blocks, SlabReduce red, SmallGrad sg, DetEntity det, fused::PrefBwdArgs pb) {
+  entity_grad_body<0, true>(DX, key_sorted, pos_sorted, nsteps, N, T, D, dt, de, sentinel, gWe, n_ent_blocks, n_red_blocks, red, sg, 0, det.seg_part, det.sg_part, pb);
 }
 
 __global__ __launch_bounds__(256) void k_det_tail(const int32_t* __restrict__ key_sorted, int64_t nsteps, int de, int sentinel, float* __restrict__ gWe,
@@ -329,8 +338,16 @@
 }
 
 void entity_grad(hipStream_t s, const float* DX, int frag_order, const int32_t* key_sorted, const int32_t* pos_sorted, int64_t n_index, int64_t N,
-                 int T, int D, int dt, int de, int Ve, float* gWe, const SlabReduce* red, const SmallGrad* sg, const DetEntity* det) {
+                 int T, int D, int dt, int de, int Ve, float* gWe, const SlabReduce* red, const SmallGrad* sg, const DetEntity* det, const fused::PrefBwdArgs* prefix) {
   if (n_index <= 0 && !red && !sg) return;
+  fused::PrefBwdArgs pb;
+  memset(&pb, 0, sizeof(pb));
+  pb.virt0 = INT32_MAX;
+  if (prefix && prefix->kmax > 0) {
+    KPRN_REQUIRE(frag_order == 2 && prefix->virt0 > 0 && prefix->dx0 && prefix->up, KPRN_E_UNSUPPORTED, "prefix passenger: the compact entity slice only");
+    pb = *prefix;
+  }
+  const int first = pb.kmax > 0 ? 1 : 0;
   const int64_t segs = (n_index + 63) / 64;
   const int n_ent = (int)((segs + 3) / 4);
   SlabReduce r;
@@ -341,18 +358,18 @@
   if (red) { r = *red; n_red = ((r.n_elem + 255) / 256) * r.ny * r.L; }
   if (sg) { g = *sg; n_sg = g.nblocks; }
   static const int dbg = KPRN_DEV_ENV("KPRN_EGRAD_DBG") ? atoi(KPRN_DEV_ENV("KPRN_EGRAD_DBG")) : 0;
-  const dim3 grid((unsigned)(n_ent + n_red + n_sg));
+  const dim3 grid((unsigned)(first + n_ent + n_red + n_sg));
   if (det) {
     KPRN_REQUIRE(frag_order == 2 || (frag_order == 0 && !red && !sg), KPRN_E_UNSUPPORTED,
                  "deterministic entity gradient: the compact entity slice, or row-major dx without passenger jobs");
     if (frag_order == 0)
-      hipLaunchKernelGGL(k_egrad_det_rowmajor, grid, dim3(256), 0, s, DX, key_sorted, pos_sorted, n_index, N, T, D, dt, de, Ve, gWe, n_ent, n_red, r, g, *det);
+      hipLaunchKernelGGL(k_egrad_det_rowmajor, grid, dim3(256), 0, s, DX, key_sorted, pos_sorted, n_index, N, T, D, dt, de, Ve, gWe, n_ent, n_red, r, g, *det, pb);
     else
-    hipLaunchKernelGGL(k_egrad_det, grid, dim3(256), 0, s, DX, key_sorted, pos_sorted, n_index, N, T, D, dt, de, Ve, gWe, n_ent, n_red, r, g, *det);
+    hipLaunchKernelGGL(k_egrad_det, grid, dim3(256), 0, s, DX, key_sorted, pos_sorted, n_index, N, T, D, dt, de, Ve, gWe, n_ent, n_red, r, g, *det, pb);
   } else
-  if (frag_order == 1) hipLaunchKernelGGL(k_entity_grad<1>, grid, dim3(256), 0, s, DX, key_sorted, pos_sorted, n_index, N, T, D, dt, de, Ve, gWe, n_ent, n_red, r, g, dbg);
-  else if (frag_order == 2) hipLaunchKernelGGL(k_entity_grad<2>, grid, dim3(256), 0, s, DX, key_sorted, pos_sorted, n_index, N, T, D, dt, de, Ve, gWe, n_ent, n_red, r, g, dbg);
-  else hipLaunchKernelGGL(k_entity_grad<0>, grid, dim3(256), 0, s, DX, key_sorted, pos_sorted, n_index, N, T, D, dt, de, Ve, gWe, n_ent, n_red, r, g, dbg);
+  if (frag_order == 1) hipLaunchKernelGGL(k_entity_grad<1>, grid, dim3(256), 0, s, DX, key_sorted, pos_sorted, n_index, N, T, D, dt, de, Ve, gWe, n_ent, n_red, r, g, dbg, pb);
+  else if (frag_order == 2) hipLaunchKernelGGL(k_entity_grad<2>, grid, dim3(256), 0, s, DX, key_sorted, pos_sorted, n_index, N, T, D, dt, de, Ve, gWe, n_ent, n_red, r, g, dbg, pb);
+  else hipLaunchKernelGGL(k_entity_grad<0>, grid, dim3(256), 0, s, DX, key_sorted, pos_sorted, n_index, N, T, D, dt, de, Ve, gWe, n_ent, n_red, r, g, dbg, pb);
   HIP_TRY(hipGetLastError());
 }
 }
diff --git a/kprn_amd/csrc/kernels_basic.hip b/kprn_amd/csrc/kernels_basic.hip
--- a/kprn_amd/csrc/kernels_basic.hip
+++ b/kprn_amd/csrc/kernels_basic.hip
@@ -1495,9 +1495,11 @@
 }
 __global__ __launch_bounds__(256) void k_small_tables_finish_f32(const float* __restrict__ Ct, int ns, int GH, int Din, int dt, int de, int dr, int Vt, int Vr,
                                                                  const float* __restrict__ Wt, const float* __restrict__ Wr, const float* __restrict__ Wi,
-                                                                 float* __restrict__ gWi, float* __restrict__ gWt, float* __restrict__ gWr, int with_e) {
+                                                                 float* __restrict__ gWi, float* __restrict__ gWt, float* __restrict__ gWr, int with_e,
+                                                                 const bidx::PrefixApply pa) {
   __shared__ float g[128];
   const int tid = threadIdx.x, NZ = ns + (with_e ? de : 0);
+  if ((int)blockIdx.x >= GH + Vr + Vt) { bidx::prefix_apply_block(pa, (int)blockIdx.x - (GH + Vr + Vt), 3); return; }
   if ((int)blockIdx.x < GH) {
     const int k = blockIdx.x;
     const float* row = Ct + (int64_t)k * NZ;
@@ -1508,12 +1510,13 @@
       if (j < dt) {
         for (int y = 0; y < Vt; ++y) v += g[Vr + y] * Wt[y * dt + j];
       } else if (j < dt + de) {
-        if (!with_e) continue;
-        v = row[ns + j - dt];
+        if (!with_e && pa.kmax == 0) continue;
+        if (with_e) v = row[ns + j - dt];
       } else {
         const int jj = j - dt - de;
         for (int r = 0; r < Vr; ++r) v += g[r] * Wr[r * dr + jj];
       }
+      if (pa.kmax > 0) v += bidx::prefix_rank1(pa, 0, k * Din + j);
       gWi[(int64_t)k * Din + j] += v;
     }
     return;
@@ -1534,15 +1537,25 @@
       float v = 0.f;
 #pragma unroll
       for (int q = 0; q < 16; ++q) v += red[q * 16 + j];
+      if (pa.kmax > 0) {
+        const int hits = rel ? (pa.ref[pa.F - 1] - 1 == r ? 1 : 0) : bidx::prefix_type_hits(pa, r - Vr);
+        if (hits > 0) { const float pv = bidx::prefix_dx_sum(pa, col0 + jj); for (int q = 0; q < hits; ++q) v += pv; }
+      }
       (rel ? gWr + (int64_t)r * dr : gWt + (int64_t)(r - Vr) * dt)[jj] += v;
     }
     __syncthreads();
   }
 }
 void small_tables_finish(hipStream_t s, const float* Ct, int ns, int GH, int Din, int dt, int de, int dr, int Vt, int Vr, const float* Wt, const float* Wr,
-                         const float* Wi, float* gWi, float* gWt, float* gWr, bool ct_has_entity) {
-  hipLaunchKernelGGL(k_small_tables_finish_f32, dim3((unsigned)(GH + Vr + Vt)), dim3(256), 0, s, Ct, ns, GH, Din, dt, de, dr, Vt, Vr, Wt, Wr, Wi, gWi, gWt, gWr,
-                     ct_has_entity ? 1 : 0);
+                         const float* Wi, float* gWi, float* gWt, float* gWr, bool ct_has_entity, const bidx::PrefixApply* prefix) {
+  bidx::PrefixApply pa;
+  memset(&pa, 0, sizeof(pa));
+  if (prefix) {
+    pa = *prefix;
+    KPRN_REQUIRE(pa.G * pa.H == GH && pa.H == Din && pa.dt == dt && pa.de == de && pa.dr == dr, KPRN_E_ARG, "prefix apply job: not this finish launch's layer shape");
+  }
+  hipLaunchKernelGGL(k_small_tables_finish_f32, dim3((unsigned)(GH + Vr + Vt + bidx::prefix_apply_blocks(pa))), dim3(256), 0, s, Ct, ns, GH, Din, dt, de, dr, Vt, Vr, Wt,
+                     Wr, Wi, gWi, gWt, gWr, ct_has_entity ? 1 : 0, pa);
   HIP_TRY(hipGetLastError());
 }
 
diff --git a/kprn_amd/csrc/kprn_api.hip b/kprn_amd/csrc/kprn_api.hip
--- a/kprn_amd/csrc/kprn_api.hip
+++ b/kprn_amd/csrc/kprn_api.hip
@@ -1822,6 +1822,8 @@
     h->score_dual = v;
   } else if (strcmp(key, "catchup_prefix") == 0) {
     h->catchup_prefix = atoi(value) != 0;
+  } else if (strcmp(key, "prefix_beside") == 0) {
+    h->prefix_beside = atoi(value) != 0;
   } else if (strcmp(key, "fused_small_tables") == 0) {
     h->fused_small_tables = atoi(value) != 0;
   } else if (strcmp(key, "persist_layers") == 0) {
diff --git a/kprn_amd/csrc/kprn_internal.h b/kprn_amd/csrc/kprn_internal.h
--- a/kprn_amd/csrc/kprn_internal.h
+++ b/kprn_amd/csrc/kprn_internal.h
@@ -66,7 +66,7 @@
 
 struct DetScratch { float* p = nullptr; int64_t cap = 0; };
 
-namespace fused { constexpr int KCAP = 8; }
+namespace fused { constexpr int KCAP = 8; struct PrefBwdArgs; }
 
 struct kprn_graph;
 struct kprn_sampler;
@@ -209,6 +209,7 @@
   bool adam_merged = true;
   bool bwd_pipe = true;
   int score_dual = 2;
+  bool prefix_beside = true;
   bool catchup_prefix = true;
   bool fused_small_tables = true;
   float score_split = 0.f;
@@ -307,6 +308,7 @@
 void scratch_reserve(void** scratch, size_t* bytes, size_t need);
 }
 
+namespace bidx { struct PrefixApply; }
 namespace kk {
 void validate_indices(hipStream_t s, const int32_t* idx, int64_t nsteps, int F, int nT, int Vt, int Ve, int Vr, int32_t* flag);
 void embed_gather(hipStream_t s, const int32_t* idx, int64_t N, int T, int F, int nT, const float* Wt, const float* We,
@@ -358,7 +360,7 @@
 bool embed_scatter_det_ok(int dt, int dr, int Vt, int Vr);
 void onehot_cols(hipStream_t s, const int32_t* idx, int64_t N, int T, int F, int Vr, int Vt, float* X, int64_t ldx, int col0, int ns);
 void small_tables_finish(hipStream_t s, const float* Ct, int ns, int GH, int Din, int dt, int de, int dr, int Vt, int Vr, const float* Wt, const float* Wr,
-                         const float* Wi, float* gWi, float* gWt, float* gWr, bool ct_has_entity = true);
+                         const float* Wi, float* gWi, float* gWt, float* gWr, bool ct_has_entity = true, const bidx::PrefixApply* prefix = nullptr);
 void sumsq(hipStream_t s, const float* x, int64_t n, float* out);
 void sumsq_rows(hipStream_t s, const float* G, const int32_t* rows, const int32_t* count, int d, float* out);
 constexpr int SUMSQ_DET_BLOCKS = 512;
@@ -466,13 +468,75 @@
   else if (i < nB) unsafeAtomicAdd(a.gbi[l] + (i - 2 * nW), v);
   else unsafeAtomicAdd(a.gG[l] + (i - nB), v);
 }
+struct PrefixApply {
+  int kmax;
+  int L, kcap, r1_stride, G, H;
+  const float* r1;
+  const float* hs;
+  const float* x0;
+  int64_t hs_stride;
+  const float* dx;
+  float* gWi[2]; float* gWo[2]; float* gbi[2];
+  float *gWt, *gWe, *gWr;
+  int dt, de, dr, nT, F;
+  int32_t ref[16];
+};
+__host__ __device__ __forceinline__ int prefix_apply_blocks(const PrefixApply& a) {
+  const int GH = a.G * a.H, nB = 2 * GH * a.H + GH;
+  return a.kmax > 0 ? a.L * ((nB + 255) / 256) + 1 : 0;
+}
+__device__ __forceinline__ float prefix_rank1(const PrefixApply& a, int l, int i) {
+  const int GH = a.G * a.H, nW = GH * a.H;
+  float v = 0.f;
+  for (int t = 0; t < a.kmax; ++t) {
+    const float* r1 = a.r1 + ((int64_t)l * a.kcap + t) * a.r1_stride;
+    if (i < nW) v += r1[GH + i / a.H] * (l == 0 ? a.x0[i % a.H] : a.hs[(int64_t)(t * a.L + l - 1) * a.hs_stride + i % a.H]);
+    else if (i < 2 * nW) v += r1[(i - nW) / a.H] * a.hs[(int64_t)(t * a.L + l) * a.hs_stride + (i - nW) % a.H];
+    else v += r1[GH + (i - 2 * nW)];
+  }
+  return v;
+}
+__device__ __forceinline__ float prefix_dx_sum(const PrefixApply& a, int j) {
+  float v = 0.f;
+  for (int t = 0; t < a.kmax; ++t) v += a.dx[t * a.H + j];
+  return v;
+}
+__device__ __forceinline__ int prefix_type_hits(const PrefixApply& a, int y) {
+  int n = 0;
+  for (int q = 0; q < a.nT; ++q) n += (a.ref[a.F - a.nT - 2 + q] - 1 == y) ? 1 : 0;
+  return n;
+}
+__device__ __forceinline__ void prefix_apply_block(const PrefixApply& a, int jb, int skip) {
+  const int GH = a.G * a.H, nW = GH * a.H, nB = 2 * nW + GH;
+  const int nbx = (nB + 255) / 256;
+  if (jb < a.L * nbx) {
+    const int l = jb / nbx, i = (jb - l * nbx) * 256 + (int)threadIdx.x;
+    if (i >= nB || (l == 0 && i < nW && (skip & 1))) return;
+    const float v = prefix_rank1(a, l, i);
+    if (i < nW) a.gWi[l][i] += v;
+    else if (i < 2 * nW) a.gWo[l][i - nW] += v;
+    else a.gbi[l][i - 2 * nW] += v;
+    return;
+  }
+  const int j = threadIdx.x;
+  if (j >= a.H) return;
+  const float v = prefix_dx_sum(a, j);
+  if (j < a.dt) {
+    if (!(skip & 2))
+      for (int q = 0; q < a.nT; ++q) a.gWt[(int64_t)(a.ref[a.F - a.nT - 2 + q] - 1) * a.dt + j] += v;
+  } else if (j < a.dt + a.de) {
+    a.gWe[(int64_t)(a.ref[a.F - 2] - 1) * a.de + (j - a.dt)] += v;
+  } else if (!(skip & 2)) {
+    a.gWr[(int64_t)(a.ref[a.F - 1] - 1) * a.dr + (j - a.dt - a.de)] += v;
+  }
+}
 struct SmallGrad {
   const float* DX; const int32_t* idx; const int32_t* tile_k;
   int64_t N, n_mtiles; int T, F, nT, dt, de, dr, Vt, Vr;
   float* gWt; float* gWr; int nblocks;
 };
 template <bool DET = false>
-__device__ __forceinline__ void small_grad_block(const SmallGrad& a, int bx, float* det_part = nullptr) {
+__device__ __forceinline__ void small_grad_block(const SmallGrad& a, int bx, float (*sg_red)[16][16] , float* det_part = nullptr) {
   typedef float f32x4_ __attribute__((ext_vector_type(4)));
   const int lane = threadIdx.x & 63, wv = threadIdx.x >> 6;
   const int arow = lane & 15, ag = lane >> 4;
@@ -520,7 +584,6 @@
         acc = __builtin_amdgcn_mfma_f32_16x16x4f32(onehot, xv, acc, 0, 0, 0);
       }
   }
-  __shared__ float sg_red[4][16][16];
 #pragma unroll
   for (int i = 0; i < 4; ++i) sg_red[wv][4 * ag + i][arow] = acc[i];
   __syncthreads();
@@ -539,7 +602,8 @@
   float* sg_part;
 };
 void entity_grad(hipStream_t s, const float* DX, int frag_order, const int32_t* key_sorted, const int32_t* pos_sorted, int64_t n_index, int64_t N,
-                 int T, int D, int dt, int de, int Ve, float* gWe, const SlabReduce* red = nullptr, const SmallGrad* sg = nullptr, const DetEntity* det = nullptr);
+                 int T, int D, int dt, int de, int Ve, float* gWe, const SlabReduce* red = nullptr, const SmallGrad* sg = nullptr, const DetEntity* det = nullptr,
+                 const fused::PrefBwdArgs* prefix = nullptr );
 void entity_grad_tail(hipStream_t s, const int32_t* key_sorted, int64_t n_index, int de, int Ve, float* gWe, const DetEntity& det, const SmallGrad* sg);
 size_t merge_scratch_bytes(int64_t n, int Ve);
 void merge_rows(hipStream_t s, const void* all, int world, int cap, int de, int Ve, float* G, int32_t* union_rows, int32_t* union_count,
@@ -575,6 +639,9 @@
 void mc_prepare(kprn_handle* h);
 void forward_mc(kprn_handle* h, const kprn_batch* b, bool save);
 bool prefix_backward(kprn_handle* h, const kprn_batch* b, int64_t n_tiles);
+bool prefix_beside_route(const kprn_handle* h, const kprn_batch* b, bool have_index);
+void prefix_beside_jobs(kprn_handle* h, const kprn_batch* b, int64_t n_tiles, PrefBwdArgs* pb, bidx::PrefixApply* pa);
+void prefix_apply_launch(kprn_handle* h, const bidx::PrefixApply& pa);
 void release(kprn_handle* h);
 void handover_stats(kprn_handle* h, const kprn_batch* b, int64_t* out );
 }
diff --git a/kprn_amd/csrc/lstm_fused_bwd.hip b/kprn_amd/csrc/lstm_fused_bwd.hip
--- a/kprn_amd/csrc/lstm_fused_bwd.hip
+++ b/kprn_amd/csrc/lstm_fused_bwd.hip
@@ -3,6 +3,7 @@
 #include <memory>
 
 #include "lstm_fused_common.h"
+#include "prefix_bwd_dev.h"
 
 namespace fused {
 
@@ -772,7 +773,10 @@
     const int ct = std::max(T, s->cap_Tb);
     HIP_TRY(kprn_dev_malloc((void**)&s->DX, (size_t)ct * (cn + 2 * MT) * DH * sizeof(float)));
     if (s->DXe) hipFree(s->DXe);
-    HIP_TRY(kprn_dev_malloc((void**)&s->DXe, (size_t)(ct * (cn + 2 * MT) + KCAP) * c.de * sizeof(float)));
+    HIP_TRY(kprn_dev_malloc((void**)&s->DXe, (size_t)(ct * (cn + 2 * MT) + KCAP + 1) * c.de * sizeof(float)));
+    s->dxe_zero_pos = (int64_t)ct * (cn + 2 * MT) + KCAP;
+    KPRN_REQUIRE(s->dxe_zero_pos <= INT32_MAX, KPRN_E_UNSUPPORTED, "fused backward: position index past 2^31");
+    HIP_TRY(hipMemsetAsync(s->DXe + (size_t)s->dxe_zero_pos * c.de, 0, (size_t)c.de * sizeof(float), strm));
     s->cap_Nb = cn; s->cap_Tb = ct;
   }
   if (!s->part) HIP_TRY(kprn_dev_malloc((void**)&s->part, (size_t)2 * s->num_cu * PART_G * sizeof(float)));
@@ -795,7 +799,9 @@
   const int64_t n_tiles = small ? (N + 15) / 16 : n_tiles64;
   const int nmt = small ? 1 : 4;
   const int grid = (int)std::min<int64_t>(n_tiles, (int64_t)s->num_cu);
-  bool have_r1 = false, reduced = false, ident = false;
+  bool have_r1 = false, reduced = false, ident = false, beside = false;
+  PrefBwdArgs pbw;
+  bidx::PrefixApply papply;
   std::unique_ptr<ProfScope> bwd_scope;
   bidx::SlabReduce ra;
   BwdArgs pipe_top;
@@ -882,7 +888,11 @@
       }
       if (bottom && h->after_bptt_hook) h->after_bptt_hook(h);
     }
-    if (bottom) have_r1 = prefix_backward(h, b, n_tiles64);
+    if (bottom) {
+      beside = prefix_beside_route(h, b, have_index);
+      if (beside) prefix_beside_jobs(h, b, n_tiles64, &pbw, &papply);
+      else have_r1 = prefix_backward(h, b, n_tiles64);
+    }
     if (bottom) {
       for (int q = 0; q < 2; ++q) {
         const int ll = q < L ? q : 0;
@@ -912,7 +922,7 @@
       }
       const bidx::DetEntity de_{s->det_seg, s->det_sg};
       bidx::entity_grad(strm, s->DXe, 2, b->key_sorted, b->pos_sorted, b->n_index, N, T, DH, c.dt, c.de, c.Ve, a.gWe, &ra,
-                        sg_on ? &sg : nullptr, det ? &de_ : nullptr);
+                        sg_on ? &sg : nullptr, det ? &de_ : nullptr, beside ? &pbw : nullptr);
       if (det) bidx::entity_grad_tail(strm, b->key_sorted, b->n_index, c.de, c.Ve, a.gWe, de_, sg_on ? &sg : nullptr);
       reduced = true;
     }
@@ -973,7 +983,9 @@
   if (ident) {
     ProfScope ps(h, "small_tables_finish");
     kk::small_tables_finish(strm, s->gG, NS_ID, 4 * DH, DH, c.dt, c.de, c.dr, c.Vt, c.Vr, h->dense + h->off_Wt, h->dense + h->off_Wr, h->dense + h->layer[0].Wi,
-                            gd + h->layer[0].Wi, gd + h->off_Wt, gd + h->off_Wr, false);
+                            gd + h->layer[0].Wi, gd + h->off_Wt, gd + h->off_Wr, false, beside ? &papply : nullptr);
+  } else if (beside) {
+    prefix_apply_launch(h, papply);
   }
 }
 
diff --git a/kprn_amd/csrc/lstm_fused_common.h b/kprn_amd/csrc/lstm_fused_common.h
--- a/kprn_amd/csrc/lstm_fused_common.h
+++ b/kprn_amd/csrc/lstm_fused_common.h
@@ -327,6 +327,8 @@
   float* pfs = nullptr;
   float* pfx = nullptr;
   float* PG = nullptr;
+  float* pap = nullptr;
+  int64_t dxe_zero_pos = 0;
   float* r1 = nullptr;
   void* mc_wsp = nullptr; float* mc_bias = nullptr; bool mc_dirty = true; int mc_ns = 0;
   float* mc_hseq[2] = {nullptr, nullptr}; int64_t mc_capN[2] = {0, 0}; int mc_capT[2] = {0, 0};
diff --git a/kprn_amd/csrc/lstm_fused_prefix.hip b/kprn_amd/csrc/lstm_fused_prefix.hip
--- a/kprn_amd/csrc/lstm_fused_prefix.hip
+++ b/kprn_amd/csrc/lstm_fused_prefix.hip
@@ -1,5 +1,9 @@
+#include <stdint.h>
+#include <string.h>
+
 #include "lstm_fused_common.h"
 #include "adam_rows_dev.h"
+#include "prefix_bwd_dev.h"
 
 namespace fused {
 
@@ -121,99 +125,12 @@
   kk_dev::adam_rows_lane_block<G>(ra, (int64_t)blockIdx.x - 1);
 }
 
-struct PrefBwdArgs {
-  int kmax;
-  int32_t ref[16];
-  int F, nT, L, T;
-  int dt, de, dr;
-  const float* Wi[2];
-  const float* Wo[2];
-  const float* pfs;
-  const float* pfx;
-  float* PG;
-  float* r1;
-  float *gWt, *gWe, *gWr;
-  float* DXv;
-  float* DXe_v;
-  int entity_direct;
-};
-
-__device__ __forceinline__ float col_dot(const float (&w)[64], const float* v256, float (*red)[DH]) {
-  const int c = threadIdx.x & 63, part = threadIdx.x >> 6;
-  float acc0 = 0.f, acc1 = 0.f;
-#pragma unroll
-  for (int i = 0; i < 64; i += 2) { acc0 += w[i] * v256[part * 64 + i]; acc1 += w[i + 1] * v256[part * 64 + i + 1]; }
-  red[part][c] = acc0 + acc1;
-  __syncthreads();
-  return (red[0][c] + red[1][c]) + (red[2][c] + red[3][c]);
-}
-
 __global__ __launch_bounds__(256) void k_prefix_bwd(PrefBwdArgs a) {
   __shared__ float dAn[4 * DH], dAg[4 * DH], up[KCAP][DH], red[4][DH], red2[4][DH];
-  const int r = threadIdx.x;
-  const int c = r & 63, part = r >> 6;
-  const int L = a.L;
-  const int kmax = a.kmax;
-  const int32_t* ids = a.ref;
-  for (int l = L - 1; l >= 0; --l) {
-    float wi[64], wo[64];
-#pragma unroll
-    for (int i = 0; i < 64; ++i) {
-      wi[i] = a.Wi[l][(int64_t)(part * 64 + i) * DH + c];
-      wo[i] = a.Wo[l][(int64_t)(part * 64 + i) * DH + c];
-    }
-    float dA_next = 0.f;
-    float dc_next = 0.f;
-    for (int t = kmax - 1; t >= 0; --t) {
-      float* pg = a.PG + ((int64_t)l * (KCAP + 1) + (t + 1)) * PFB;
-      float* r1 = a.r1 + ((int64_t)l * KCAP + t) * R1;
-      const float v = dA_next + pg[r];
-      pg[r] = 0.f;
-      dAn[r] = v;
-      r1[r] = v;
-      float pgc = 0.f;
-      if (r < DH) {
-        r1[2 * 4 * DH + r] = a.pfs[((int64_t)(t * L + l) * NPL + 6) * DH + r];
-        r1[2 * 4 * DH + DH + r] = (l == 0) ? a.pfx[r] : a.pfs[((int64_t)(t * L + l - 1) * NPL + 6) * DH + r];
-        pgc = pg[4 * DH + r];
-        pg[4 * DH + r] = 0.f;
-      }
-      __syncthreads();
-      const float dh = col_dot(wo, dAn, red);
-      if (r < DH) {
-        const float dc = dc_next + pgc;
-        const float dhv = dh + ((l < L - 1) ? up[t][r] : 0.f);
-        const float* P = a.pfs + (int64_t)(t * L + l) * NPL * DH + r;
-        const float dC = dc + dhv * P[4 * DH];
-        dAg[r] = dC * P[0 * DH];
-        dAg[DH + r] = dC * P[1 * DH];
-        dAg[2 * DH + r] = dC * P[2 * DH];
-        dAg[3 * DH + r] = dhv * P[3 * DH];
-        dc_next = dC * P[5 * DH];
-      }
-      __syncthreads();
-      dA_next = dAg[r];
-      r1[4 * DH + r] = dA_next;
-      const float dx = col_dot(wi, dAg, red2);
-      if (r < DH) {
-        if (l > 0) {
-          up[t][r] = dx;
-        } else {
-          a.DXv[((int64_t)t * 4 + (r >> 4)) * 256 + (r & 15) * 4] = dx;
-          if (a.DXe_v && r >= a.dt && r < a.dt + a.de) a.DXe_v[(int64_t)t * a.de + (r - a.dt)] = dx;
-          if (r < a.dt) {
-            for (int q = 0; q < a.nT; ++q) unsafeAtomicAdd(a.gWt + (int64_t)(ids[a.F - a.nT - 2 + q] - 1) * a.dt + r, dx);
-          } else if (r < a.dt + a.de) {
-            if (a.entity_direct) unsafeAtomicAdd(a.gWe + (int64_t)(ids[a.F - 2] - 1) * a.de + (r - a.dt), dx);
-          } else {
-            unsafeAtomicAdd(a.gWr + (int64_t)(ids[a.F - 1] - 1) * a.dr + (r - a.dt - a.de), dx);
-          }
-        }
-      }
-      __syncthreads();
-    }
-  }
-}
+  prefix_bwd_walk<false>(a, dAn, dAg, up, red, red2);
+}
+
+__global__ __launch_bounds__(256) void k_prefix_terms(bidx::PrefixApply a) { bidx::prefix_apply_block(a, blockIdx.x, 0); }
 
 static void ensure_prefix_buffers(State* s, hipStream_t stream) {
   if (s->pfb) return;
@@ -280,11 +197,10 @@
   s->pf_batch = b->serial;
 }
 
-bool prefix_backward(kprn_handle* h, const kprn_batch* b, int64_t n_tiles) {
-  State* s = st(h);
-  const kprn_config& c = h->cfg;
-  if (!b->tile_k || b->h_kmax == 0) return false;
-  PrefBwdArgs a;
+static void prefix_bwd_args(kprn_handle* h, const kprn_batch* b, int64_t n_tiles, PrefBwdArgs& a) {
+  State* s = st(h);
+  const kprn_config& c = h->cfg;
+  memset(&a, 0, sizeof(a));
   a.kmax = b->h_kmax;
   for (int q = 0; q < 16; ++q) a.ref[q] = b->h_ref[q];
   a.F = b->F; a.nT = c.num_types; a.L = c.L; a.T = b->T;
@@ -299,10 +215,50 @@
   a.DXv = s->DX + (size_t)n_tiles * 4 * b->T * 4 * 256;
   a.DXe_v = s->DXe_on ? s->DXe + (size_t)n_tiles * MT * b->T * c.de : nullptr;
   a.entity_direct = (kprn_dbg_mask() & 16) ? 1 : 0;
+  a.virt0 = INT32_MAX;
+}
+
+bool prefix_backward(kprn_handle* h, const kprn_batch* b, int64_t n_tiles) {
+  if (!b->tile_k || b->h_kmax == 0) return false;
+  PrefBwdArgs a;
+  prefix_bwd_args(h, b, n_tiles, a);
   ProfScope ps(h, "prefix_bwd");
   hipLaunchKernelGGL(k_prefix_bwd, dim3(1), dim3(256), 0, h->stream, a);
   HIP_TRY(hipGetLastError());
   return true;
 }
 
-}
+bool prefix_beside_route(const kprn_handle* h, const kprn_batch* b, bool have_index) {
+  return h->prefix_beside && b->tile_k && b->h_kmax > 0 && have_index && !(kprn_dbg_mask() & 1);
+}
+
+void prefix_beside_jobs(kprn_handle* h, const kprn_batch* b, int64_t n_tiles, PrefBwdArgs* pb, bidx::PrefixApply* pa) {
+  State* s = st(h);
+  const kprn_config& c = h->cfg;
+  if (!s->pap) HIP_TRY(kprn_dev_malloc((void**)&s->pap, (size_t)2 * KCAP * DH * sizeof(float)));
+  prefix_bwd_args(h, b, n_tiles, *pb);
+  pb->DXv = nullptr; pb->DXe_v = nullptr; pb->entity_direct = 0;
+  pb->dx0 = s->pap; pb->up = s->pap + (size_t)KCAP * DH;
+  pb->virt0 = (int)(n_tiles * MT * (int64_t)b->T);
+  pb->zero_pos = (int)s->dxe_zero_pos;
+  memset(pa, 0, sizeof(*pa));
+  pa->kmax = b->h_kmax; pa->L = c.L; pa->kcap = KCAP; pa->r1_stride = R1; pa->G = 4; pa->H = DH;
+  pa->r1 = s->r1; pa->dx = s->pap;
+  pa->hs = s->pfs + (size_t)6 * DH; pa->hs_stride = (int64_t)NPL * DH; pa->x0 = s->pfx;
+  float* gd = h->g_dense;
+  for (int l = 0; l < 2; ++l) {
+    const int ll = l < c.L ? l : 0;
+    pa->gWi[l] = gd + h->layer[ll].Wi; pa->gWo[l] = gd + h->layer[ll].Wo; pa->gbi[l] = gd + h->layer[ll].bi;
+  }
+  pa->gWt = pb->gWt; pa->gWe = pb->gWe; pa->gWr = pb->gWr;
+  pa->dt = c.dt; pa->de = c.de; pa->dr = c.dr; pa->nT = c.num_types; pa->F = b->F;
+  for (int q = 0; q < 16; ++q) pa->ref[q] = b->h_ref[q];
+}
+
+void prefix_apply_launch(kprn_handle* h, const bidx::PrefixApply& pa) {
+  ProfScope ps(h, "prefix_apply");
+  hipLaunchKernelGGL(k_prefix_terms, dim3((unsigned)bidx::prefix_apply_blocks(pa)), dim3(256), 0, h->stream, pa);
+  HIP_TRY(hipGetLastError());
+}
+
+}
diff --git a/kprn_amd/csrc/prefix_bwd_dev.h b/kprn_amd/csrc/prefix_bwd_dev.h
--- /dev/null
+++ b/kprn_amd/csrc/prefix_bwd_dev.h
@@ -0,0 +1,139 @@
+#pragma once
+#include "lstm_fused_common.h"
+
+namespace fused {
+
+struct PrefBwdArgs {
+  int kmax;
+  int32_t ref[16];
+  int F, nT, L, T;
+  int dt, de, dr;
+  const float* Wi[2];
+  const float* Wo[2];
+  const float* pfs;
+  const float* pfx;
+  float* PG;
+  float* r1;
+  float *gWt, *gWe, *gWr;
+  float* DXv;
+  float* DXe_v;
+  int entity_direct;
+  float* dx0;
+  float* up;
+  int virt0;
+  int zero_pos;
+};
+
+__device__ __forceinline__ float col_dot(const float (&w)[64], const float* v256, float (*red)[DH]) {
+  const int c = threadIdx.x & 63, part = threadIdx.x >> 6;
+  float acc0 = 0.f, acc1 = 0.f;
+#pragma unroll
+  for (int i = 0; i < 64; i += 2) { acc0 += w[i] * v256[part * 64 + i]; acc1 += w[i + 1] * v256[part * 64 + i + 1]; }
+  red[part][c] = acc0 + acc1;
+  __syncthreads();
+  return (red[0][c] + red[1][c]) + (red[2][c] + red[3][c]);
+}
+constexpr int CDS = 32;
+static_assert(CDS == 32 || CDS == 64, "col_dot_stream: two batches, or one");
+__device__ __forceinline__ float col_dot_stream(const float* __restrict__ W, const float mine, float (*red)[DH]) {
+  const int c = threadIdx.x & 63, part = __builtin_amdgcn_readfirstlane(threadIdx.x >> 6);
+  float acc[4] = {0.f, 0.f, 0.f, 0.f};
+#pragma unroll 1
+  for (int q = 0; q < 64 / CDS; ++q) {
+    const __amdgpu_buffer_rsrc_t rs = __builtin_amdgcn_make_buffer_rsrc((void*)(W + (int64_t)(part * 64 + q * CDS) * DH), 0, CDS * DH * 4, 0x00020000);
+    float x[CDS];
+#pragma unroll
+    for (int i = 0; i < CDS; ++i)
+      x[i] = __builtin_bit_cast(float, __builtin_amdgcn_raw_buffer_load_b32(rs, c * 4, i * DH * 4, 0));
+#pragma unroll
+    for (int i = 0; i < CDS; ++i) {
+      float f;
+      if (q == 0) f = __builtin_bit_cast(float, __builtin_amdgcn_readlane(__builtin_bit_cast(int, mine), i));
+      else f = __builtin_bit_cast(float, __builtin_amdgcn_readlane(__builtin_bit_cast(int, mine), (CDS + i) & 63));
+      acc[i & 3] += x[i] * f;
+    }
+  }
+  red[part][c] = (acc[0] + acc[1]) + (acc[2] + acc[3]);
+  __syncthreads();
+  return (red[0][c] + red[1][c]) + (red[2][c] + red[3][c]);
+}
+
+template <bool STREAM>
+__device__ __forceinline__ void prefix_bwd_walk(const PrefBwdArgs& a, float* dAn, float* dAg, float (*up)[DH], float (*red)[DH], float (*red2)[DH]) {
+  const int r = threadIdx.x;
+  const int c = r & 63, part = r >> 6;
+  const int L = a.L;
+  const int kmax = a.kmax;
+  const int32_t* ids = a.ref;
+  for (int l = L - 1; l >= 0; --l) {
+    float wi[STREAM ? 1 : 64], wo[STREAM ? 1 : 64];
+    if constexpr (!STREAM) {
+#pragma unroll
+      for (int i = 0; i < 64; ++i) {
+        wi[i] = a.Wi[l][(int64_t)(part * 64 + i) * DH + c];
+        wo[i] = a.Wo[l][(int64_t)(part * 64 + i) * DH + c];
+      }
+    }
+    float dA_next = 0.f;
+    float dc_next = 0.f;
+    for (int t = kmax - 1; t >= 0; --t) {
+      float* pg = a.PG + ((int64_t)l * (KCAP + 1) + (t + 1)) * PFB;
+      float* r1 = a.r1 + ((int64_t)l * KCAP + t) * R1;
+      const float v = dA_next + pg[r];
+      pg[r] = 0.f;
+      dAn[r] = v;
+      r1[r] = v;
+      float pgc = 0.f;
+      float P0 = 0.f, P1 = 0.f, P2 = 0.f, P3 = 0.f, P4 = 0.f, P5 = 0.f, upv = 0.f;
+      if (r < DH) {
+        const float* P = a.pfs + (int64_t)(t * L + l) * NPL * DH + r;
+        P0 = P[0 * DH]; P1 = P[1 * DH]; P2 = P[2 * DH]; P3 = P[3 * DH]; P4 = P[4 * DH]; P5 = P[5 * DH];
+        if (l < L - 1) upv = up[t][r];
+        if constexpr (!STREAM) {
+          r1[2 * 4 * DH + r] = a.pfs[((int64_t)(t * L + l) * NPL + 6) * DH + r];
+          r1[2 * 4 * DH + DH + r] = (l == 0) ? a.pfx[r] : a.pfs[((int64_t)(t * L + l - 1) * NPL + 6) * DH + r];
+        }
+        pgc = pg[4 * DH + r];
+        pg[4 * DH + r] = 0.f;
+      }
+      __syncthreads();
+      float dh;
+      if constexpr (STREAM) dh = col_dot_stream(a.Wo[l], v, red); else dh = col_dot(wo, dAn, red);
+      if (r < DH) {
+        const float dc = dc_next + pgc;
+        const float dhv = dh + upv;
+        const float dC = dc + dhv * P4;
+        dAg[r] = dC * P0;
+        dAg[DH + r] = dC * P1;
+        dAg[2 * DH + r] = dC * P2;
+        dAg[3 * DH + r] = dhv * P3;
+        dc_next = dC * P5;
+      }
+      __syncthreads();
+      dA_next = dAg[r];
+      r1[4 * DH + r] = dA_next;
+      float dx;
+      if constexpr (STREAM) dx = col_dot_stream(a.Wi[l], dA_next, red2); else dx = col_dot(wi, dAg, red2);
+      if (r < DH) {
+        if (l > 0) {
+          up[t][r] = dx;
+        } else if constexpr (STREAM) {
+          a.dx0[t * DH + r] = dx;
+        } else {
+          a.DXv[((int64_t)t * 4 + (r >> 4)) * 256 + (r & 15) * 4] = dx;
+          if (a.DXe_v && r >= a.dt && r < a.dt + a.de) a.DXe_v[(int64_t)t * a.de + (r - a.dt)] = dx;
+          if (r < a.dt) {
+            for (int q = 0; q < a.nT; ++q) unsafeAtomicAdd(a.gWt + (int64_t)(ids[a.F - a.nT - 2 + q] - 1) * a.dt + r, dx);
+          } else if (r < a.dt + a.de) {
+            if (a.entity_direct) unsafeAtomicAdd(a.gWe + (int64_t)(ids[a.F - 2] - 1) * a.de + (r - a.dt), dx);
+          } else {
+            unsafeAtomicAdd(a.gWr + (int64_t)(ids[a.F - 1] - 1) * a.dr + (r - a.dt - a.de), dx);
+          }
+        }
+      }
+      __syncthreads();
+    }
+  }
+}
+
+}
```

Result: no change. 51.36 million (median of 6 runs) (+0.8%).
